# MachinaIO/mxx

Hardware: AMD Instinct MI355X
Metric: dcrt_ring_ops_per_s (higher is better)
Workload: dtype u32

## Files before the change

include/gpupoly.h:

```cpp
#ifndef GPUPOLY_H
#define GPUPOLY_H

#include <stddef.h>
#include <stdint.h>

#ifdef __cplusplus
extern "C" {
#endif

typedef struct GpuContext GpuContext;
typedef struct GpuMatrix GpuMatrix;
typedef struct GpuEventSet GpuEventSet;
typedef struct GpuP1CovarianceCache GpuP1CovarianceCache;
typedef struct GpuComm GpuComm;

typedef struct GpuRngSeed {
    uint64_t words[4];
} GpuRngSeed;

#define GPU_POLY_FORMAT_COEFF 0
#define GPU_POLY_FORMAT_EVAL 1
#define GPU_MATRIX_DIST_UNIFORM 0
#define GPU_MATRIX_DIST_GAUSS 1
#define GPU_MATRIX_DIST_BIT 2
#define GPU_MATRIX_DIST_TERNARY 3
#define GPU_MATRIX_LAYOUT_WORDS 0
#define GPU_MATRIX_LAYOUT_PACKED24 1

int gpu_context_create(uint32_t logN, uint32_t L, uint32_t dnum, const uint64_t *moduli, size_t moduli_len,
                       const int *gpu_ids, size_t gpu_ids_len, GpuContext **out_ctx);
void gpu_context_destroy(GpuContext *ctx);
int gpu_context_get_N(const GpuContext *ctx, int *out_N);

int gpu_event_set_wait(GpuEventSet *events);
void gpu_event_set_destroy(GpuEventSet *events);

int gpu_device_count(int *out_count);
int gpu_device_mem_info(int device, size_t *out_free, size_t *out_total);
int gpu_device_synchronize(void);
int gpu_device_reset(void);

const char *gpu_last_error(void);
int gpu_set_last_error(const char *msg);

void *gpu_pinned_alloc(size_t bytes);
void gpu_pinned_free(void *ptr);

int gpu_matrix_create(GpuContext *ctx, int level, size_t rows, size_t cols, int format, GpuMatrix **out);
void gpu_matrix_destroy(GpuMatrix *mat);
int gpu_matrix_copy(GpuMatrix *dst, const GpuMatrix *src);
int gpu_matrix_copy_block(GpuMatrix *out, const GpuMatrix *src, size_t dst_row, size_t dst_col, size_t src_row,
                          size_t src_col, size_t rows, size_t cols);

int gpu_matrix_add(GpuMatrix *out, const GpuMatrix *lhs, const GpuMatrix *rhs);
int gpu_matrix_sub(GpuMatrix *out, const GpuMatrix *lhs, const GpuMatrix *rhs);
int gpu_matrix_add_block(GpuMatrix *out, const GpuMatrix *src, size_t dst_row, size_t dst_col, size_t src_row,
                         size_t src_col, size_t rows, size_t cols);
int gpu_matrix_mul(GpuMatrix *out, const GpuMatrix *lhs, const GpuMatrix *rhs);
int gpu_matrix_mul_scalar(GpuMatrix *out, const GpuMatrix *lhs, const GpuMatrix *scalar);
int gpu_matrix_equal(const GpuMatrix *lhs, const GpuMatrix *rhs, int *out_equal);

int gpu_matrix_ntt_all(GpuMatrix *mat);
int gpu_matrix_intt_all(GpuMatrix *mat);

int gpu_matrix_fill_gadget(GpuMatrix *out, uint32_t base_bits);
int gpu_matrix_fill_small_gadget(GpuMatrix *out, uint32_t base_bits);
int gpu_matrix_fill_small_decomposed_identity_chunk(GpuMatrix *out, const GpuMatrix *scalar_by_digit,
                                                    size_t chunk_idx);
int gpu_matrix_decompose_base(const GpuMatrix *src, uint32_t base_bits, GpuMatrix *out);
int gpu_matrix_decompose_base_small(const GpuMatrix *src, uint32_t base_bits, GpuMatrix *out);

int gpu_matrix_sample_distribution(GpuMatrix *out, int dist_type, double sigma, GpuRngSeed seed);
int gpu_matrix_sample_distribution_columns(GpuMatrix *out, int dist_type, double sigma, GpuRngSeed seed,
                                           size_t full_ncol, size_t col_offset);
int gpu_matrix_gauss_samp_gq_arb_base(GpuMatrix *src, uint32_t base_bits, double c, double dgg_stddev,
                                      GpuRngSeed seed, GpuMatrix *out);
int gpu_matrix_sample_p1_full(const GpuMatrix *a_mat, const GpuMatrix *b_mat, const GpuMatrix *d_mat,
                              const GpuMatrix *tp2, double sigma, double s, double dgg_stddev, GpuRngSeed seed,
                              GpuMatrix *out);
int gpu_matrix_create_p1_covariance_cache(const GpuMatrix *a_mat, const GpuMatrix *b_mat, const GpuMatrix *d_mat,
                                          double sigma, double s, double dgg_stddev,
                                          GpuP1CovarianceCache **out_cache);
void gpu_matrix_destroy_p1_covariance_cache(GpuP1CovarianceCache *cache);
int gpu_matrix_sample_p1_full_cached(const GpuP1CovarianceCache *cache, const GpuMatrix *tp2, GpuRngSeed seed,
                                     GpuMatrix *out);

int gpu_matrix_load_rns_batch(GpuMatrix *mat, const uint8_t *bytes, size_t bytes_per_poly, int format,
                              GpuEventSet **out_events);
int gpu_matrix_store_rns_batch(const GpuMatrix *mat, uint8_t *bytes_out, size_t bytes_per_poly, int format,
                               GpuEventSet **out_events);
int gpu_matrix_store_const_coeff_batch(const GpuMatrix *mat, uint64_t *words_out, size_t words_per_poly,
                                       GpuEventSet **out_events);
int gpu_matrix_store_compact_bytes(GpuMatrix *mat, uint8_t *payload_out, size_t payload_capacity,
                                   uint16_t *out_max_coeff_bits, uint16_t *out_bytes_per_coeff,
                                   size_t *out_payload_len);
int gpu_matrix_load_compact_bytes(GpuMatrix *mat, const uint8_t *payload, size_t payload_len,
                                  uint16_t max_coeff_bits);
int gpu_poly_store_compact_bytes(GpuMatrix *poly, uint8_t *payload_out, size_t payload_capacity,
                                 uint16_t *out_max_coeff_bits, uint16_t *out_bytes_per_coeff,
                                 size_t *out_payload_len);
int gpu_poly_load_compact_bytes(GpuMatrix *poly, const uint8_t *payload, size_t payload_len,
                                uint16_t max_coeff_bits);

int gpupoly_matrix_mul_decompose(GpuMatrix *out, const GpuMatrix *lhs, const GpuMatrix *rhs, uint32_t base_bits);
int gpupoly_matrix_mul_decompose_many(GpuMatrix *const *outs, const GpuMatrix *const *lhss,
                                      const GpuMatrix *const *addends, const GpuMatrix *const *scalars, size_t n,
                                      const GpuMatrix *rhs, uint32_t base_bits);
int gpupoly_matrix_mul_decompose_pairs(GpuMatrix *const *outs, const GpuMatrix *const *addends,
                                       const GpuMatrix *const *lhss, const GpuMatrix *const *rhss,
                                       const GpuMatrix *const *scalars, size_t n,
                                       size_t col_start, uint32_t base_bits, int negate);
int gpupoly_matrix_mul_batch(GpuMatrix *const *outs, const GpuMatrix *const *lhss, const GpuMatrix *const *rhss, size_t count);
#define GPUPOLY_OP_MUL 0
#define GPUPOLY_OP_ADD 1
#define GPUPOLY_OP_SUB 2
#define GPUPOLY_OP_MUL_SCALAR 3
#define GPUPOLY_OP_NEG 4
#define GPUPOLY_OP_DECOMPOSE 5
#define GPUPOLY_OP_MUL_DECOMPOSE 6
typedef struct GpuBatchOp {
    int kind;
    GpuMatrix *out;
    const GpuMatrix *lhs;
    const GpuMatrix *rhs;
} GpuBatchOp;
int gpupoly_batch(const GpuBatchOp *ops, size_t count, uint32_t base_bits);
int gpupoly_matrix_mul_decompose_small(GpuMatrix *out, const GpuMatrix *lhs, const GpuMatrix *rhs, uint32_t base_bits);
int gpupoly_matrix_mul_tensor_identity(GpuMatrix *out, const GpuMatrix *lhs, const GpuMatrix *rhs, size_t identity_size);
int gpupoly_matrix_mul_tensor_identity_decompose(GpuMatrix *out, const GpuMatrix *lhs, const GpuMatrix *rhs,
                                                 size_t identity_size, uint32_t base_bits);
int gpupoly_matrix_mul_scalar_intt(GpuMatrix *out, const GpuMatrix *lhs, const GpuMatrix *scalar_1x1);
int gpupoly_matrix_transpose(GpuMatrix *out, const GpuMatrix *src);
int gpupoly_matrix_tensor(GpuMatrix *out, const GpuMatrix *lhs, const GpuMatrix *rhs);
int gpupoly_matrix_add_rows(GpuMatrix *out, size_t dst_row, const GpuMatrix *lhs, const GpuMatrix *rhs);
int gpupoly_matrix_ntt_add_rows(GpuMatrix *out, size_t dst_row, GpuMatrix *coeff, const GpuMatrix *addend,
                                int consume_coeff);
int gpupoly_matrix_row_view(GpuMatrix *m, size_t row, size_t rows, GpuMatrix **out_view);
int gpupoly_matrix_reshape_view(GpuMatrix *m, size_t rows, size_t cols, GpuMatrix **out_view);
int gpupoly_matrix_neg(GpuMatrix *out, const GpuMatrix *src);
int gpupoly_matrix_fill_zero(GpuMatrix *out);
int gpupoly_matrix_fill_identity(GpuMatrix *out, const GpuMatrix *scalar_1x1);
int gpupoly_matrix_sample_decomposed(GpuMatrix *out, int dist_type, double sigma, GpuRngSeed seed, uint32_t base_bits,
                                     int small);
int gpupoly_matrix_decompose_rows(const GpuMatrix *src, uint32_t base_bits, int small, size_t row_start, GpuMatrix *out);
int gpupoly_matrix_sample_decomposed_window(GpuMatrix *out, int dist_type, double sigma, GpuRngSeed seed,
                                            uint32_t base_bits, int small, size_t src_rows, size_t full_ncol,
                                            size_t col_offset, size_t row_start);
int gpupoly_timer_start(GpuContext *ctx);
int gpupoly_timer_stop(GpuContext *ctx, float *out_ms);
int gpupoly_timer_mark(GpuContext *ctx, uint32_t slot);
int gpupoly_timer_elapsed(GpuContext *ctx, uint32_t slot_begin, uint32_t slot_end, float *out_ms);
int gpupoly_matrix_device_ptr(const GpuMatrix *mat, void **out_ptr, size_t *out_bytes);
int gpupoly_matrix_layout(const GpuMatrix *mat, int *out);
int gpupoly_matrix_copy_to_context(GpuContext *dst_ctx, const GpuMatrix *src, GpuMatrix **out);
int gpupoly_context_device(const GpuContext *ctx, int *out_device);
int gpupoly_context_word_bytes(const GpuContext *ctx, int *out_bytes);
const char *gpupoly_context_last_kernel(const GpuContext *ctx);
int gpupoly_context_stream(const GpuContext *ctx, void **out_stream);
int gpupoly_comm_create(GpuContext *const *ctxs, size_t n, GpuComm **out_comm);
void gpupoly_comm_destroy(GpuComm *comm);
int gpupoly_comm_size(const GpuComm *comm, int *out_size);
const char *gpupoly_comm_backend(const GpuComm *comm);
int gpupoly_matrix_all_gather_columns(GpuComm *comm, const GpuMatrix *const *local_blocks, GpuMatrix *const *full);
int gpupoly_matrix_sample_distribution_segments(GpuMatrix *out, int dist_type, double sigma, const GpuRngSeed *seeds,
                                                const size_t *seg_cols, size_t nseg);
int gpupoly_matrix_sample_p1_full_cached_segments(const GpuP1CovarianceCache *cache, const GpuMatrix *tp2,
                                                  const GpuRngSeed *seeds, const size_t *seg_cols, size_t nseg,
                                                  GpuMatrix *out);
int gpupoly_matrix_gauss_samp_gq_arb_base_segments(GpuMatrix *src, uint32_t base_bits, double c, double dgg_stddev,
                                                   const GpuRngSeed *seeds, const size_t *seg_cols, size_t nseg,
                                                   GpuMatrix *out);
#define GPUPOLY_BLOCKS_STACKED 0
#define GPUPOLY_BLOCKS_COLUMNS 1
int gpupoly_matrix_sample_distribution_blocks(GpuMatrix *out, int dist_type, const GpuRngSeed *seeds, size_t nblk,
                                              int layout, const size_t *seg_cols);
#define GPUPOLY_HASH_KECCAK256 0
#define GPUPOLY_HASH_SHA3_256 1
#define GPUPOLY_TAGS_TABLE 0
#define GPUPOLY_TAGS_INDEXED_LE64 1
#define GPUPOLY_TAGS_INDEXED_DECIMAL 2
typedef struct GpuHashTags {
    int hash;
    int form;
    uint8_t key[32];
    const uint8_t *tags;
    const size_t *tag_offsets;
    size_t prefix_len;
    uint64_t first_index;
} GpuHashTags;
int gpupoly_hash_seeds(GpuContext *ctx, const GpuHashTags *tags, size_t ntags, GpuRngSeed *seeds_out);
int gpupoly_matrix_sample_hash_blocks(GpuMatrix *out, int dist_type, const GpuHashTags *tags, size_t nblk, int layout,
                                      const size_t *seg_cols);
int gpupoly_matrix_sample_gauss_blocks(GpuMatrix *out, double sigma, const GpuRngSeed *seeds, size_t nblk, int layout,
                                       const size_t *seg_cols);
int gpupoly_matrix_sample_hash_gauss_blocks(GpuMatrix *out, double sigma, const GpuHashTags *tags, size_t nblk, int layout,
                                            const size_t *seg_cols);
int gpupoly_matrix_concat_columns(GpuMatrix *out, const GpuMatrix *const *blocks, size_t n);
int gpupoly_matrix_split_columns(const GpuMatrix *src, GpuMatrix *const *blocks, size_t n);
int gpupoly_trapdoor_preimage_many(const GpuMatrix *re, const GpuP1CovarianceCache *cache, const GpuMatrix *public_matrix,
                                   uint32_t base_bits, const GpuMatrix *const *targets, size_t n, const GpuRngSeed *seeds,
                                   GpuMatrix *const *outs);
int gpupoly_trapdoor_preimage_keyed(const GpuMatrix *const *res, const GpuP1CovarianceCache *const *caches,
                                    const GpuMatrix *const *public_matrices, size_t nkeys, uint32_t base_bits,
                                    const uint32_t *key_of, const GpuMatrix *const *targets, size_t n,
                                    const GpuRngSeed *seeds, GpuMatrix *const *outs);
int gpupoly_matrix_sample_decomposed_blocks(GpuMatrix *out, int dist_type, const GpuRngSeed *seeds, size_t nblk,
                                            uint32_t base_bits, int small, size_t src_rows, size_t full_ncol,
                                            size_t col_offset);
int gpupoly_matrix_sample_hash_decomposed_blocks(GpuMatrix *out, int dist_type, const GpuHashTags *tags, size_t nblk,
                                                 uint32_t base_bits, int small, size_t src_rows, size_t full_ncol,
                                                 size_t col_offset);
int gpupoly_matrix_lut_targets(GpuMatrix *const *outs, size_t nrows_T, const GpuMatrix *w_identity, const GpuMatrix *w_gy,
                               const GpuMatrix *w_v, const GpuMatrix *w_vx, size_t col_start, uint32_t base_bits,
                               const uint64_t *y_words, size_t words_per_y, const uint64_t *idx, const GpuHashTags *tags);
int gpupoly_matrix_lut_targets_combine(GpuMatrix *const *outs, size_t nrows_T, const GpuMatrix *w_identity,
                                       const GpuMatrix *w_gy, const GpuMatrix *product, size_t col_start, uint32_t base_bits,
                                       const uint64_t *y_words, size_t words_per_y, const uint64_t *idx);
int gpupoly_matrix_lwe_targets(GpuMatrix *const *outs, size_t nrows_T, const GpuMatrix *a_z, const GpuMatrix *a_lt,
                               size_t col_start, uint32_t base_bits, const uint64_t *y_words, size_t words_per_y,
                               const uint64_t *x, const GpuHashTags *tags);
int gpupoly_matrix_lwe_targets_combine(GpuMatrix *const *outs, size_t nrows_T, const GpuMatrix *a_lt,
                                       const GpuMatrix *digits, const GpuMatrix *product, size_t col_start,
                                       uint32_t base_bits, const uint64_t *y_words, size_t words_per_y, const uint64_t *x);
int gpupoly_matrix_wee25_targets(GpuMatrix *const *outs, size_t nblocks_T, size_t nparts_P, const GpuMatrix *t_bottom,
                                 size_t part_start, size_t secret_size, uint32_t base_bits, const uint64_t *idx,
                                 const GpuHashTags *tags);
int gpupoly_matrix_wee25_targets_product(GpuMatrix *const *outs, size_t nblocks_T, size_t nparts_P, const GpuMatrix *w_stacked,
                                         const GpuMatrix *t_bottom, size_t part_start, size_t secret_size,
                                         uint32_t base_bits, const uint64_t *idx);
int gpupoly_matrix_ggh15_lookup(GpuMatrix *const *outs, size_t nslots_S, const GpuMatrix *mid_identity,
                                const GpuMatrix *mid_gy, const GpuMatrix *mid_v, const GpuMatrix *mid_vx,
                                const GpuMatrix *mid_rand, const GpuMatrix *mid_gate1,
                                const GpuMatrix *const *lut_preimages, const GpuMatrix *const *xs, size_t col_start,
                                uint32_t base_bits, const uint64_t *y_words, size_t words_per_y, const GpuHashTags *tags);
int gpupoly_matrix_ggh15_lookup_combine(GpuMatrix *const *outs, size_t nslots_S, const GpuMatrix *mid_identity,
                                        const GpuMatrix *mid_gy, const GpuMatrix *mid_v, const GpuMatrix *mid_vx,
                                        const GpuMatrix *mid_rand, const GpuMatrix *mid_gate1,
                                        const GpuMatrix *const *lut_preimages, const GpuMatrix *const *xs, size_t col_start,
                                        uint32_t base_bits, const uint64_t *y_words, size_t words_per_y,
                                        const GpuMatrix *digits);
int gpupoly_matrix_scale_round(GpuMatrix *out, const GpuMatrix *in, uint64_t t, int round_half);
int gpupoly_matrix_crt_recompose_rounded(GpuMatrix *out, const GpuMatrix *const *terms, const int *signs,
                                         size_t terms_per_level, size_t num_slots);
int gpupoly_matrix_store_coeff_words(const GpuMatrix *mat, uint64_t *out, size_t words_per_coeff);
int gpupoly_matrix_load_coeff_words(GpuMatrix *mat, const uint64_t *words, size_t words_per_coeff, size_t coeffs_per_poly,
                                    int out_format);
int gpupoly_matrix_centered_max_abs(const GpuMatrix *mat, uint64_t *out, size_t words_per_value);
int gpupoly_matrix_extract_bits(const GpuMatrix *mat, const uint64_t *lo, const uint64_t *hi, size_t words_per_bound,
                                uint8_t *out, size_t bytes_per_poly);
int gpupoly_matrix_store_coeff_ints(const GpuMatrix *mat, void *out, int elem_bytes, int centred, size_t coeffs_per_poly,
                                    uint64_t *out_misfit_count, uint64_t *out_first_misfit);
int gpupoly_matrix_store_compact_bytes_many(GpuMatrix *const *mats, size_t n, uint8_t *payload_out, size_t payload_capacity,
                                            uint16_t *out_max_coeff_bits, uint16_t *out_bytes_per_coeff,
                                            size_t *out_payload_offsets, size_t *out_payload_lens, size_t *out_total_len);
int gpupoly_matrix_load_compact_bytes_many(GpuMatrix *const *mats, size_t n, const uint8_t *const *payloads,
                                           const size_t *payload_lens, const uint16_t *max_coeff_bits);
int gpupoly_matrix_fill_monomial(GpuMatrix *out, uint64_t shift, int format);
int gpupoly_matrix_mul_monomial(GpuMatrix *out, const GpuMatrix *in, uint64_t shift);
int gpupoly_matrix_monomial_sum(GpuMatrix *out, const GpuMatrix *addend, const GpuMatrix *const *mats,
                                const uint64_t *shifts, size_t n, int negate);
int gpupoly_matrix_mul_sum(GpuMatrix *out, size_t dst_col, size_t cols, const GpuMatrix *addend,
                           const GpuMatrix *const *lhss, const GpuMatrix *const *rhss, size_t n, int negate);
int gpupoly_matrix_mul_acc(GpuMatrix *out, const GpuMatrix *lhs, const GpuMatrix *rhs, int negate);
int gpupoly_matrix_mul_gadget(GpuMatrix *out, size_t dst_col, const GpuMatrix *lhs, const GpuMatrix *scalar_1x1,
                              size_t gadget_col, size_t cols, const GpuMatrix *addend, int negate, uint32_t base_bits,
                              int small);
int gpupoly_matrix_gadget_mul(GpuMatrix *out, const GpuMatrix *rhs, const GpuMatrix *addend, int negate,
                              uint32_t base_bits, int small);
int gpupoly_matrix_mul_decompose_gadget_scalar_many(GpuMatrix *const *outs, const GpuMatrix *const *lhss,
                                                    const GpuMatrix *const *addends, size_t n, const GpuMatrix *scalar_1x1,
                                                    int negate, uint32_t base_bits);
int gpupoly_matrix_mul_decompose_gadget_const_many(GpuMatrix *const *outs, const GpuMatrix *const *lhss,
                                                   const GpuMatrix *const *addends, size_t n, const uint64_t *const_words,
                                                   size_t words_per_const, int negate, uint32_t base_bits);
uint64_t gpupoly_launch_count(void);
int gpupoly_detmath_eval(GpuContext *ctx, int fn, const double *host_in, double *host_out, size_t n);
int gpupoly_device_can_access_peer(int device, int peer, int *out_can);
int gpupoly_marker_launch(GpuContext *ctx, uint32_t id);
int gpupoly_trace_begin(void);
const char *gpupoly_trace_end(void);
const char *gpupoly_version(void);
int gpupoly_reload_env(void);

#ifdef __cplusplus
}
#endif
#endif
```

mxx_amd/__init__.py:

```python
from ._ffi import (
    GPU_MATRIX_DIST_BIT,
    GPU_MATRIX_DIST_GAUSS,
    GPU_MATRIX_DIST_TERNARY,
    GPU_MATRIX_DIST_UNIFORM,
    GPU_POLY_FORMAT_COEFF,
    GPU_POLY_FORMAT_EVAL,
    GpuPolyError,
    GpuRngSeed,
    detected_gpu_device_count,
    detected_gpu_device_ids,
    gpu_device_sync,
)
from .matrix import (
    GpuDCRTMatrixRnsSnapshot,
    GpuDCRTPolyMatrix,
    GpuP1CovarianceCache,
    block_offsets,
    block_size,
    one_rns_bytes,
    rns_bytes_len,
    rns_bytes_len_for_level,
)
from .params import DCRTPolyParams, GpuContext, GpuDCRTPolyParams, gen_crt_basis
from .poly import GpuDCRTPoly
from . import storage
from .sampler import (
    DistType,
    GpuDCRTPolyHashSampler,
    GpuDCRTPolyUniformSampler,
    IndexedTags,
    hash_seed_for_matrix,
    keccak256,
    random_gpu_rng_seed,
    sample_gpu_matrix_native,
    sample_gpu_matrix_with_seed,
    sample_gpu_matrix_with_seed_columns,
)
from .trapdoor import (
    GpuDCRTPolyTrapdoorSampler,
    GpuDCRTTrapdoor,
    GpuPerturbationSamples,
    coeff_cached_matrix,
    compute_preimage_norm,
    p1_covariance_parameters,
    preimage_c,
    preimage_smoothing_parameter,
)
from . import lookup
from . import lwe_lookup
from . import ggh15_eval
from . import slot_transfer
from . import commit
```

mxx_amd/_ffi.py:

```python
from __future__ import annotations

import ctypes as C
import os

_HERE = os.path.dirname(os.path.abspath(__file__))
LIB_PATH = os.environ.get("MXX_GPUPOLY_LIB") or os.path.join(_HERE, "libgpupoly.so")

GPU_POLY_FORMAT_COEFF = 0
GPU_POLY_FORMAT_EVAL = 1
GPU_MATRIX_DIST_UNIFORM = 0
GPU_MATRIX_DIST_GAUSS = 1
GPU_MATRIX_DIST_BIT = 2
GPU_MATRIX_DIST_TERNARY = 3
GPUPOLY_BLOCKS_STACKED = 0
GPUPOLY_BLOCKS_COLUMNS = 1
GPUPOLY_HASH_KECCAK256 = 0
GPUPOLY_HASH_SHA3_256 = 1
GPUPOLY_TAGS_TABLE = 0
GPUPOLY_TAGS_INDEXED_LE64 = 1
GPUPOLY_TAGS_INDEXED_DECIMAL = 2


class GpuPolyError(RuntimeError):
    """Raised where the reference's Rust wrapper panics (`check_status`, gpu.rs:259-263)."""


class GpuRngSeed(C.Structure):

    _fields_ = [("words", C.c_uint64 * 4)]

    @classmethod
    def from_bytes(cls, b: bytes) -> "GpuRngSeed":
        if len(b) != 32:
            raise ValueError("seed must be 32 bytes")
        s = cls()
        for i in range(4):
            s.words[i] = int.from_bytes(b[8 * i : 8 * i + 8], "little")
        return s

    def to_bytes(self) -> bytes:
        return b"".join(int(w).to_bytes(8, "little") for w in self.words)


class GpuHashTags(C.Structure):

    _fields_ = [("hash", C.c_int), ("form", C.c_int), ("key", C.c_uint8 * 32), ("tags", C.c_void_p),
                ("tag_offsets", C.POINTER(C.c_size_t)), ("prefix_len", C.c_size_t), ("first_index", C.c_uint64)]


class GpuBatchOp(C.Structure):

    _fields_ = [("kind", C.c_int), ("out", C.c_void_p), ("lhs", C.c_void_p), ("rhs", C.c_void_p)]


GPUPOLY_OP_MUL, GPUPOLY_OP_ADD, GPUPOLY_OP_SUB, GPUPOLY_OP_MUL_SCALAR, GPUPOLY_OP_NEG, GPUPOLY_OP_DECOMPOSE, GPUPOLY_OP_MUL_DECOMPOSE = range(7)

_vp = C.c_void_p
_sz = C.c_size_t
_u8p = C.POINTER(C.c_uint8)

SIGNATURES = {
    "gpu_context_create": (C.c_int, [C.c_uint32, C.c_uint32, C.c_uint32, C.POINTER(C.c_uint64), _sz, C.POINTER(C.c_int), _sz, C.POINTER(_vp)]),
    "gpu_context_destroy": (None, [_vp]),
    "gpu_context_get_N": (C.c_int, [_vp, C.POINTER(C.c_int)]),
    "gpu_event_set_wait": (C.c_int, [_vp]),
    "gpu_event_set_destroy": (None, [_vp]),
    "gpu_device_count": (C.c_int, [C.POINTER(C.c_int)]),
    "gpu_device_mem_info": (C.c_int, [C.c_int, C.POINTER(_sz), C.POINTER(_sz)]),
    "gpu_device_synchronize": (C.c_int, []),
    "gpu_device_reset": (C.c_int, []),
    "gpu_last_error": (C.c_char_p, []),
    "gpu_set_last_error": (C.c_int, [C.c_char_p]),
    "gpu_pinned_alloc": (_vp, [_sz]),
    "gpu_pinned_free": (None, [_vp]),
    "gpu_matrix_create": (C.c_int, [_vp, C.c_int, _sz, _sz, C.c_int, C.POINTER(_vp)]),
    "gpu_matrix_destroy": (None, [_vp]),
    "gpu_matrix_copy": (C.c_int, [_vp, _vp]),
    "gpu_matrix_copy_block": (C.c_int, [_vp, _vp, _sz, _sz, _sz, _sz, _sz, _sz]),
    "gpu_matrix_add": (C.c_int, [_vp, _vp, _vp]),
    "gpu_matrix_sub": (C.c_int, [_vp, _vp, _vp]),
    "gpu_matrix_add_block": (C.c_int, [_vp, _vp, _sz, _sz, _sz, _sz, _sz, _sz]),
    "gpu_matrix_mul": (C.c_int, [_vp, _vp, _vp]),
    "gpu_matrix_mul_scalar": (C.c_int, [_vp, _vp, _vp]),
    "gpu_matrix_equal": (C.c_int, [_vp, _vp, C.POINTER(C.c_int)]),
    "gpu_matrix_ntt_all": (C.c_int, [_vp]),
    "gpu_matrix_intt_all": (C.c_int, [_vp]),
    "gpu_matrix_fill_gadget": (C.c_int, [_vp, C.c_uint32]),
    "gpu_matrix_fill_small_gadget": (C.c_int, [_vp, C.c_uint32]),
    "gpu_matrix_fill_small_decomposed_identity_chunk": (C.c_int, [_vp, _vp, _sz]),
    "gpu_matrix_decompose_base": (C.c_int, [_vp, C.c_uint32, _vp]),
    "gpu_matrix_decompose_base_small": (C.c_int, [_vp, C.c_uint32, _vp]),
    "gpu_matrix_sample_distribution": (C.c_int, [_vp, C.c_int, C.c_double, GpuRngSeed]),
    "gpu_matrix_sample_distribution_columns": (C.c_int, [_vp, C.c_int, C.c_double, GpuRngSeed, _sz, _sz]),
    "gpu_matrix_gauss_samp_gq_arb_base": (C.c_int, [_vp, C.c_uint32, C.c_double, C.c_double, GpuRngSeed, _vp]),
    "gpu_matrix_sample_p1_full": (C.c_int, [_vp, _vp, _vp, _vp, C.c_double, C.c_double, C.c_double, GpuRngSeed, _vp]),
    "gpu_matrix_create_p1_covariance_cache": (C.c_int, [_vp, _vp, _vp, C.c_double, C.c_double, C.c_double, C.POINTER(_vp)]),
    "gpu_matrix_destroy_p1_covariance_cache": (None, [_vp]),
    "gpu_matrix_sample_p1_full_cached": (C.c_int, [_vp, _vp, GpuRngSeed, _vp]),
    "gpu_matrix_load_rns_batch": (C.c_int, [_vp, _vp, _sz, C.c_int, C.POINTER(_vp)]),
    "gpu_matrix_store_rns_batch": (C.c_int, [_vp, _vp, _sz, C.c_int, C.POINTER(_vp)]),
    "gpu_matrix_store_const_coeff_batch": (C.c_int, [_vp, _vp, _sz, C.POINTER(_vp)]),
    "gpu_matrix_store_compact_bytes": (C.c_int, [_vp, _vp, _sz, C.POINTER(C.c_uint16), C.POINTER(C.c_uint16), C.POINTER(_sz)]),
    "gpu_matrix_load_compact_bytes": (C.c_int, [_vp, _vp, _sz, C.c_uint16]),
    "gpu_poly_store_compact_bytes": (C.c_int, [_vp, _vp, _sz, C.POINTER(C.c_uint16), C.POINTER(C.c_uint16), C.POINTER(_sz)]),
    "gpu_poly_load_compact_bytes": (C.c_int, [_vp, _vp, _sz, C.c_uint16]),
    "gpupoly_matrix_mul_decompose": (C.c_int, [_vp, _vp, _vp, C.c_uint32]),
    "gpupoly_matrix_mul_decompose_many": (C.c_int, [C.POINTER(C.c_void_p), C.POINTER(C.c_void_p), C.POINTER(C.c_void_p), C.POINTER(C.c_void_p), C.c_size_t, _vp, C.c_uint32]),
    "gpupoly_matrix_mul_decompose_pairs": (C.c_int, [C.POINTER(C.c_void_p), C.POINTER(C.c_void_p), C.POINTER(C.c_void_p), C.POINTER(C.c_void_p), C.POINTER(C.c_void_p), _sz, _sz, C.c_uint32, C.c_int]),
    "gpupoly_matrix_mul_batch":(C.c_int, [C.POINTER(C.c_void_p), C.POINTER(C.c_void_p), C.POINTER(C.c_void_p), C.c_size_t]),
    "gpupoly_batch": (C.c_int, [C.POINTER(GpuBatchOp), C.c_size_t, C.c_uint32]),
    "gpupoly_matrix_mul_decompose_small": (C.c_int, [_vp, _vp, _vp, C.c_uint32]),
    "gpupoly_matrix_mul_tensor_identity": (C.c_int, [_vp, _vp, _vp, C.c_size_t]),
    "gpupoly_matrix_mul_tensor_identity_decompose": (C.c_int, [_vp, _vp, _vp, C.c_size_t, C.c_uint32]),
    "gpupoly_matrix_mul_scalar_intt": (C.c_int, [_vp, _vp, _vp]),
    "gpupoly_matrix_transpose": (C.c_int, [_vp, _vp]),
    "gpupoly_matrix_tensor": (C.c_int, [_vp, _vp, _vp]),
    "gpupoly_matrix_add_rows": (C.c_int, [_vp, C.c_size_t, _vp, _vp]),
    "gpupoly_matrix_ntt_add_rows": (C.c_int, [_vp, C.c_size_t, _vp, _vp, C.c_int]),
    "gpupoly_matrix_row_view": (C.c_int, [_vp, C.c_size_t, C.c_size_t, C.POINTER(C.c_void_p)]),
    "gpupoly_matrix_reshape_view": (C.c_int, [_vp, C.c_size_t, C.c_size_t, C.POINTER(C.c_void_p)]),
    "gpupoly_matrix_neg": (C.c_int, [_vp, _vp]),
    "gpupoly_matrix_fill_zero": (C.c_int, [_vp]),
    "gpupoly_matrix_fill_identity": (C.c_int, [_vp, _vp]),
    "gpupoly_matrix_sample_decomposed": (C.c_int, [_vp, C.c_int, C.c_double, GpuRngSeed, C.c_uint32, C.c_int]),
    "gpupoly_matrix_decompose_rows": (C.c_int, [_vp, C.c_uint32, C.c_int, _sz, _vp]),
    "gpupoly_matrix_sample_decomposed_window": (C.c_int, [_vp, C.c_int, C.c_double, GpuRngSeed, C.c_uint32, C.c_int, _sz, _sz, _sz, _sz]),
    "gpupoly_timer_start": (C.c_int, [_vp]),
    "gpupoly_timer_stop": (C.c_int, [_vp, C.POINTER(C.c_float)]),
    "gpupoly_timer_mark": (C.c_int, [_vp, C.c_uint32]),
    "gpupoly_timer_elapsed": (C.c_int, [_vp, C.c_uint32, C.c_uint32, C.POINTER(C.c_float)]),
    "gpupoly_matrix_device_ptr": (C.c_int, [_vp, C.POINTER(_vp), C.POINTER(_sz)]),
    "gpupoly_matrix_layout": (C.c_int, [_vp, C.POINTER(C.c_int)]),
    "gpupoly_matrix_copy_to_context": (C.c_int, [_vp, _vp, C.POINTER(_vp)]),
    "gpupoly_context_device": (C.c_int, [_vp, C.POINTER(C.c_int)]),
    "gpupoly_context_word_bytes": (C.c_int, [_vp, C.POINTER(C.c_int)]),
    "gpupoly_context_last_kernel": (C.c_char_p, [_vp]),
    "gpupoly_context_stream": (C.c_int, [_vp, C.POINTER(C.c_void_p)]),
    "gpupoly_comm_create": (C.c_int, [C.POINTER(C.c_void_p), C.c_size_t, C.POINTER(_vp)]),
    "gpupoly_comm_destroy": (None, [_vp]),
    "gpupoly_comm_size": (C.c_int, [_vp, C.POINTER(C.c_int)]),
    "gpupoly_comm_backend": (C.c_char_p, [_vp]),
    "gpupoly_matrix_all_gather_columns": (C.c_int, [_vp, C.POINTER(C.c_void_p), C.POINTER(C.c_void_p)]),
    "gpupoly_matrix_sample_distribution_segments": (C.c_int, [_vp, C.c_int, C.c_double, C.POINTER(GpuRngSeed), C.POINTER(_sz), _sz]),
    "gpupoly_matrix_sample_distribution_blocks": (C.c_int, [_vp, C.c_int, C.POINTER(GpuRngSeed), _sz, C.c_int, C.POINTER(_sz)]),
    "gpupoly_hash_seeds": (C.c_int, [_vp, C.POINTER(GpuHashTags), _sz, C.POINTER(GpuRngSeed)]),
    "gpupoly_matrix_sample_hash_blocks": (C.c_int, [_vp, C.c_int, C.POINTER(GpuHashTags), _sz, C.c_int, C.POINTER(_sz)]),
    "gpupoly_matrix_sample_gauss_blocks": (C.c_int, [_vp, C.c_double, C.POINTER(GpuRngSeed), _sz, C.c_int, C.POINTER(_sz)]),
    "gpupoly_matrix_sample_hash_gauss_blocks": (C.c_int, [_vp, C.c_double, C.POINTER(GpuHashTags), _sz, C.c_int, C.POINTER(_sz)]),
    "gpupoly_matrix_sample_decomposed_blocks": (C.c_int, [_vp, C.c_int, C.POINTER(GpuRngSeed), _sz, C.c_uint32, C.c_int, _sz, _sz, _sz]),
    "gpupoly_matrix_sample_hash_decomposed_blocks": (C.c_int, [_vp, C.c_int, C.POINTER(GpuHashTags), _sz, C.c_uint32, C.c_int, _sz, _sz, _sz]),
    "gpupoly_matrix_lut_targets": (C.c_int, [C.POINTER(C.c_void_p), _sz, _vp, _vp, _vp, _vp, _sz, C.c_uint32, C.POINTER(C.c_uint64), _sz,
                                   C.POINTER(C.c_uint64), C.POINTER(GpuHashTags)]),
    "gpupoly_matrix_lut_targets_combine": (C.c_int, [C.POINTER(C.c_void_p), _sz, _vp, _vp, _vp, _sz, C.c_uint32, C.POINTER(C.c_uint64), _sz,
                                           C.POINTER(C.c_uint64)]),
    "gpupoly_matrix_lwe_targets": (C.c_int, [C.POINTER(C.c_void_p), _sz, _vp, _vp, _sz, C.c_uint32, C.POINTER(C.c_uint64), _sz,
                                   C.POINTER(C.c_uint64), C.POINTER(GpuHashTags)]),
    "gpupoly_matrix_lwe_targets_combine": (C.c_int, [C.POINTER(C.c_void_p), _sz, _vp, _vp, _vp, _sz, C.c_uint32, C.POINTER(C.c_uint64), _sz,
                                           C.POINTER(C.c_uint64)]),
    "gpupoly_matrix_wee25_targets": (C.c_int, [C.POINTER(C.c_void_p), _sz, _sz, _vp, _sz, _sz, C.c_uint32, C.POINTER(C.c_uint64),
                                     C.POINTER(GpuHashTags)]),
    "gpupoly_matrix_wee25_targets_product": (C.c_int, [C.POINTER(C.c_void_p), _sz, _sz, _vp, _vp, _sz, _sz, C.c_uint32,
                                             C.POINTER(C.c_uint64)]),
    "gpupoly_matrix_ggh15_lookup": (C.c_int, [C.POINTER(C.c_void_p), _sz, _vp, _vp, _vp, _vp, _vp, _vp, C.POINTER(C.c_void_p),
                                    C.POINTER(C.c_void_p), _sz, C.c_uint32, C.POINTER(C.c_uint64), _sz, C.POINTER(GpuHashTags)]),
    "gpupoly_matrix_ggh15_lookup_combine": (C.c_int, [C.POINTER(C.c_void_p), _sz, _vp, _vp, _vp, _vp, _vp, _vp, C.POINTER(C.c_void_p),
                                            C.POINTER(C.c_void_p), _sz, C.c_uint32, C.POINTER(C.c_uint64), _sz, _vp]),
    "gpupoly_matrix_sample_p1_full_cached_segments":(C.c_int, [_vp, _vp, C.POINTER(GpuRngSeed), C.POINTER(_sz), _sz, _vp]),
    "gpupoly_matrix_gauss_samp_gq_arb_base_segments": (C.c_int, [_vp, C.c_uint32, C.c_double, C.c_double, C.POINTER(GpuRngSeed), C.POINTER(_sz), _sz, _vp]),
    "gpupoly_matrix_concat_columns": (C.c_int, [_vp, C.POINTER(C.c_void_p), _sz]),
    "gpupoly_matrix_split_columns": (C.c_int, [_vp, C.POINTER(C.c_void_p), _sz]),
    "gpupoly_trapdoor_preimage_many": (C.c_int, [_vp, _vp, _vp, C.c_uint32, C.POINTER(C.c_void_p), _sz, C.POINTER(GpuRngSeed), C.POINTER(C.c_void_p)]),
    "gpupoly_trapdoor_preimage_keyed": (C.c_int, [C.POINTER(C.c_void_p), C.POINTER(C.c_void_p), C.POINTER(C.c_void_p), _sz, C.c_uint32,
                                        C.POINTER(C.c_uint32), C.POINTER(C.c_void_p), _sz, C.POINTER(GpuRngSeed), C.POINTER(C.c_void_p)]),
    "gpupoly_launch_count": (C.c_uint64, []),
    "gpupoly_matrix_scale_round": (C.c_int, [_vp, _vp, C.c_uint64, C.c_int]),
    "gpupoly_matrix_crt_recompose_rounded": (C.c_int, [_vp, C.POINTER(C.c_void_p), C.POINTER(C.c_int), _sz, _sz]),
    "gpupoly_matrix_store_coeff_words": (C.c_int, [_vp, C.POINTER(C.c_uint64), _sz]),
    "gpupoly_matrix_load_coeff_words": (C.c_int, [_vp, C.POINTER(C.c_uint64), _sz, _sz, C.c_int]),
    "gpupoly_matrix_centered_max_abs": (C.c_int, [_vp, C.POINTER(C.c_uint64), _sz]),
    "gpupoly_matrix_extract_bits": (C.c_int, [_vp, C.POINTER(C.c_uint64), C.POINTER(C.c_uint64), _sz, _u8p, _sz]),
    "gpupoly_matrix_store_coeff_ints": (C.c_int, [_vp, _vp, C.c_int, C.c_int, _sz, C.POINTER(C.c_uint64), C.POINTER(C.c_uint64)]),
    "gpupoly_matrix_fill_monomial": (C.c_int, [_vp, C.c_uint64, C.c_int]),
    "gpupoly_matrix_mul_monomial": (C.c_int, [_vp, _vp, C.c_uint64]),
    "gpupoly_matrix_monomial_sum": (C.c_int, [_vp, _vp, C.POINTER(C.c_void_p), C.POINTER(C.c_uint64), _sz, C.c_int]),
    "gpupoly_matrix_mul_sum": (C.c_int, [_vp, _sz, _sz, _vp, C.POINTER(C.c_void_p), C.POINTER(C.c_void_p), _sz, C.c_int]),
    "gpupoly_matrix_mul_acc": (C.c_int, [_vp, _vp, _vp, C.c_int]),
    "gpupoly_matrix_mul_gadget": (C.c_int, [_vp, _sz, _vp, _vp, _sz, _sz, _vp, C.c_int, C.c_uint32, C.c_int]),
    "gpupoly_matrix_gadget_mul": (C.c_int, [_vp, _vp, _vp, C.c_int, C.c_uint32, C.c_int]),
    "gpupoly_matrix_mul_decompose_gadget_scalar_many": (C.c_int, [C.POINTER(C.c_void_p), C.POINTER(C.c_void_p), C.POINTER(C.c_void_p), _sz, _vp, C.c_int, C.c_uint32]),
    "gpupoly_matrix_mul_decompose_gadget_const_many": (C.c_int, [C.POINTER(C.c_void_p), C.POINTER(C.c_void_p), C.POINTER(C.c_void_p), _sz, C.POINTER(C.c_uint64), _sz, C.c_int, C.c_uint32]),
    "gpupoly_matrix_store_compact_bytes_many": (C.c_int, [C.POINTER(C.c_void_p), _sz, _vp, _sz, C.POINTER(C.c_uint16), C.POINTER(C.c_uint16), C.POINTER(_sz), C.POINTER(_sz), C.POINTER(_sz)]),
    "gpupoly_matrix_load_compact_bytes_many": (C.c_int, [C.POINTER(C.c_void_p), _sz, C.POINTER(C.c_void_p), C.POINTER(_sz), C.POINTER(C.c_uint16)]),
    "gpupoly_detmath_eval": (C.c_int, [_vp, C.c_int, C.POINTER(C.c_double), C.POINTER(C.c_double), _sz]),
    "gpupoly_device_can_access_peer": (C.c_int, [C.c_int, C.c_int, C.POINTER(C.c_int)]),
    "gpupoly_marker_launch": (C.c_int, [_vp, C.c_uint32]),
    "gpupoly_trace_begin": (C.c_int, []),
    "gpupoly_trace_end": (C.c_char_p, []),
    "gpupoly_version": (C.c_char_p, []),
    "gpupoly_reload_env": (C.c_int, []),
}

_lib = None


def lib() -> C.CDLL:
    global _lib
    if _lib is None:
        if not os.path.exists(LIB_PATH):
            raise GpuPolyError(
                f"{LIB_PATH} is missing: build it with `python -c 'import __graft_entry__ as g; g.build()'` "
                "(or `make -C mxx_amd/csrc`). mxx_amd has no CPU fallback."
            )
        handle = C.CDLL(LIB_PATH)
        for name, (res, args) in SIGNATURES.items():
            fn = getattr(handle, name)
            fn.restype = res
            fn.argtypes = args
        _lib = handle
    return _lib


def last_error_string() -> str:
    msg = lib().gpu_last_error()
    return msg.decode("utf-8", "replace") if msg else "unknown GPU error"


def check_status(code: int, context: str) -> None:
    if code != 0:
        raise GpuPolyError(f"{context} failed: {last_error_string()}")


def reload_env() -> None:
    check_status(lib().gpupoly_reload_env(), "gpupoly_reload_env")


def trace_begin() -> None:
    check_status(lib().gpupoly_trace_begin(), "gpupoly_trace_begin")


def trace_end() -> list[dict]:
    text = lib().gpupoly_trace_end()
    if text is None:
        raise GpuPolyError(f"gpupoly_trace_end failed: {last_error_string()}")
    out = []
    for ln in text.decode().splitlines():
        name, blocks, threads, nbytes, ms = ln.split("\t")
        out.append({"kernel": name.strip("()"), "blocks": int(blocks), "threads": int(threads), "bytes": float(nbytes), "ms": float(ms)})
    return out


def gpu_device_sync() -> None:
    check_status(lib().gpu_device_synchronize(), "gpu_device_synchronize")


def detected_gpu_device_ids() -> list[int]:
    n = C.c_int(0)
    if lib().gpu_device_count(C.byref(n)) != 0 or n.value <= 0:
        return []
    return list(range(n.value))


def peer_access_matrix(devices=None) -> list[list[int]]:
    devs = detected_gpu_device_ids() if devices is None else list(devices)
    out = []
    for a in devs:
        row = []
        for b in devs:
            can = C.c_int(0)
            check_status(lib().gpupoly_device_can_access_peer(a, b, C.byref(can)), "gpupoly_device_can_access_peer")
            row.append(int(can.value))
        out.append(row)
    return out


def detected_gpu_device_count() -> int:
    return len(detected_gpu_device_ids())


def wait_and_destroy_events(events: _vp) -> None:
    if events:
        st = lib().gpu_event_set_wait(events)
        lib().gpu_event_set_destroy(events)
        check_status(st, "gpu_event_set_wait")
```

mxx_amd/csrc/common.h:

```cpp
#pragma once

#include <hip/hip_runtime.h>

#include <atomic>
#include <cstddef>
#include <cstdint>
#include <cstdio>
#include <exception>
#include <map>
#include <unordered_map>
#include <mutex>
#include <string>
#include <vector>

#include "../../include/gpupoly.h"

constexpr size_t GPUPOLY_MAX_LIMBS = 64;

struct LimbConst {
    uint64_t q;
    uint64_t mu;
    uint64_t mu64;
    uint64_t n_inv;
    uint64_t n_inv_sh;
    uint64_t mu32;
    uint64_t inv_last_w;
    uint64_t inv_last_w_sh;
    uint32_t kbits;
    uint32_t lazy_terms;
};

struct EnvSwitches {
    int ntt_path = 0;
    int ntt14 = 0;
    bool decompose_fused = true;
    char matmul_path = 0;
    int matmul_tile = 0;
    bool gsamp_simple = false;
    bool gsamp_no_uni = false;
    bool p1_simple = false;
    int sampler_per_lane = 0;
    int sampler_fill_every = 0;
    bool ntt64_int = false;
    int ntt_phase = 0;
    bool serde_general = false;
    bool rng_compat = false;
    bool pack24 = true;
    int skinny24 = 0;
    int skinny24_shape = 0;
    size_t mul_decompose_many_budget = 0;
    size_t mul_decompose_pairs_budget = 0;
    size_t gadget_scalar_budget = 0;
    size_t ggh15_lookup_budget = 0;
    char mul_sum_path = 0;
    size_t crt_recompose_chunk_bytes = size_t(256) << 20;
    void load();
};

struct GpuContext {
    EnvSwitches env;
    int device = 0;
    std::vector<int> gpu_ids;
    uint32_t logN = 0;
    int N = 0;
    int level = 0;
    uint32_t dnum = 0;
    int limb_count = 0;
    bool wide = false;
    int word_bytes = 4;
    uint32_t crt_bits = 0;
    std::vector<uint64_t> moduli;
    hipStream_t stream = nullptr;
    LimbConst *d_limbs = nullptr;
    LimbConst *d_limbs_r = nullptr;
    void *d_tw_fwd = nullptr;
    void *d_tw_fwd_sh = nullptr;
    void *d_tw_inv = nullptr;
    void *d_tw_inv_sh = nullptr;
    void *d_tw2_fwd = nullptr;
    void *d_tw2_inv = nullptr;
    bool lazy_ok = false;
    bool tight_ok = false;
    void *d_tw2s_inv = nullptr;
    bool signed_ok = false;
    void *d_twf_fwd = nullptr, *d_twf_inv = nullptr;
    void *d_flimbs = nullptr;
    bool f64_ok = false;
    uint64_t *d_garner = nullptr;
    std::vector<uint64_t> garner_inv;
    std::vector<LimbConst> limbs;
    hipEvent_t timer_start = nullptr, timer_stop = nullptr;
    std::vector<hipEvent_t> marks;
    std::mutex mutex;
    bool pool_ok = false;
    std::mutex alloc_mutex;
    std::multimap<size_t, void *> free_blocks;
    std::unordered_map<void *, size_t> live_blocks;
    size_t cached_bytes = 0, cache_limit = 0;
    std::atomic<const char *> last_kernel{""};
    bool pack24_ok = false;
    std::mutex layout_mutex;
    std::map<uint32_t, void *> gadget_weights;
    std::map<std::vector<uint64_t>, void *> gadget_const_tables;
};

struct LayoutTag {
    std::atomic<int> v{GPU_MATRIX_LAYOUT_WORDS};
    LayoutTag() = default;
    LayoutTag(const LayoutTag &o) : v(o.v.load(std::memory_order_acquire)) {}
    LayoutTag &operator=(const LayoutTag &o) {
        v.store(o.v.load(std::memory_order_acquire), std::memory_order_release);
        return *this;
    }
};

struct GpuMatrix {
    GpuContext *ctx = nullptr;
    int level = 0;
    size_t rows = 0, cols = 0;
    int format = GPU_POLY_FORMAT_EVAL;
    void *storage = nullptr;
    size_t bytes = 0;
    LayoutTag layout;
    bool borrowed = false;
    GpuMatrix *parent = nullptr;
    int views = 0;
};

struct GpuEventSet {
    std::vector<hipEvent_t> events;
    int device = 0;
    void *staging = nullptr;
    GpuContext *ctx = nullptr;
    void *dev_staging = nullptr;
};

struct GpuP1CovarianceCache {
    GpuContext *ctx = nullptr;
    int level = 0;
    size_t d = 0, m = 0, n = 0;
    double sigma = 0, s = 0, dgg_stddev = 0;
    double *sqrt_var = nullptr;
    double *update_coeff = nullptr;
    void *karney_div = nullptr;
};

struct P1KeyEntry {
    const double *sqrt_var;
    const double *update_coeff;
    const void *karney_div;
};

static inline dim3 item_grid(size_t items, unsigned threads) {
    const size_t blocks = (items + threads - 1) / threads;
    const size_t max_x = (static_cast<size_t>(1) << 31) / threads;
    if (blocks <= max_x) return dim3(static_cast<unsigned>(blocks ? blocks : 1));
    const size_t y = (blocks + max_x - 1) / max_x;
    return dim3(static_cast<unsigned>((blocks + y - 1) / y), static_cast<unsigned>(y));
}
#if defined(__HIPCC__)
__device__ __forceinline__ size_t item_index() {
    return (static_cast<size_t>(blockIdx.y) * gridDim.x + blockIdx.x) * blockDim.x + threadIdx.x;
}
#endif

extern std::atomic<uint64_t> g_kernel_launches;
extern std::atomic<int> g_trace_on;
void trace_launch_begin(const char *name, hipStream_t stream, dim3 grid, dim3 block);
void trace_launch_end(hipStream_t stream);
void trace_set_bytes(double bytes);
#define MXX_TRACE_BYTES(b)                                                                        \
    do {                                                                                          \
        if (g_trace_on.load(std::memory_order_relaxed)) trace_set_bytes(static_cast<double>(b)); \
    } while (0)
#define MXX_LAUNCH(kern, grid, block, lds, strm, ...)                          \
    do {                                                                       \
        g_kernel_launches.fetch_add(1, std::memory_order_relaxed);             \
        const bool mxx_tr_ = g_trace_on.load(std::memory_order_relaxed) != 0;  \
        if (mxx_tr_) trace_launch_begin(#kern, strm, grid, block);             \
        hipLaunchKernelGGL(kern, grid, block, lds, strm, __VA_ARGS__);         \
        if (mxx_tr_) trace_launch_end(strm);                                   \
    } while (0)
#define MXX_TRACED_COPY(name, strm, bytes, stmt)                               \
    do {                                                                       \
        const bool mxx_tr_ = g_trace_on.load(std::memory_order_relaxed) != 0;  \
        if (mxx_tr_) {                                                         \
            trace_set_bytes(static_cast<double>(bytes));                       \
            trace_launch_begin(name, strm, dim3(0), dim3(0));                  \
        }                                                                      \
        stmt;                                                                  \
        if (mxx_tr_) trace_launch_end(strm);                                   \
    } while (0)

int set_error(const char *msg);
int set_error(const std::string &msg);
int set_error(hipError_t err, const char *what);

#define HIP_TRY(expr)                                          \
    do {                                                       \
        hipError_t _e = (expr);                                \
        if (_e != hipSuccess) return set_error(_e, #expr);     \
    } while (0)

template <auto... KERNELS>
static int lds_opt_in(const GpuContext *ctx, size_t lds) {
    static std::atomic<uint64_t> configured{0};
    const uint64_t bit = 1ull << (ctx->device & 63);
    if (lds <= 64 * 1024 || (configured.load() & bit)) return 0;
    for (const void *f : {reinterpret_cast<const void *>(KERNELS)...})
        HIP_TRY(hipFuncSetAttribute(f, hipFuncAttributeMaxDynamicSharedMemorySize, static_cast<int>(lds)));
    configured.fetch_or(bit);
    return 0;
}

extern int (*g_roctx_push)(const char *);
extern int (*g_roctx_pop)();
void roctx_init_once();
struct RoctxScope {
    bool on;
    explicit RoctxScope(const char *name) {
        roctx_init_once();
        on = g_roctx_push != nullptr;
        if (on) g_roctx_push(name);
    }
    ~RoctxScope() {
        if (on) g_roctx_pop();
    }
};

#define ABI_GUARD_BEGIN try { RoctxScope roctx_scope_(__func__);
#define ABI_GUARD_END                                                         \
    }                                                                         \
    catch (const std::exception &e) { return set_error(e.what()); }           \
    catch (...) { return set_error("unknown exception in libgpupoly"); }

inline size_t matrix_polys(const GpuMatrix *m) { return m->rows * m->cols; }
inline size_t matrix_limbs(const GpuMatrix *m) { return static_cast<size_t>(m->level) + 1; }
inline size_t matrix_words(const GpuMatrix *m) { return matrix_polys(m) * matrix_limbs(m) * static_cast<size_t>(m->ctx->N); }

void *words_ptr(const GpuMatrix *m);
const void *packed24_ptr(const GpuMatrix *m, bool *packed);
inline size_t packed24_bytes(const GpuMatrix *m) { return m->bytes / 4 * 3; }
inline bool storage_overlaps(const GpuMatrix *x, const GpuMatrix *y) {
    if (x == y) return true;
    if (!x->storage || !y->storage || x->bytes == 0 || y->bytes == 0) return false;
    const size_t xb = x->layout.v.load(std::memory_order_acquire) == GPU_MATRIX_LAYOUT_PACKED24 ? packed24_bytes(x) : x->bytes;
    const size_t yb = y->layout.v.load(std::memory_order_acquire) == GPU_MATRIX_LAYOUT_PACKED24 ? packed24_bytes(y) : y->bytes;
    const char *xs = static_cast<const char *>(x->storage), *ys = static_cast<const char *>(y->storage);
    return xs < ys + yb && ys < xs + xb;
}
inline bool same_block(const GpuMatrix *x, const GpuMatrix *y) {
    return x == y || (x->storage == y->storage && x->bytes == y->bytes);
}
inline bool partial_overlap(const GpuMatrix *out, const GpuMatrix *operand) {
    return storage_overlaps(out, operand) && !same_block(out, operand);
}
inline bool row_block_overlaps(const GpuMatrix *m, size_t row, size_t rows, const GpuMatrix *y) {
    if (m->layout.v.load(std::memory_order_acquire) == GPU_MATRIX_LAYOUT_PACKED24) return rows && m->cols && storage_overlaps(m, y);
    if (!m->storage) return false;
    const size_t poly_bytes = matrix_limbs(m) * static_cast<size_t>(m->ctx->N) * m->ctx->word_bytes;
    GpuMatrix block;
    block.storage = static_cast<char *>(m->storage) + row * m->cols * poly_bytes;
    block.bytes = rows * m->cols * poly_bytes;
    return storage_overlaps(&block, y);
}
bool pack24_eligible(const GpuMatrix *m);
int pack24_store(GpuMatrix *m, bool ntt);

int sample_impl(GpuMatrix *out, int dist, double sigma, GpuRngSeed seed, size_t full_ncol, size_t col_offset, bool keep_coeff,
                size_t row_offset = 0, uint32_t tower_first = 0, uint32_t tower_count = 0);

struct RngBlockWindow {
    size_t cols, full_ncol, col_offset;
};
int sample_blocks_impl(const char *entry, bool hashed, GpuMatrix *out, int dist_type, const GpuRngSeed *seeds, const GpuHashTags *tags,
                       size_t nblk, int layout, const size_t *seg_cols, const RngBlockWindow *win, const double *sigma = nullptr);
int sample_decomposed_blocks_impl(const char *entry, bool hashed, GpuMatrix *out, int dist_type, const GpuRngSeed *seeds,
                                  const GpuHashTags *tags, size_t nblk, uint32_t base_bits, int small, size_t src_rows, size_t full_ncol,
                                  size_t col_offset);

int hash_tags_check(const char *entry, const GpuHashTags *tags, size_t ntags, size_t *table_bytes);
size_t hash_tags_staged_words(const GpuHashTags *tags, size_t ntags, size_t table_bytes);
void hash_tags_stage(const GpuHashTags *tags, size_t ntags, size_t table_bytes, uint64_t *staging);
int launch_hash_seeds(GpuContext *ctx, GpuRngSeed *d_seeds, const GpuHashTags *tags, size_t ntags, const uint64_t *d_staged);

int ctx_activate(const GpuContext *ctx);
bool ctx_is_registered(const GpuContext *ctx);
int ctx_alloc(GpuContext *ctx, size_t bytes, void **out);
void ctx_free(GpuContext *ctx, void *ptr);
struct CtxBlock {
    GpuContext *ctx;
    void *ptr = nullptr;
    explicit CtxBlock(GpuContext *c) : ctx(c) {}
    CtxBlock(const CtxBlock &) = delete;
    CtxBlock &operator=(const CtxBlock &) = delete;
    ~CtxBlock() {
        if (ptr) ctx_free(ctx, ptr);
    }
    int alloc(size_t bytes) { return ctx_alloc(ctx, bytes, &ptr); }
    void *release() {
        void *p = ptr;
        ptr = nullptr;
        return p;
    }
};
int matrix_check_same_shape(const GpuMatrix *a, const GpuMatrix *b, const char *who);
int coeff_domain_source(const GpuMatrix *mat, CtxBlock &scratch, const void **src);

int launch_ntt(GpuContext *ctx, void *data, size_t vectors, int limbs_per_poly, bool inverse);
int launch_ntt_lds_u32(GpuContext *ctx, uint32_t *data, size_t vectors, uint32_t L, bool inverse);
int launch_ntt_digits_u32(GpuContext *ctx, uint32_t *out, const uint32_t *coeff, size_t out_vectors, uint32_t L,
                          uint32_t src_cols, uint32_t towers, uint32_t dpt, uint32_t base_bits, size_t k, uint32_t td0 = 0);
int launch_ntt_lds_u64(GpuContext *ctx, uint64_t *data, size_t vectors, uint32_t L, bool inverse);
int launch_ntt_digits_u64(GpuContext *ctx, uint64_t *out, const uint64_t *coeff, size_t out_vectors, uint32_t L,
                          uint32_t src_cols, uint32_t towers, uint32_t dpt, uint32_t base_bits, size_t k, uint32_t td0 = 0);
int launch_intt_oop_u32(GpuContext *ctx, uint32_t *out, const uint32_t *in, size_t vectors, uint32_t L);
int launch_ntt_add_u32(GpuContext *ctx, uint32_t *out, const uint32_t *src, const uint32_t *add, size_t vectors, uint32_t L);
int launch_mul_intt_u32(GpuContext *ctx, uint32_t *out, const uint32_t *in, const uint32_t *w, size_t vectors, uint32_t L);
int launch_matmul(GpuMatrix *out, const GpuMatrix *lhs, const GpuMatrix *rhs);
int launch_ntt_fwd_pack24_u32(GpuContext *ctx, uint32_t *out, const uint32_t *in, size_t vectors, uint32_t L);
int launch_matmul_skinny24(GpuMatrix *out, const GpuMatrix *lhs, const GpuMatrix *rhs, bool small_grid);
int skinny24_parse_shape(const char *s);
int launch_matmul_dma_u32(GpuMatrix *out, const GpuMatrix *lhs, const GpuMatrix *rhs);
int launch_matmul_dma32_u32(GpuMatrix *out, const GpuMatrix *lhs, const GpuMatrix *rhs);
int launch_matmul_mfma_u32(GpuMatrix *out, const GpuMatrix *lhs, const GpuMatrix *rhs);
int launch_copy_block(GpuMatrix *out, const GpuMatrix *src, size_t dst_row, size_t dst_col, size_t src_row,
                      size_t src_col, size_t rows, size_t cols, bool add);
int sample_p1_keyed_segments(const GpuP1CovarianceCache *cache, const P1KeyEntry *d_keys, const GpuMatrix *tp2,
                             const GpuRngSeed *seeds, const size_t *seg_cols, size_t nseg, GpuMatrix *out);
int launch_scatter_i64(GpuMatrix *out, const int64_t *vals);
int finish_staged_i64(GpuMatrix *out, CtxBlock &stage, hipError_t launch_err, const char *what, bool transform = true);
```

mxx_amd/csrc/runtime.hip:

```cpp
#include "common.h"

#include <algorithm>
#include <cstdlib>
#include <iterator>
#include <map>
#include <cstring>
#include <dlfcn.h>

typedef unsigned __int128 u128h;

static thread_local std::string g_last_error;

int set_error(const char *msg) {
    g_last_error = msg ? msg : "unknown error";
    return 1;
}
int set_error(const std::string &msg) {
    g_last_error = msg;
    return 1;
}
int set_error(hipError_t err, const char *what) {
    g_last_error = std::string(what ? what : "hip call") + ": " + hipGetErrorString(err);
    (void)hipGetLastError();
    return 1;
// ... 81 lines not shown
    HIP_TRY(hipGetLastError());
    return 0;
    ABI_GUARD_END
}

extern "C" int gpupoly_trace_begin(void) {
    ABI_GUARD_BEGIN
    std::lock_guard<std::mutex> lk(g_trace_mutex);
    for (const TraceEntry &en : g_trace) {
        trace_event_return(en.device, en.e0);
        trace_event_return(en.device, en.e1);
    }
    g_trace.clear();
    g_trace_on.store(1, std::memory_order_relaxed);
    return 0;
    ABI_GUARD_END
}

extern "C" const char *gpupoly_trace_end(void) {
    try {
        g_trace_on.store(0, std::memory_order_relaxed);
        std::lock_guard<std::mutex> lk(g_trace_mutex);
        g_trace_report.clear();
        int prev = 0;
        (void)hipGetDevice(&prev);
        char line[512];
        for (const TraceEntry &en : g_trace) {
            if (!en.closed) continue;
            (void)hipSetDevice(en.device);
            float ms = 0;
            hipError_t e = hipEventSynchronize(en.e1);
            if (e == hipSuccess) e = hipEventElapsedTime(&ms, en.e0, en.e1);
            if (e != hipSuccess) {
                (void)hipSetDevice(prev);
                set_error(e, "gpupoly_trace_end: hipEventElapsedTime");
                return nullptr;
            }
            std::snprintf(line, sizeof line, "%s\t%llu\t%u\t%.0f\t%.6f\n", en.name, en.blocks, en.threads, en.bytes, ms);
            g_trace_report += line;
        }
        for (const TraceEntry &en : g_trace) {
            trace_event_return(en.device, en.e0);
            trace_event_return(en.device, en.e1);
        }
        g_trace.clear();
        (void)hipSetDevice(prev);
        return g_trace_report.c_str();
    } catch (...) {
        set_error("gpupoly_trace_end: exception");
        return nullptr;
    }
}

int (*g_roctx_push)(const char *) = nullptr;
int (*g_roctx_pop)() = nullptr;
void roctx_init_once() {
    static std::once_flag once;
    std::call_once(once, [] {
        const char *sw = std::getenv("MXX_HIP_ROCTX");
        const bool profiled = std::getenv("ROCP_TOOL_LIBRARIES") != nullptr || std::getenv("ROCPROFILER_REGISTER_FORCE_LOAD") != nullptr;
        if (sw ? sw[0] == '0' : !profiled) return;
        for (const char *name : {"librocprofiler-sdk-roctx.so.1", "librocprofiler-sdk-roctx.so", "libroctx64.so.4", "libroctx64.so"}) {
            void *h = dlopen(name, RTLD_NOW | RTLD_GLOBAL);
            if (!h) continue;
            auto push = reinterpret_cast<int (*)(const char *)>(dlsym(h, "roctxRangePushA"));
            auto pop = reinterpret_cast<int (*)()>(dlsym(h, "roctxRangePop"));
            if (push && pop) {
                g_roctx_pop = pop;
                g_roctx_push = push;
                return;
            }
        }
    });
}

static inline uint64_t h_mulmod(uint64_t a, uint64_t b, uint64_t q) { return (uint64_t)(((u128h)a * b) % q); }
static uint64_t h_powmod(uint64_t b, uint64_t e, uint64_t q) {
    uint64_t r = 1 % q;
    b %= q;
    while (e) {
        if (e & 1) r = h_mulmod(r, b, q);
        b = h_mulmod(b, b, q);
        e >>= 1;
    }
    return r;
}
static uint64_t h_invmod_prime(uint64_t a, uint64_t q) { return h_powmod(a % q, q - 2, q); }

static bool h_is_prime(uint64_t n) {
    static const uint64_t bases[] = {2, 3, 5, 7, 11, 13, 17, 19, 23, 29, 31, 37};
    if (n < 2) return false;
    for (uint64_t b : bases)
        if (n % b == 0) return n == b;
    uint64_t d = n - 1;
    int s = 0;
    while (!(d & 1)) { d >>= 1; ++s; }
    for (uint64_t b : bases) {
        uint64_t x = h_powmod(b, d, n);
        if (x == 1 || x == n - 1) continue;
        bool comp = true;
        for (int r = 1; r < s; ++r) {
            x = h_mulmod(x, x, n);
            if (x == n - 1) { comp = false; break; }
        }
        if (comp) return false;
    }
    return true;
}

static uint64_t h_min_primitive_root(uint64_t q, uint64_t order) {
    uint64_t qm1 = q - 1;
    int v = __builtin_ctzll(qm1);
    int want = __builtin_ctzll(order);
    uint64_t odd = qm1 >> v;
    uint64_t maximal = 0;
    for (uint64_t x = 2; x < q; ++x) {
        uint64_t r = h_powmod(x, odd, q);
        if (h_powmod(r, 1ull << (v - 1), q) != 1) { maximal = r; break; }
    }
    uint64_t root = h_powmod(maximal, 1ull << (v - want), q);
    uint64_t sq = h_mulmod(root, root, q);
    uint64_t cur = root, best = root;
    for (uint64_t i = 1; i < order / 2; ++i) {
        cur = h_mulmod(cur, sq, q);
        if (cur < best) best = cur;
    }
    return best;
}

static inline uint32_t h_bitrev(uint32_t x, uint32_t bits) {
    uint32_t r = 0;
    for (uint32_t i = 0; i < bits; ++i) { r = (r << 1) | (x & 1); x >>= 1; }
    return r;
}
static inline uint32_t h_bits(uint64_t v) { return v ? 64 - (uint32_t)__builtin_clzll(v) : 0; }

void EnvSwitches::load() {
    *this = EnvSwitches();
    if (const char *e = std::getenv("MXX_HIP_NTT_PATH")) {
        if (e[0] == 'l') ntt_path = 1;
        else if (e[0] == 'g' && e[1] == 'e') ntt_path = 2;
        else if (e[0] == 'g' && e[1] == 'l') ntt_path = 3;
    }
    if (const char *e = std::getenv("MXX_HIP_NTT14")) ntt14 = e[0] == 'w' ? 1 : (e[0] == 'u' ? 2 : 0);
    if (const char *e = std::getenv("MXX_HIP_DECOMPOSE_FUSED")) decompose_fused = e[0] != '0';
    if (const char *e = std::getenv("MXX_HIP_MATMUL_PATH")) matmul_path = e[0];
    if (const char *e = std::getenv("MXX_HIP_MATMUL_TILE")) {
        if (e[0] && e[1] && e[2]) matmul_tile = ((e[0] - '0') * 100 + (e[1] - '0') * 10 + (e[2] - '0')) * 2 + (e[3] == 'p');
    }
    if (const char *e = std::getenv("MXX_HIP_GSAMP")) {
        gsamp_simple = e[0] == 's';
        gsamp_no_uni = e[0] == 'n';
    }
    if (const char *e = std::getenv("MXX_HIP_P1")) p1_simple = e[0] == 's';
    if (const char *e = std::getenv("MXX_HIP_NTT64")) ntt64_int = e[0] == 'i';
    if (const char *e = std::getenv("MXX_HIP_RNG_COMPAT")) rng_compat = e[0] == 'r';
    if (const char *e = std::getenv("MXX_HIP_SERDE")) serde_general = e[0] == 'g';
    if (const char *e = std::getenv("MXX_HIP_PACK24")) pack24 = !(std::strcmp(e, "0") == 0 || std::strcmp(e, "off") == 0);
    if (const char *e = std::getenv("MXX_HIP_SKINNY24")) {
        if (std::strcmp(e, "0") == 0) skinny24 = 1;
        else if (std::strncmp(e, "force", 5) == 0 && (e[5] == 0 || e[5] == ':')) {
            skinny24 = 2;
            if (e[5] == ':') skinny24_shape = skinny24_parse_shape(e + 6) ? skinny24_parse_shape(e + 6) : -1;
        }
    }
    if (const char *e = std::getenv("MXX_HIP_MUL_DECOMPOSE_MANY_BUDGET")) mul_decompose_many_budget = static_cast<size_t>(std::strtoull(e, nullptr, 10));
    if (const char *e = std::getenv("MXX_HIP_MUL_DECOMPOSE_PAIRS_BUDGET")) mul_decompose_pairs_budget = static_cast<size_t>(std::strtoull(e, nullptr, 10));
    if (const char *e = std::getenv("MXX_HIP_GADGET_SCALAR_BUDGET")) gadget_scalar_budget = static_cast<size_t>(std::strtoull(e, nullptr, 10));
    if (const char *e = std::getenv("MXX_HIP_GGH15_LOOKUP_BUDGET")) ggh15_lookup_budget = static_cast<size_t>(std::strtoull(e, nullptr, 10));
    if (const char *e = std::getenv("MXX_HIP_CRT_RECOMPOSE_CHUNK_BYTES")) {
        const size_t v = static_cast<size_t>(std::strtoull(e, nullptr, 10));
        if (v >= 1) crt_recompose_chunk_bytes = v;
    }
    if (const char *e = std::getenv("MXX_HIP_MUL_SUM_PATH")) mul_sum_path = (e[0] == 't' || e[0] == 's') ? e[0] : 0;
    if (const char *e = std::getenv("MXX_HIP_SAMPLER_PER_LANE")) {
        const int v = std::atoi(e);
        if (v >= 1 && v <= 4096) sampler_per_lane = v;
    }
    if (const char *e = std::getenv("MXX_HIP_NTT_PHASE")) {
        const int v = std::atoi(e);
        if (v >= 0 && v <= 127) ntt_phase = v;
    }
    if (const char *e = std::getenv("MXX_HIP_SAMPLER_FILL_EVERY")) {
        const int v = std::atoi(e);
        if (v >= 1 && v <= 8) sampler_fill_every = v;
    }
}

static std::mutex g_registry_mutex;
static std::vector<GpuContext *> g_contexts;
bool ctx_is_registered(const GpuContext *ctx) {
    std::lock_guard<std::mutex> lk(g_registry_mutex);
    return std::find(g_contexts.begin(), g_contexts.end(), ctx) != g_contexts.end();
}

extern "C" int gpupoly_reload_env(void) {
    std::lock_guard<std::mutex> lk(g_registry_mutex);
    for (GpuContext *c : g_contexts) c->env.load();
    return 0;
}

int ctx_activate(const GpuContext *ctx) {
    HIP_TRY(hipSetDevice(ctx->device));
    return 0;
}

static size_t round_block(size_t bytes) {
    const size_t gran = bytes >= (size_t(1) << 20) ? (size_t(1) << 20) : 4096;
    return (bytes + gran - 1) / gran * gran;
}

static void cache_trim(GpuContext *ctx, size_t limit) {
    while (ctx->cached_bytes > limit && !ctx->free_blocks.empty()) {
        auto it = std::prev(ctx->free_blocks.end());
        (void)hipFree(it->second);
        ctx->cached_bytes -= it->first;
        ctx->free_blocks.erase(it);
    }
}

int ctx_alloc(GpuContext *ctx, size_t bytes, void **out) {
    *out = nullptr;
    if (bytes == 0) return 0;
    const size_t want = round_block(bytes);
    std::lock_guard<std::mutex> lk(ctx->alloc_mutex);
    auto it = ctx->free_blocks.lower_bound(want);
    if (it != ctx->free_blocks.end() && it->first <= want + want / 4) {
        *out = it->second;
        ctx->live_blocks[*out] = it->first;
        ctx->cached_bytes -= it->first;
        ctx->free_blocks.erase(it);
        return 0;
    }
    hipError_t e = hipMalloc(out, want);
    if (e != hipSuccess) {
        (void)hipGetLastError();
        cache_trim(ctx, 0);
        e = hipMalloc(out, want);
    }
    if (e != hipSuccess) {
        (void)hipGetLastError();
        {
            std::lock_guard<std::mutex> reg(g_registry_mutex);
            for (GpuContext *other : g_contexts) {
                if (other == ctx || other->device != ctx->device) continue;
                if (!other->alloc_mutex.try_lock()) continue;
                cache_trim(other, 0);
                other->alloc_mutex.unlock();
            }
        }
        e = hipMalloc(out, want);
        if (e != hipSuccess) {
            *out = nullptr;
            return set_error(e, "hipMalloc");
        }
    }
    ctx->live_blocks[*out] = want;
    return 0;
}

void ctx_free(GpuContext *ctx, void *ptr) {
    if (!ptr) return;
    std::lock_guard<std::mutex> lk(ctx->alloc_mutex);
    auto it = ctx->live_blocks.find(ptr);
    if (it == ctx->live_blocks.end()) {
        (void)hipFree(ptr);
        return;
    }
    const size_t size = it->second;
    ctx->live_blocks.erase(it);
    if (!ctx->pool_ok) {
        (void)hipFree(ptr);
        return;
    }
    ctx->free_blocks.emplace(size, ptr);
    ctx->cached_bytes += size;
    cache_trim(ctx, ctx->cache_limit);
}

template <typename W>
static int upload_tables(GpuContext *ctx, const std::vector<std::vector<uint64_t>> &fwd,
                         const std::vector<std::vector<uint64_t>> &inv) {
    const size_t N = ctx->N, L = ctx->limb_count;
    const unsigned shift = sizeof(W) * 8;
    std::vector<W> h_f(L * N), h_fs(L * N), h_i(L * N), h_is(L * N);
    for (size_t l = 0; l < L; ++l) {
        uint64_t q = ctx->moduli[l];
        for (size_t j = 0; j < N; ++j) {
            h_f[l * N + j] = (W)fwd[l][j];
            h_fs[l * N + j] = (W)(((u128h)fwd[l][j] << shift) / q);
            h_i[l * N + j] = (W)inv[l][j];
            h_is[l * N + j] = (W)(((u128h)inv[l][j] << shift) / q);
        }
    }
    size_t bytes = L * N * sizeof(W);
    HIP_TRY(hipMalloc(&ctx->d_tw_fwd, bytes));
    HIP_TRY(hipMalloc(&ctx->d_tw_fwd_sh, bytes));
    HIP_TRY(hipMalloc(&ctx->d_tw_inv, bytes));
    HIP_TRY(hipMalloc(&ctx->d_tw_inv_sh, bytes));
    HIP_TRY(hipMemcpy(ctx->d_tw_fwd, h_f.data(), bytes, hipMemcpyHostToDevice));
    HIP_TRY(hipMemcpy(ctx->d_tw_fwd_sh, h_fs.data(), bytes, hipMemcpyHostToDevice));
    HIP_TRY(hipMemcpy(ctx->d_tw_inv, h_i.data(), bytes, hipMemcpyHostToDevice));
    HIP_TRY(hipMemcpy(ctx->d_tw_inv_sh, h_is.data(), bytes, hipMemcpyHostToDevice));
    std::vector<W> h_pf(2 * L * N), h_pi(2 * L * N);
    for (size_t i = 0; i < L * N; ++i) {
        h_pf[2 * i] = static_cast<W>(0) - h_f[i];
        h_pf[2 * i + 1] = h_fs[i];
        h_pi[2 * i] = h_i[i];
        h_pi[2 * i + 1] = h_is[i];
    }
    HIP_TRY(hipMalloc(&ctx->d_tw2_fwd, 2 * bytes));
    HIP_TRY(hipMalloc(&ctx->d_tw2_inv, 2 * bytes));
    HIP_TRY(hipMemcpy(ctx->d_tw2_fwd, h_pf.data(), 2 * bytes, hipMemcpyHostToDevice));
    HIP_TRY(hipMemcpy(ctx->d_tw2_inv, h_pi.data(), 2 * bytes, hipMemcpyHostToDevice));
    if (sizeof(W) == 8 && ctx->crt_bits <= 51 && N >= 2) {
        struct HostTwF { double w, wi; };
        struct HostF64Limb { double q, qinv; HostTwF n_inv, last_w; };
        std::vector<HostTwF> tf(L * N), ti(L * N);
        std::vector<HostF64Limb> fl(L);
        for (size_t l = 0; l < L; ++l) {
            const double qd = static_cast<double>(ctx->moduli[l]);
            for (size_t j = 0; j < N; ++j) {
                tf[l * N + j] = {static_cast<double>(fwd[l][j]), static_cast<double>(fwd[l][j]) / qd};
                ti[l * N + j] = {static_cast<double>(inv[l][j]), static_cast<double>(inv[l][j]) / qd};
            }
            const LimbConst &lc = ctx->limbs[l];
            fl[l] = {qd, 1.0 / qd, {static_cast<double>(lc.n_inv), static_cast<double>(lc.n_inv) / qd},
                     {static_cast<double>(lc.inv_last_w), static_cast<double>(lc.inv_last_w) / qd}};
        }
        HIP_TRY(hipMalloc(&ctx->d_twf_fwd, sizeof(HostTwF) * L * N));
        HIP_TRY(hipMalloc(&ctx->d_twf_inv, sizeof(HostTwF) * L * N));
        HIP_TRY(hipMalloc(&ctx->d_flimbs, sizeof(HostF64Limb) * L));
        HIP_TRY(hipMemcpy(ctx->d_twf_fwd, tf.data(), sizeof(HostTwF) * L * N, hipMemcpyHostToDevice));
        HIP_TRY(hipMemcpy(ctx->d_twf_inv, ti.data(), sizeof(HostTwF) * L * N, hipMemcpyHostToDevice));
        HIP_TRY(hipMemcpy(ctx->d_flimbs, fl.data(), sizeof(HostF64Limb) * L, hipMemcpyHostToDevice));
        ctx->f64_ok = true;
    }
    if (ctx->signed_ok && sizeof(W) == 4) {
        auto signed_pair = [](uint64_t w, uint64_t q, W *dst) {
            const int64_t c = w > q / 2 ? static_cast<int64_t>(w) - static_cast<int64_t>(q) : static_cast<int64_t>(w);
            __int128 num = static_cast<__int128>(c) << 32;
            __int128 fl = num / static_cast<__int128>(q);
            if (num % static_cast<__int128>(q) < 0) fl -= 1;
            dst[0] = static_cast<W>(static_cast<uint32_t>(static_cast<int32_t>(c)));
            dst[1] = static_cast<W>(static_cast<uint32_t>(static_cast<int32_t>(fl)));
        };
        for (size_t l = 0; l < L; ++l)
            for (size_t j = 0; j < N; ++j) signed_pair(inv[l][j], ctx->moduli[l], &h_pi[2 * (l * N + j)]);
        HIP_TRY(hipMalloc(&ctx->d_tw2s_inv, 2 * bytes));
        HIP_TRY(hipMemcpy(ctx->d_tw2s_inv, h_pi.data(), 2 * bytes, hipMemcpyHostToDevice));
    }
    return 0;
}

static void context_release(GpuContext *ctx) {
    if (!ctx) return;
    {
        std::lock_guard<std::mutex> reg(g_registry_mutex);
        g_contexts.erase(std::remove(g_contexts.begin(), g_contexts.end(), ctx), g_contexts.end());
    }
    (void)hipSetDevice(ctx->device);
    if (ctx->stream) (void)hipStreamSynchronize(ctx->stream);
    for (auto &kv : ctx->free_blocks) (void)hipFree(kv.second);
    for (auto &kv : ctx->live_blocks) (void)hipFree(kv.first);
    if (ctx->d_limbs) (void)hipFree(ctx->d_limbs);
    if (ctx->d_limbs_r) (void)hipFree(ctx->d_limbs_r);
    if (ctx->d_twf_fwd) (void)hipFree(ctx->d_twf_fwd);
    if (ctx->d_twf_inv) (void)hipFree(ctx->d_twf_inv);
    if (ctx->d_flimbs) (void)hipFree(ctx->d_flimbs);
    if (ctx->d_tw_fwd) (void)hipFree(ctx->d_tw_fwd);
    if (ctx->d_tw_fwd_sh) (void)hipFree(ctx->d_tw_fwd_sh);
    if (ctx->d_tw_inv) (void)hipFree(ctx->d_tw_inv);
    if (ctx->d_tw_inv_sh) (void)hipFree(ctx->d_tw_inv_sh);
    if (ctx->d_garner) (void)hipFree(ctx->d_garner);
    if (ctx->d_tw2_fwd) (void)hipFree(ctx->d_tw2_fwd);
    if (ctx->d_tw2_inv) (void)hipFree(ctx->d_tw2_inv);
    if (ctx->d_tw2s_inv) (void)hipFree(ctx->d_tw2s_inv);
    for (auto &kv : ctx->gadget_weights) (void)hipFree(kv.second);
    for (auto &kv : ctx->gadget_const_tables) (void)hipFree(kv.second);
    if (ctx->timer_start) (void)hipEventDestroy(ctx->timer_start);
    if (ctx->timer_stop) (void)hipEventDestroy(ctx->timer_stop);
    for (hipEvent_t ev : ctx->marks)
        if (ev) (void)hipEventDestroy(ev);
    if (ctx->stream) (void)hipStreamDestroy(ctx->stream);
    delete ctx;
}

extern "C" int gpu_context_create(uint32_t logN, uint32_t L, uint32_t dnum, const uint64_t *moduli,
                                  size_t moduli_len, const int *gpu_ids, size_t gpu_ids_len, GpuContext **out_ctx) {
    ABI_GUARD_BEGIN
    if (!out_ctx) return set_error("gpu_context_create: null out_ctx");
    *out_ctx = nullptr;
    if (!moduli || moduli_len == 0) return set_error("gpu_context_create: empty moduli");
    if (moduli_len != static_cast<size_t>(L) + 1) return set_error("gpu_context_create: moduli_len must equal L+1");
    if (moduli_len > GPUPOLY_MAX_LIMBS) return set_error("gpu_context_create: too many limbs");
    if (!gpu_ids || gpu_ids_len == 0) return set_error("gpu_context_create: empty gpu_ids");
    if (logN < 1 || logN > 17) return set_error("gpu_context_create: logN out of range [1,17]");
    int dev_count = 0;
    HIP_TRY(hipGetDeviceCount(&dev_count));
    for (size_t i = 0; i < gpu_ids_len; ++i) {
        if (gpu_ids[i] < 0 || gpu_ids[i] >= dev_count) return set_error("gpu_context_create: invalid gpu id");
        for (size_t j = 0; j < i; ++j)
            if (gpu_ids[j] == gpu_ids[i]) return set_error("gpu_context_create: duplicate gpu id");
    }
    const uint64_t N = 1ull << logN;
    bool wide = false;
    for (size_t i = 0; i < moduli_len; ++i) {
        uint64_t q = moduli[i];
        if (q < 3 || (q - 1) % (2 * N) != 0) return set_error("gpu_context_create: modulus must be = 1 (mod 2N)");
        if (!h_is_prime(q)) return set_error("gpu_context_create: modulus is not prime");
        if (q >> 62) return set_error("gpu_context_create: modulus must be < 2^62");
        if (q >> 31) wide = true;
        for (size_t j = 0; j < i; ++j)
            if (moduli[j] == q) return set_error("gpu_context_create: duplicate modulus");
    }

    GpuContext *ctx = new GpuContext();
    ctx->device = gpu_ids[0];
    ctx->gpu_ids.assign(gpu_ids, gpu_ids + gpu_ids_len);
    ctx->logN = logN;
    ctx->N = static_cast<int>(N);
    ctx->level = static_cast<int>(L);
    ctx->dnum = dnum;
    ctx->limb_count = static_cast<int>(moduli_len);
    ctx->wide = wide;
    ctx->word_bytes = wide ? 8 : 4;
    ctx->moduli.assign(moduli, moduli + moduli_len);

    hipError_t e = hipSetDevice(ctx->device);
    if (e != hipSuccess) { delete ctx; return set_error(e, "hipSetDevice"); }
    e = hipStreamCreateWithFlags(&ctx->stream, hipStreamNonBlocking);
    if (e != hipSuccess) { delete ctx; return set_error(e, "hipStreamCreate"); }

    ctx->env.load();
    {
        ctx->pool_ok = true;
        size_t free_b = 0, total_b = 0;
        ctx->cache_limit = size_t(64) << 30;
        if (hipMemGetInfo(&free_b, &total_b) == hipSuccess && free_b) ctx->cache_limit = free_b / 2;
        else (void)hipGetLastError();
        const char *env = std::getenv("MXX_HIP_MEMPOOL_RELEASE_THRESHOLD_BYTES");
        if (!env) env = std::getenv("MXX_CUDA_MEMPOOL_RELEASE_THRESHOLD_BYTES");
        if (env && *env) ctx->cache_limit = std::strtoull(env, nullptr, 10);
        const char *nopool = std::getenv("MXX_HIP_DISABLE_MEMPOOL");
        if (nopool && *nopool == '1') ctx->pool_ok = false;
    }

    std::vector<std::vector<uint64_t>> fwd(moduli_len), inv(moduli_len);
    ctx->limbs.resize(moduli_len);
    uint32_t crt_bits = 0;
    for (size_t l = 0; l < moduli_len; ++l) {
        uint64_t q = moduli[l];
        uint64_t psi = h_min_primitive_root(q, 2 * N);
        uint64_t ipsi = h_invmod_prime(psi, q);
        fwd[l].resize(N);
        inv[l].resize(N);
        uint64_t p = 1, ip = 1;
        for (uint64_t i = 0; i < N; ++i) {
            uint32_t r = h_bitrev(static_cast<uint32_t>(i), logN);
            fwd[l][r] = p;
            inv[l][r] = ip;
            p = h_mulmod(p, psi, q);
            ip = h_mulmod(ip, ipsi, q);
        }
        LimbConst &lc = ctx->limbs[l];
        lc.q = q;
        lc.kbits = h_bits(q);
        crt_bits = std::max(crt_bits, lc.kbits);
        lc.mu = static_cast<uint64_t>((((u128h)1) << (2 * lc.kbits)) / q);
        lc.mu64 = static_cast<uint64_t>((((u128h)1) << 64) / q);
        lc.n_inv = h_invmod_prime(N % q, q);
        lc.n_inv_sh = static_cast<uint64_t>(((u128h)lc.n_inv << (wide ? 64 : 32)) / q);
        lc.mu32 = (((uint64_t)1) << 32) / q;
        lc.inv_last_w = h_mulmod(inv[l][1 % N], lc.n_inv, q);
        lc.inv_last_w_sh = static_cast<uint64_t>(((u128h)lc.inv_last_w << (wide ? 64 : 32)) / q);
        if (!wide) {
            u128h q2 = (u128h)(q - 1) * (q - 1);
            u128h terms = ((((u128h)1) << 64) - q) / q2;
            lc.lazy_terms = terms > (1u << 20) ? (1u << 20) : static_cast<uint32_t>(terms);
        } else {
            u128h q2 = (u128h)(q - 1) * (q - 1);
            u128h terms = (~(u128h)0 - q) / q2;
            lc.lazy_terms = terms > (1u << 20) ? (1u << 20) : static_cast<uint32_t>(terms);
        }
    }
    ctx->crt_bits = crt_bits;
    ctx->lazy_ok = crt_bits + 7 <= (wide ? 64u : 32u);
    ctx->tight_ok = !wide && !ctx->lazy_ok && crt_bits + 4 <= 32u;
    ctx->signed_ok = !wide && crt_bits <= 24;
    ctx->pack24_ok = !wide && crt_bits <= 24 && ctx->N % 4 == 0;

    ctx->garner_inv.assign(moduli_len * moduli_len, 0);
    for (size_t i = 0; i < moduli_len; ++i)
        for (size_t j = 0; j < i; ++j)
            ctx->garner_inv[i * moduli_len + j] = h_invmod_prime(moduli[j] % moduli[i], moduli[i]);

    int rc = 0;
    e = hipMalloc(&ctx->d_limbs, sizeof(LimbConst) * moduli_len);
    if (e == hipSuccess)
        e = hipMemcpy(ctx->d_limbs, ctx->limbs.data(), sizeof(LimbConst) * moduli_len, hipMemcpyHostToDevice);
    if (e == hipSuccess) e = hipMalloc(&ctx->d_garner, sizeof(uint64_t) * moduli_len * moduli_len);
    if (e == hipSuccess)
        e = hipMemcpy(ctx->d_garner, ctx->garner_inv.data(), sizeof(uint64_t) * moduli_len * moduli_len,
                      hipMemcpyHostToDevice);
    if (e == hipSuccess && !wide) {
        std::vector<LimbConst> lr = ctx->limbs;
        for (LimbConst &c : lr) {
            const uint64_t r = (1ull << 32) % c.q;
            c.n_inv = h_mulmod(c.n_inv, r, c.q);
            c.n_inv_sh = static_cast<uint64_t>(((u128h)c.n_inv << 32) / c.q);
            c.inv_last_w = h_mulmod(c.inv_last_w, r, c.q);
            c.inv_last_w_sh = static_cast<uint64_t>(((u128h)c.inv_last_w << 32) / c.q);
        }
        e = hipMalloc(&ctx->d_limbs_r, sizeof(LimbConst) * moduli_len);
        if (e == hipSuccess) e = hipMemcpy(ctx->d_limbs_r, lr.data(), sizeof(LimbConst) * moduli_len, hipMemcpyHostToDevice);
// ... 197 lines not shown
```

mxx_amd/csrc/trapdoor.hip:

```cpp
#include "common.h"
#include "modarith.h"
#include "rng.h"

#include <algorithm>
#include <cstdlib>

static constexpr uint64_t kTagGadget = 0x6761646765746731ull;
static constexpr uint64_t kTagP1 = 0x7065727475726231ull;
static constexpr int kGaussMaxDigits = 64;

__host__ __device__ __forceinline__ uint64_t gadget_stream0(uint32_t i, uint32_t t) {
    return ((static_cast<uint64_t>(i) + 1) << 8) | (static_cast<uint64_t>(t) + 1);
}

template <typename W, int MAXD>
__global__ void __launch_bounds__(128) gauss_samp_gq_kernel(W *__restrict__ out, const W *__restrict__ src,
                                     const LimbConst *__restrict__ limbs, size_t src_polys, uint32_t src_cols,
                                     uint32_t L, uint32_t N, uint32_t dpt, uint32_t base_bits, double c, size_t k,
                                     GpuRngSeed seed) {
    __shared__ uint32_t ring[128 * RNG_RING_SLOTS];
    const size_t idx = item_index();
    const size_t total = src_polys * L * N;
    if (idx >= total) return;
    const uint32_t i = static_cast<uint32_t>(idx % N);
    const size_t pt = idx / N;
    const uint32_t t = static_cast<uint32_t>(pt % L);
    const size_t p = pt / L;
    const uint64_t qt = limbs[t].q;
    uint64_t value = static_cast<uint64_t>(src[(p * L + t) * N + i]) % qt;

    const uint64_t base = 1ull << base_bits;
    const double base_f = static_cast<double>(base);
    const double sigma = c / (base_f + 1.0);
    const double kf = static_cast<double>(dpt);

    int64_t m_digits[MAXD], v_digits[MAXD], z[MAXD];
    double a[MAXD], zf[MAXD], cvec[MAXD];
    {
        uint64_t mq = qt, vv = value;
#pragma unroll
        for (int d = 0; d < MAXD; ++d) {
            if (d < (int)dpt) {
                m_digits[d] = static_cast<int64_t>(mq % base);
                mq /= base;
                v_digits[d] = static_cast<int64_t>(vv % base);
                vv /= base;
            } else {
                m_digits[d] = 0;
                v_digits[d] = 0;
            }
        }
    }
    ChaChaRng rng;
    rng_init(rng, ring, seed, gadget_stream0(i, t), static_cast<uint64_t>(p) + 1, 0, kTagGadget);
#pragma unroll
    for (int d = 0; d < MAXD; ++d) {
        if ((d & 3) == 0) rng_fill_lane(rng);
        zf[d] = d < (int)dpt ? sigma * rng_standard_normal(rng) : 0.0;
    }

    {
        double prev_c = 0.0;
#pragma unroll
        for (int d = 0; d < MAXD; ++d) {
            if (d < (int)dpt) {
                cvec[d] = (prev_c + static_cast<double>(m_digits[d])) / base_f;
                prev_c = cvec[d];
            } else {
                cvec[d] = 0.0;
            }
        }
        double prev_a = 0.0;
#pragma unroll
        for (int d = 0; d < MAXD; ++d) {
            if (d < (int)dpt) {
                const double ld = d == 0 ? sqrt(base_f * (1.0 + 1.0 / kf) + 1.0)
                                         : sqrt(base_f * (1.0 + 1.0 / (kf - static_cast<double>(d))));
                double pd;
                if (d + 1 < (int)dpt) {
                    const double hn = sqrt(base_f * (1.0 - 1.0 / (kf - static_cast<double>(d))));
                    pd = ld * zf[d] + hn * zf[d + 1 < MAXD ? d + 1 : d];
                } else {
                    const double hd = d == 0 ? 0.0 : sqrt(base_f * (1.0 - 1.0 / (kf - static_cast<double>(d - 1))));
                    pd = hd * zf[d];
                }
                a[d] = (prev_a + static_cast<double>(v_digits[d]) - pd) / base_f;
                prev_a = a[d];
            } else {
                a[d] = 0.0;
            }
        }
    }
    const int last = static_cast<int>(dpt) - 1;
    double a_last = 0.0, c_last = 1.0;
#pragma unroll
    for (int d = 0; d < MAXD; ++d)
        if (d == last) {
            a_last = a[d];
            c_last = cvec[d];
        }
    const int64_t z_last = sample_integer_karney(rng, -a_last / c_last, sigma / c_last);
#pragma unroll
    for (int d = 0; d < MAXD; ++d) a[d] += static_cast<double>(z_last) * cvec[d];
#pragma unroll
    for (int d = 0; d < MAXD; ++d) {
        if (d < last) z[d] = sample_integer_karney(rng, -a[d], sigma);
        else z[d] = z_last;
    }

    const size_t r = p / src_cols, col = p - r * src_cols;
    int64_t z_prev = 0;
#pragma unroll
    for (int d = 0; d < MAXD; ++d) {
        if (d < (int)dpt) {
            int64_t digit;
            if (dpt == 1) digit = static_cast<int64_t>(base) * z[0] + m_digits[0] * z[0] + v_digits[0];
            else if (d == 0) digit = static_cast<int64_t>(base) * z[0] + m_digits[0] * z_last + v_digits[0];
            else if (d < last) digit = static_cast<int64_t>(base) * z[d] - z_prev + m_digits[d] * z_last + v_digits[d];
            else digit = m_digits[d] * z_last - z_prev + v_digits[d];
            z_prev = z[d];
            const size_t orow = r * k + static_cast<size_t>(t) * dpt + d;
            const size_t opoly = orow * src_cols + col;
            for (uint32_t l = 0; l < L; ++l)
                out[(opoly * L + l) * N + i] = signed_to_residue_mu<W>(digit, limbs[l].q, limbs[l].mu64);
        }
    }
}

struct GqTower {
    double c_last, sd;
    KarneyDivisor div;
    double cvec[4];
};

__global__ void gq_tower_kernel(GqTower *__restrict__ towers, const LimbConst *__restrict__ limbs, uint32_t L,
                                uint32_t dpt, uint32_t base_bits, double c) {
    const uint32_t t = blockIdx.x * blockDim.x + threadIdx.x;
    if (t >= L) return;
    const uint64_t base = 1ull << base_bits;
    const double base_f = static_cast<double>(base);
    const double sigma = c / (base_f + 1.0);
    const uint64_t qt = limbs[t].q;
    double c_last = 0.0;
    GqTower g;
    for (uint32_t d = 0; d < 4; ++d) g.cvec[d] = 0.0;
    for (uint32_t d = 0; d < dpt; ++d) {
        c_last = (c_last + static_cast<double>(static_cast<int64_t>((qt >> (base_bits * d)) & (base - 1)))) / base_f;
        if (d < 4) g.cvec[d] = c_last;
    }
    g.c_last = c_last;
    g.sd = sigma / c_last;
    g.div = karney_divisor(g.sd);
    towers[t] = g;
}

struct GqPertConsts {
    double ld[4], hn[4];
};

static inline GqPertConsts gq_pert_consts(uint32_t dpt, uint32_t base_bits) {
    GqPertConsts k{};
    const double base_f = static_cast<double>(1ull << base_bits), kf = static_cast<double>(dpt);
    for (uint32_t d = 0; d < 4 && d < dpt; ++d) {
        k.ld[d] = d == 0 ? sqrt(base_f * (1.0 + 1.0 / kf) + 1.0) : sqrt(base_f * (1.0 + 1.0 / (kf - static_cast<double>(d))));
        k.hn[d] = sqrt(base_f * (1.0 - 1.0 / (kf - static_cast<double>(d))));
    }
    return k;
}

template <typename W, int MAXD, bool SEG = false>
__global__ void __launch_bounds__(256) gauss_samp_prep_kernel(double *__restrict__ a_out, uint64_t *__restrict__ left_out,
                                       const W *__restrict__ src, const LimbConst *__restrict__ limbs,
                                       ChaChaKey key, size_t total, uint32_t L, uint32_t logN,
                                       uint32_t dpt, uint32_t base_bits, double c, GqPertConsts pc,
                                       uint32_t src_cols, SegArg<SEG> segs) {
    static_assert(MAXD <= 4, "GqPertConsts holds four digits");
    const size_t idx = item_index();
    if (idx >= total) return;
    const uint32_t i = static_cast<uint32_t>(idx & ((1u << logN) - 1));
    const uint32_t pt = static_cast<uint32_t>(idx >> logN);
    uint32_t p = pt / L;
    const uint32_t t = pt - p * L;
    if constexpr (SEG) {
        const uint32_t p_u = static_cast<uint32_t>(__builtin_amdgcn_readfirstlane(p));
        const uint32_t row = p_u / src_cols, col = p_u - row * src_cols;
        const uint32_t j = rng_segment_of(segs, col);
        key = segs.key[j];
        p = row * (segs.start[j + 1] - segs.start[j]) + (col - segs.start[j]);
    }
    const uint64_t qt = limbs[t].q;
    uint64_t value = static_cast<uint64_t>(src[idx]);
    if (value >= qt) value %= qt;
    const uint64_t base = 1ull << base_bits;
    const double base_f = static_cast<double>(base);
    const double sigma = c / (base_f + 1.0);

    uint64_t w[8];
    chacha_block_words(key, gadget_stream0(i, t), static_cast<uint64_t>(p) + 1, 0, w);
    double zf[MAXD];
#pragma unroll
    for (int d = 0; d < MAXD; ++d)
        zf[d] = d < (int)dpt ? sigma * (sqrt(-2.0 * det_log(u64_to_open01(w[2 * d]))) * det_cos2pi(u64_to_open01(w[2 * d + 1]))) : 0.0;
#pragma unroll
    for (int j = 0; j < 8; ++j)
        if (j >= 2 * (int)dpt) left_out[static_cast<size_t>(j - 2 * (int)dpt) * total + idx] = w[j];
    double prev_a = 0.0;
#pragma unroll
    for (int d = 0; d < MAXD; ++d) {
        if (d < (int)dpt) {
            double pd;
            if (d + 1 < (int)dpt) pd = pc.ld[d] * zf[d] + pc.hn[d] * zf[d + 1 < MAXD ? d + 1 : d];
            else pd = (d == 0 ? 0.0 : pc.hn[d - 1 < 0 ? 0 : d - 1]) * zf[d];
            const double vd = static_cast<double>(static_cast<int64_t>((value >> (base_bits * d)) & (base - 1)));
            const double ad = (prev_a + vd - pd) / base_f;
            prev_a = ad;
            a_out[static_cast<size_t>(d) * total + idx] = ad;
        }
    }
}

template <typename W, int MAXD, int SV, bool UNI = false, bool SEG = false>
__global__ void __launch_bounds__(SAMPLER_THREADS, 4) gauss_samp_lanes_kernel(int64_t *__restrict__ stage,
                                        const LimbConst *__restrict__ limbs, ChaChaKey key,
                                        const GqTower *__restrict__ towers, const double *__restrict__ a_in,
                                        const uint64_t *__restrict__ left_in, size_t total, uint32_t src_cols,
                                        uint32_t L, uint32_t logN, uint32_t dpt, uint32_t base_bits, double c,
                                        KarneyDivisor div_sigma, uint32_t per_lane, uint32_t fill_every,
                                        SegArg<SEG> segs) {
    static_assert(!SEG || UNI, "segments need a wave's chunk inside one polynomial");
    __shared__ uint32_t ring[SAMPLER_THREADS * RNG_RING_SLOTS];
    const uint64_t base = 1ull << base_bits;
    const double base_f = static_cast<double>(base);
    const double sigma = c / (base_f + 1.0);
    const int last = static_cast<int>(dpt) - 1;
    const uint32_t nleft = 8 - 2 * dpt;
    WaveChunk chunk = wave_chunk(total, per_lane);
    const uint32_t pt_u = static_cast<uint32_t>(__builtin_amdgcn_readfirstlane(static_cast<uint32_t>(chunk.base >> logN)));
    uint32_t p_u = pt_u / L;
    const uint32_t t_u = pt_u - p_u * L;
    const GqTower tw_u = towers[UNI ? t_u : 0];
    if constexpr (SEG) {
        const uint32_t row = p_u / src_cols, col = p_u - row * src_cols;
        const uint32_t j = rng_segment_of(segs, col);
        key = segs.key[j];
        p_u = row * (segs.start[j + 1] - segs.start[j]) + (col - segs.start[j]);
    }

    ChaChaRng rng;
    rng_init_keyed(rng, ring, key, 0, 0, SAMPLER_THREADS);
    KarneyFsm f;
    karney_reset(f);
    bool fin = true, have = false;
    uint32_t ph = 0;
    size_t idx = 0;
    uint32_t tower = 0;
    double a[MAXD];
    int64_t z[MAXD];
    int64_t z_last = 0;
#pragma unroll
    for (int d = 0; d < MAXD; ++d) { a[d] = 0.0; z[d] = 0; }

    auto integer_ready = [&]() {
        if (f.st == KS_DONE && !fin) {
            if (ph == 0) {
                z_last = f.result;
                const double zl = static_cast<double>(z_last);
#pragma unroll
                for (int d = 0; d < MAXD; ++d)
                    if (d < (int)dpt) a[d] += zl * (UNI ? tw_u.cvec[d] : towers[tower].cvec[d]);
            } else {
#pragma unroll
                for (int d = 0; d < MAXD; ++d)
                    if (d == (int)ph - 1) z[d] = f.result;
            }
            ++ph;
            if (ph == dpt) {
                fin = true;
            } else {
                double an = 0.0;
#pragma unroll
                for (int d = 0; d < MAXD; ++d)
                    if (d == (int)ph - 1) an = a[d];
                karney_begin(f, -an, sigma, div_sigma);
            }
        }
    };
    auto element_done = [&]() {
        const bool take = f.st == KS_DONE && fin;
        if (take && have) {
#pragma unroll
            for (int d = 0; d < MAXD; ++d) {
                if (d < (int)dpt) {
                    stage[idx * dpt + d] = d < last ? z[d] : z_last;
                }
            }
        }
        const uint32_t e = wave_take(chunk, take);
        if (take) {
            have = e < chunk.len;
            if (have) {
                idx = chunk.base + e;
                const uint32_t i = static_cast<uint32_t>(idx & ((1u << logN) - 1));
                uint32_t p, t;
                if constexpr (UNI) {
                    p = p_u;
                    t = t_u;
                } else {
                    const uint32_t pt = static_cast<uint32_t>(idx >> logN);
                    p = pt / L;
                    t = pt - p * L;
                }
                tower = t;
                rng_reopen(rng, gadget_stream0(i, t), static_cast<uint64_t>(p) + 1, 1);
                const uint32_t slot0 = (rng.tail >> RNG_DRAW_LOG) & (RNG_RING_SLOTS - 1);
                for (uint32_t w = 0; w < nleft; ++w) {
                    const uint64_t lw = left_in[static_cast<size_t>(w) * total + idx];
                    rng.ring[(slot0 + 4 * dpt + 2 * w) * rng.ring_stride] = static_cast<uint32_t>(lw);
                    rng.ring[(slot0 + 4 * dpt + 2 * w + 1) * rng.ring_stride] = static_cast<uint32_t>(lw >> 32);
                }
                rng.head = rng.tail + 2 * RNG_U64_DRAWS * dpt;
                rng.tail += RNG_BLOCK_DRAWS;
                double a_last = 0.0;
#pragma unroll
                for (int d = 0; d < MAXD; ++d) {
                    if (d < (int)dpt) {
                        a[d] = a_in[static_cast<size_t>(d) * total + idx];
                        a_last = a[d];
                    }
                }
                ph = 0;
                fin = false;
                if constexpr (UNI) {
                    karney_begin(f, -a_last / tw_u.c_last, tw_u.sd, tw_u.div);
                } else {
                    const GqTower tw = towers[t];
                    karney_begin(f, -a_last / tw.c_last, tw.sd, tw.div);
                }
            } else {
                f.st = KS_IDLE;
            }
        }
    };
    for (uint32_t step = 0;; ++step) {
        integer_ready();
        element_done();
        if (__all(f.st == KS_IDLE)) break;
        rng_fill_wave(rng, f.st != KS_IDLE, step % fill_every == 0, 16, karney_urgent(SV));
        karney_heavy(f, rng);
#pragma unroll
        for (int s4 = 0; s4 < KARNEY_SUPERSTEP / SV; ++s4) karney_light(f, rng);
#pragma unroll
        for (int sv = 1; sv < SV; ++sv) {
            integer_ready();
            karney_heavy(f, rng);
#pragma unroll
            for (int s4 = 0; s4 < KARNEY_SUPERSTEP / SV; ++s4) karney_light(f, rng);
        }
    }
}

template <typename W>
__global__ void __launch_bounds__(256) gauss_samp_expand_kernel(W *__restrict__ out, const int64_t *__restrict__ stage,
                                         const W *__restrict__ src, const LimbConst *__restrict__ limbs, size_t total,
                                         uint32_t src_cols, uint32_t L, uint32_t logN, uint32_t dpt, uint32_t k,
                                         uint32_t base_bits) {
    const size_t idx = item_index();
    if (idx >= total) return;
    const uint32_t i = static_cast<uint32_t>(idx & ((1u << logN) - 1));
    const uint32_t pt = static_cast<uint32_t>(idx >> logN);
    const uint32_t p = pt / L, t = pt - p * L;
    const uint32_t r = p / src_cols, col = p - r * src_cols;
    const uint64_t qt = limbs[t].q, base = 1ull << base_bits;
    uint64_t value = static_cast<uint64_t>(src[idx]);
    if (value >= qt) value %= qt;
    const int last = static_cast<int>(dpt) - 1;
    const int64_t z_last = stage[idx * dpt + last];
    int64_t z_prev = 0;
    for (uint32_t d = 0; d < dpt; ++d) {
        const int64_t md = static_cast<int64_t>((qt >> (base_bits * d)) & (base - 1));
        const int64_t vd = static_cast<int64_t>((value >> (base_bits * d)) & (base - 1));
        const int64_t zd = stage[idx * dpt + d];
        int64_t digit;
        if (dpt == 1) digit = static_cast<int64_t>(base) * zd + md * zd + vd;
        else if (d == 0) digit = static_cast<int64_t>(base) * zd + md * z_last + vd;
        else if (static_cast<int>(d) < last) digit = static_cast<int64_t>(base) * zd - z_prev + md * z_last + vd;
        else digit = md * z_last - z_prev + vd;
        z_prev = zd;
        const size_t orow = static_cast<size_t>(r) * k + t * dpt + d;
        W *dst = out + (((orow * src_cols + col) * L) << logN) + i;
        for (uint32_t l = 0; l < L; ++l)
            dst[static_cast<size_t>(l) << logN] = signed_to_residue_mu<W>(digit, limbs[l].q, limbs[l].mu64);
    }
}

template <typename W, int MAXD>
static int launch_gauss_samp_lanes(GpuContext *ctx, W *out, const W *src, size_t total, uint32_t src_cols, uint32_t L,
                                   uint32_t dpt, uint32_t base_bits, double c, size_t k, GpuRngSeed seed,
                                   const RngSegments *segs = nullptr) {
    if ((total >> ctx->logN) >> 32 || k >> 32) return set_error("gpu_matrix_gauss_samp_gq_arb_base: matrix too large");
    CtxBlock stage(ctx), a_buf(ctx), towers(ctx);
    if (towers.alloc(static_cast<size_t>(L) * sizeof(GqTower)) || a_buf.alloc(total * 8 * sizeof(uint64_t)) ||
        stage.alloc(total * dpt * sizeof(int64_t)))
        return 1;
    double *a_words = static_cast<double *>(a_buf.ptr);
    uint64_t *left_words = static_cast<uint64_t *>(a_buf.ptr) + total * dpt;
    const ChaChaKey key = chacha_subkey(seed, 0, kTagGadget);
    MXX_LAUNCH(gq_tower_kernel, dim3(1), dim3(64), 0, ctx->stream, static_cast<GqTower *>(towers.ptr), ctx->d_limbs,
                       L, dpt, base_bits, c);
    MXX_TRACE_BYTES(static_cast<double>(total) * (sizeof(W) + 8.0 * (8 - dpt)));
    if (segs)
        MXX_LAUNCH((gauss_samp_prep_kernel<W, MAXD, true>), item_grid(total, 256), dim3(256), 0,
                           ctx->stream, a_words, left_words, src, ctx->d_limbs, key, total, L,
                           ctx->logN, dpt, base_bits, c, gq_pert_consts(dpt, base_bits), src_cols, *segs);
    else
        MXX_LAUNCH((gauss_samp_prep_kernel<W, MAXD>), item_grid(total, 256), dim3(256), 0,
                           ctx->stream, a_words, left_words, src, ctx->d_limbs, key, total, L,
                           ctx->logN, dpt, base_bits, c, gq_pert_consts(dpt, base_bits), src_cols, NoSegments{});
    const LanePlan plan = lane_plan(total, static_cast<size_t>(ctx->N),
                                    sampler_per_lane(total, reinterpret_cast<const void *>(gauss_samp_lanes_kernel<W, MAXD, KARNEY_SERVICES>), ctx->device, ctx->env.sampler_per_lane),
                                    segs != nullptr, ctx->env.sampler_fill_every, kCadenceGadget, !ctx->env.gsamp_no_uni);
    const double sigma = c / (static_cast<double>(1ull << base_bits) + 1.0);
    MXX_TRACE_BYTES(static_cast<double>(total) * (8.0 * (8 - dpt) + 8.0 * dpt));
    int64_t *digits = static_cast<int64_t *>(stage.ptr);
    const GqTower *d_towers = static_cast<const GqTower *>(towers.ptr);
    const KarneyDivisor div = karney_divisor(sigma);
    if (segs)
        MXX_LAUNCH_LANES(plan, ctx->stream, (gauss_samp_lanes_kernel<W, MAXD, 1, true, true>),
                         (gauss_samp_lanes_kernel<W, MAXD, KARNEY_SERVICES, true, true>), digits, ctx->d_limbs, key, d_towers, a_words,
                         left_words, total, src_cols, L, ctx->logN, dpt, base_bits, c, div, plan.per_lane, plan.fill_every, *segs);
    else
        MXX_LAUNCH_LANES_UNI(plan, ctx->stream, (gauss_samp_lanes_kernel<W, MAXD, 1, true>), (gauss_samp_lanes_kernel<W, MAXD, 1, false>),
                             (gauss_samp_lanes_kernel<W, MAXD, KARNEY_SERVICES, true>), (gauss_samp_lanes_kernel<W, MAXD, KARNEY_SERVICES, false>),
                             digits, ctx->d_limbs, key, d_towers, a_words, left_words, total, src_cols, L, ctx->logN, dpt, base_bits, c, div,
                             plan.per_lane, plan.fill_every, NoSegments{});
    MXX_TRACE_BYTES(static_cast<double>(total) * (8.0 * dpt + sizeof(W) + static_cast<double>(dpt) * L * sizeof(W)));
    MXX_LAUNCH(gauss_samp_expand_kernel<W>, item_grid(total, 256), dim3(256), 0,
                       ctx->stream, out, digits, src, ctx->d_limbs, total, src_cols, L, ctx->logN,
                       dpt, static_cast<uint32_t>(k), base_bits);
    const hipError_t err = hipGetLastError();
    HIP_TRY(err);
    return 0;
}

template <typename W>
static int launch_gauss_samp(GpuContext *ctx, W *out, const W *src, size_t polys, uint32_t src_cols, uint32_t L,
                             uint32_t dpt, uint32_t base_bits, double c, size_t k, GpuRngSeed seed,
                             const RngSegments *segs = nullptr) {
    const size_t total = polys * L * static_cast<size_t>(ctx->N);
    const bool simple = ctx->env.gsamp_simple && !segs;
    if (!simple && dpt <= 2) return launch_gauss_samp_lanes<W, 2>(ctx, out, src, total, src_cols, L, dpt, base_bits, c, k, seed, segs);
    if (!simple && dpt <= 4) return launch_gauss_samp_lanes<W, 4>(ctx, out, src, total, src_cols, L, dpt, base_bits, c, k, seed, segs);
    if (segs) return set_error("gpupoly_matrix_gauss_samp_gq_arb_base_segments: unsupported: more than four digits per tower");
    const dim3 blocks = item_grid(total, 128);
    const uint32_t N = static_cast<uint32_t>(ctx->N);
    MXX_TRACE_BYTES(static_cast<double>(total) * (sizeof(W) + static_cast<double>(dpt) * L * sizeof(W)));
#define LAUNCH_GS(MAXD)                                                                                        \
    MXX_LAUNCH((gauss_samp_gq_kernel<W, MAXD>), dim3(blocks), dim3(128), 0, ctx->stream, out, src,      \
                       ctx->d_limbs, polys, src_cols, L, N, dpt, base_bits, c, k, seed)
    if (dpt <= 2) LAUNCH_GS(2);
    else if (dpt <= 4) LAUNCH_GS(4);
    else if (dpt <= 8) LAUNCH_GS(8);
    else if (dpt <= 20) LAUNCH_GS(20);
    else LAUNCH_GS(64);
#undef LAUNCH_GS
    HIP_TRY(hipGetLastError());
    return 0;
}

static int gauss_samp_impl(GpuMatrix *src, uint32_t base_bits, double c, GpuRngSeed seed, GpuMatrix *out, const RngSegments *segs);

extern "C" int gpu_matrix_gauss_samp_gq_arb_base(GpuMatrix *src, uint32_t base_bits, double c, double dgg_stddev,
                                                 GpuRngSeed seed, GpuMatrix *out) {
    ABI_GUARD_BEGIN
    (void)dgg_stddev;
    return gauss_samp_impl(src, base_bits, c, seed, out, nullptr);
    ABI_GUARD_END
}

extern "C" int gpupoly_matrix_gauss_samp_gq_arb_base_segments(GpuMatrix *src, uint32_t base_bits, double c, double dgg_stddev,
                                                              const GpuRngSeed *seeds, const size_t *seg_cols, size_t nseg,
                                                              GpuMatrix *out) {
    ABI_GUARD_BEGIN
    (void)dgg_stddev;
    if (!src || !out) return set_error("invalid gpupoly_matrix_gauss_samp_gq_arb_base_segments arguments");
    if (static_cast<size_t>(src->ctx->N) % SAMPLER_THREADS)
        return set_error("gpupoly_matrix_gauss_samp_gq_arb_base_segments: unsupported: ring too small for a wave per polynomial chunk");
    RngSegments segs;
    if (!rng_segments_build(segs, seeds, seg_cols, nseg, kTagGadget, src->cols))
        return set_error("gpupoly_matrix_gauss_samp_gq_arb_base_segments: segments must be 1..64, non-empty and cover the source's columns");
    return gauss_samp_impl(src, base_bits, c, GpuRngSeed{}, out, &segs);
    ABI_GUARD_END
}

static int gauss_samp_impl(GpuMatrix *src, uint32_t base_bits, double c, GpuRngSeed seed, GpuMatrix *out, const RngSegments *segs) {
    {
    if (!src || !out) return set_error("invalid gpu_matrix_gauss_samp_gq_arb_base arguments");
    if (base_bits == 0 || base_bits >= 63) return set_error("invalid base_bits in gpu_matrix_gauss_samp_gq_arb_base");
    if (!(c > 0.0)) return set_error("c must be positive in gpu_matrix_gauss_samp_gq_arb_base");
    if (src->ctx != out->ctx || src->level != out->level)
        return set_error("context mismatch in gpu_matrix_gauss_samp_gq_arb_base");
    GpuContext *ctx = src->ctx;
    const int requested = out->format;
    const size_t L = matrix_limbs(src);
    const uint32_t dpt = (ctx->crt_bits + base_bits - 1) / base_bits;
    if (dpt == 0 || dpt > kGaussMaxDigits)
        return set_error("invalid digits_per_tower in gpu_matrix_gauss_samp_gq_arb_base");
    const size_t k = static_cast<size_t>(dpt) * L;
    if (out->rows != src->rows * k || out->cols != src->cols)
        return set_error("output size mismatch in gpu_matrix_gauss_samp_gq_arb_base");
    if (storage_overlaps(src, out)) return set_error("gpu_matrix_gauss_samp_gq_arb_base: output must not alias the source");
    const size_t polys = matrix_polys(src);
    if (polys == 0) {
        out->format = GPU_POLY_FORMAT_EVAL;
        return 0;
    }
    if (ctx_activate(ctx)) return 1;
    if (src->format == GPU_POLY_FORMAT_EVAL) {
        int rc = gpu_matrix_intt_all(src);
        if (rc) return rc;
    }
    int rc = ctx->wide ? launch_gauss_samp<uint64_t>(ctx, static_cast<uint64_t *>(words_ptr(out)),
                                                     static_cast<const uint64_t *>(words_ptr(src)), polys,
                                                     (uint32_t)src->cols, (uint32_t)L, dpt, base_bits, c, k, seed, segs)
                       : launch_gauss_samp<uint32_t>(ctx, static_cast<uint32_t *>(words_ptr(out)),
                                                     static_cast<const uint32_t *>(words_ptr(src)), polys,
                                                     (uint32_t)src->cols, (uint32_t)L, dpt, base_bits, c, k, seed, segs);
    if (rc) return rc;
    out->format = GPU_POLY_FORMAT_COEFF;
    if (requested == GPU_POLY_FORMAT_EVAL) {
        rc = launch_ntt(ctx, words_ptr(out), matrix_polys(out) * L, static_cast<int>(L), false);
        if (rc) return rc;
        out->format = GPU_POLY_FORMAT_EVAL;
    }
    return 0;
    }
}

struct P1KeyedSegments {
    RngSegments segs;
    const P1KeyEntry *keys;
};
template <typename W>
__global__ void p1_covariance_kernel(const W *__restrict__ a_mat, const W *__restrict__ b_mat,
                                     const W *__restrict__ d_mat, uint32_t d, uint32_t L, uint32_t N, uint64_t q0,
                                     double sigma, double s, double dgg_stddev, double *__restrict__ cov_ws,
                                     double *__restrict__ sqrt_var_out, double *__restrict__ update_out) {
    const uint32_t i = blockIdx.x * blockDim.x + threadIdx.x;
    if (i >= N) return;
    const uint32_t m = 2 * d;
    double *cov = cov_ws + static_cast<size_t>(i) * m * m;
    double *sqrt_var = sqrt_var_out + static_cast<size_t>(i) * m;
    double *upd = update_out + static_cast<size_t>(i) * m * m;
    const double sigma2 = sigma * sigma, s2 = s * s, fallback = dgg_stddev * dgg_stddev, eps = 1e-9;
    for (uint32_t r = 0; r < d; ++r)
        for (uint32_t c = 0; c < d; ++c) {
            const size_t rc = (static_cast<size_t>(r) * d + c) * L * N + i;
            const size_t cr = (static_cast<size_t>(c) * d + r) * L * N + i;
            const double a_rc = static_cast<double>(centered_residue(a_mat[rc], q0));
            const double d_rc = static_cast<double>(centered_residue(d_mat[rc], q0));
            const double b_rc = static_cast<double>(centered_residue(b_mat[rc], q0));
            const double b_cr = static_cast<double>(centered_residue(b_mat[cr], q0));
            cov[r * m + c] = -sigma2 * a_rc + (r == c ? s2 : 0.0);
            cov[(r + d) * m + (c + d)] = -sigma2 * d_rc + (r == c ? s2 : 0.0);
            cov[r * m + (c + d)] = -sigma2 * b_rc;
            cov[(r + d) * m + c] = -sigma2 * b_cr;
        }
    for (int t = static_cast<int>(m) - 1; t >= 0; --t) {
        double var = cov[t * m + t];
        if (!(var > eps)) var = fallback;
        sqrt_var[t] = sqrt(var);
        for (int r = 0; r < t; ++r) upd[t * m + r] = cov[r * m + t] / var;
        if (t == 0) break;
        for (int r = 0; r < t; ++r) {
            const double cr = upd[t * m + r];
            for (int c = 0; c <= r; ++c) {
                const double colc = upd[t * m + c] * var;
                const double v = cov[r * m + c] - cr * colc;
                cov[r * m + c] = v;
                cov[c * m + r] = v;
            }
        }
    }
}

template <typename W, int MAXM>
__global__ void __launch_bounds__(128) p1_sample_kernel(W *__restrict__ out, const W *__restrict__ tp2,
                                 const LimbConst *__restrict__ limbs, const double *__restrict__ sqrt_var_base,
                                 const double *__restrict__ update_base, uint32_t m, uint32_t cols, uint32_t L,
                                 uint32_t N, uint64_t q0, double c_scale, GpuRngSeed seed,
                                 double *__restrict__ mean_ws) {
    __shared__ uint32_t ring[128 * RNG_RING_SLOTS];
    const size_t idx = item_index();
    if (idx >= static_cast<size_t>(cols) * N) return;
    const uint32_t col = static_cast<uint32_t>(idx / N);
    const uint32_t i = static_cast<uint32_t>(idx - static_cast<size_t>(col) * N);
    const double *sqrt_var = sqrt_var_base + static_cast<size_t>(i) * m;
    const double *upd = update_base + static_cast<size_t>(i) * m * m;
    ChaChaRng rng;
    rng_init(rng, ring, seed, static_cast<uint64_t>(col) + 1, static_cast<uint64_t>(i) + 1, 0, kTagP1);

    if constexpr (MAXM > 0) {
        double mean[MAXM];
#pragma unroll
        for (int r = 0; r < MAXM; ++r)
            mean[r] = r < (int)m ? c_scale * static_cast<double>(centered_residue(
                                                 tp2[((static_cast<size_t>(r) * cols + col) * L) * N + i], q0))
                                 : 0.0;
#pragma unroll
        for (int t = MAXM - 1; t >= 0; --t) {
            if (t >= (int)m) continue;
            const double mu = mean[t];
            const int64_t z = sample_integer_karney(rng, mu, sqrt_var[t]);
            for (uint32_t l = 0; l < L; ++l)
                out[((static_cast<size_t>(t) * cols + col) * L + l) * N + i] =
                    signed_to_residue_mu<W>(z, limbs[l].q, limbs[l].mu64);
            const double delta = static_cast<double>(z) - mu;
#pragma unroll
            for (int r = 0; r < MAXM; ++r)
                if (r < t) mean[r] += upd[t * m + r] * delta;
        }
    } else {
        double *mean = mean_ws + idx * m;
        for (uint32_t r = 0; r < m; ++r)
            mean[r] = c_scale * static_cast<double>(centered_residue(
                                    tp2[((static_cast<size_t>(r) * cols + col) * L) * N + i], q0));
        for (int t = static_cast<int>(m) - 1; t >= 0; --t) {
            const double mu = mean[t];
            const int64_t z = sample_integer_karney(rng, mu, sqrt_var[t]);
            for (uint32_t l = 0; l < L; ++l)
                out[((static_cast<size_t>(t) * cols + col) * L + l) * N + i] =
                    signed_to_residue_mu<W>(z, limbs[l].q, limbs[l].mu64);
            const double delta = static_cast<double>(z) - mu;
            for (int r = 0; r < t; ++r) mean[r] += upd[t * m + r] * delta;
        }
    }
}

__global__ void p1_divisor_kernel(KarneyDivisor *__restrict__ div, const double *__restrict__ sqrt_var, size_t count) {
    const size_t idx = item_index();
    if (idx < count) div[idx] = karney_divisor(sqrt_var[idx]);
}

template <bool SEG, bool KEYED>
using P1SegArg = typename std::conditional<KEYED, P1KeyedSegments, SegArg<SEG>>::type;
template <typename T>
__device__ __forceinline__ const T *wave_uniform_ptr(const void *p) {
    const uint64_t v = reinterpret_cast<uint64_t>(p);
    const uint32_t lo = __builtin_amdgcn_readfirstlane(static_cast<uint32_t>(v));
    const uint32_t hi = __builtin_amdgcn_readfirstlane(static_cast<uint32_t>(v >> 32));
    return reinterpret_cast<const T *>((static_cast<uint64_t>(hi) << 32) | lo);
}
template <typename W, int MAXM, int SV, bool SEG = false, bool KEYED = false>
__global__ void __launch_bounds__(SAMPLER_THREADS) p1_sample_lanes_kernel(int64_t *__restrict__ stage, const W *__restrict__ tp2,
                                       const double *__restrict__ sqrt_var_base, const double *__restrict__ update_base,
                                       const KarneyDivisor *__restrict__ div_base, uint32_t m, uint32_t cols, uint32_t L,
                                       uint32_t logN, uint64_t q0, double c_scale, ChaChaKey key, size_t total,
                                       uint32_t per_lane, uint32_t fill_every, P1SegArg<SEG, KEYED> segs) {
    static_assert(SEG || !KEYED, "the keyed form is a form of the segment path");
    __shared__ uint32_t ring[SAMPLER_THREADS * RNG_RING_SLOTS];
    WaveChunk chunk = wave_chunk(total, per_lane);
    uint32_t seg_col0 = 0;
    if constexpr (KEYED) {
        const uint32_t col_u = static_cast<uint32_t>(__builtin_amdgcn_readfirstlane(static_cast<uint32_t>(chunk.base >> logN)));
        const uint32_t j = rng_segment_of(segs.segs, col_u < cols ? col_u : cols - 1);
        key = segs.segs.key[j];
        seg_col0 = segs.segs.start[j];
        const P1KeyEntry e = segs.keys[j];
        sqrt_var_base = wave_uniform_ptr<double>(e.sqrt_var);
        update_base = wave_uniform_ptr<double>(e.update_coeff);
        div_base = wave_uniform_ptr<KarneyDivisor>(e.karney_div);
    } else if constexpr (SEG) {
        const uint32_t col_u = static_cast<uint32_t>(__builtin_amdgcn_readfirstlane(static_cast<uint32_t>(chunk.base >> logN)));
        const uint32_t j = rng_segment_of(segs, col_u < cols ? col_u : cols - 1);
        key = segs.key[j];
        seg_col0 = segs.start[j];
    }
    ChaChaRng rng;
    rng_init_keyed(rng, ring, key, 0, 0, SAMPLER_THREADS);
    KarneyFsm f;
    karney_reset(f);
    bool fin = true, have = false;
    uint32_t t = 0, col = 0, i = 0;
    double mean[MAXM], mu = 0.0;
#pragma unroll
    for (int r = 0; r < MAXM; ++r) mean[r] = 0.0;

    auto integer_ready = [&]() {
        if (f.st == KS_DONE && !fin) {
// ... 312 lines not shown
```

mxx_amd/matrix.py:

```python
from __future__ import annotations

import ctypes as C
import os
import threading
import weakref

import numpy as np

from . import _ffi
from ._ffi import GPU_POLY_FORMAT_COEFF, GPU_POLY_FORMAT_EVAL, GpuRngSeed, check_status
from .params import GpuDCRTPolyParams


def mul_decompose_column_chunk_width_is_set() -> bool:
    return bool(os.environ.get("MXX_MUL_DECOMPOSE_COLUMN_CHUNK_WIDTH"))


def mul_decompose_column_chunk_width() -> int:
    try:
        return max(1, int(os.environ.get("MXX_MUL_DECOMPOSE_COLUMN_CHUNK_WIDTH", "1")))
    except ValueError:
        return 1


# ... 1 lines not shown
    if v < 251:
        return bytes([v])
    if v < 1 << 16:
        return bytes([251]) + v.to_bytes(2, "little")
    if v < 1 << 32:
        return bytes([252]) + v.to_bytes(4, "little")
    return bytes([253]) + v.to_bytes(8, "little")


def _bincode_read_varint(data: bytes, pos: int):
    tag = data[pos]
    if tag < 251:
        return tag, pos + 1
    width = {251: 2, 252: 4, 253: 8}[tag]
    return int.from_bytes(data[pos + 1 : pos + 1 + width], "little"), pos + 1 + width


def block_size() -> int:
    try:
        value = int(os.environ.get("BLOCK_SIZE", "100"))
    except ValueError:
        return 100
    return value if value >= 1 else 100


def block_offsets(rng: range, block: int) -> list:
    assert block > 0, "block_offsets: block must be positive"
    offsets, cur = [rng.start], rng.start
    while cur < rng.stop:
        cur = min(cur + block, rng.stop)
        offsets.append(cur)
    return offsets


def rns_bytes_len_for_level(params, level: int) -> int:
    assert level < params.crt_depth(), "invalid RNS byte length level"
    return (level + 1) * params.ring_dimension() * 8


def rns_bytes_len(params) -> int:
    return rns_bytes_len_for_level(params, max(params.crt_depth() - 1, 0))


def one_rns_bytes(params) -> bytes:
    if rns_bytes_len(params) == 0:
        return b""
    one = GpuDCRTPolyMatrix.identity(params, 1)
    return one.to_rns().tobytes()


class GpuDCRTMatrixRnsSnapshot:

    __slots__ = ("_nrow", "_ncol", "_level", "_is_ntt", "_bytes_per_poly", "_bytes")

    def __init__(self, nrow, ncol, level, is_ntt, bytes_per_poly, data):
        self._nrow, self._ncol, self._level, self._is_ntt = int(nrow), int(ncol), int(level), bool(is_ntt)
        self._bytes_per_poly = int(bytes_per_poly)
        self._bytes = bytes(data)

    def nrow(self) -> int:
        return self._nrow

    def ncol(self) -> int:
        return self._ncol

    def level(self) -> int:
        return self._level

    def is_ntt(self) -> bool:
        return self._is_ntt

    def bytes_per_poly(self) -> int:
        return self._bytes_per_poly

    def bytes(self) -> bytes:
        return self._bytes

    def validate_for_params(self, params) -> None:
        assert self._level < params.crt_depth(), "invalid RNS snapshot level"
        assert self._bytes_per_poly == rns_bytes_len_for_level(params, self._level), "RNS snapshot bytes_per_poly mismatch"
        assert len(self._bytes) == self._nrow * self._ncol * self._bytes_per_poly, "RNS snapshot byte length mismatch"

    def __eq__(self, other) -> bool:
        if not isinstance(other, GpuDCRTMatrixRnsSnapshot):
            return NotImplemented
        return all(getattr(self, f) == getattr(other, f) for f in self.__slots__)

    def __repr__(self) -> str:
        return (f"GpuDCRTMatrixRnsSnapshot(nrow={self._nrow}, ncol={self._ncol}, level={self._level}, "
                f"is_ntt={self._is_ntt}, bytes_per_poly={self._bytes_per_poly}, bytes={len(self._bytes)})")


def _bincode_read_nested_bytes(data: bytes) -> list:
    pos = 0
    nrows, pos = _bincode_read_varint(data, pos)
    out = []
    for _ in range(nrows):
        ncols, pos = _bincode_read_varint(data, pos)
        row = []
        for _ in range(ncols):
            blen, pos = _bincode_read_varint(data, pos)
            assert pos + blen <= len(data), "truncated matrix block file"
            row.append(data[pos : pos + blen])
            pos += blen
        out.append(row)
    return out


def _bincode_nested_bytes(entries) -> bytes:
    parts = [_bincode_varint(len(entries))]
    for row in entries:
        parts.append(_bincode_varint(len(row)))
        for e in row:
            parts.append(_bincode_varint(len(e)))
            parts.append(bytes(e))
    return b"".join(parts)


_pinned_tls = threading.local()


def _pinned_capacity() -> int:
    return getattr(_pinned_tls, "size", 0)


def _pinned_buffer(nbytes: int) -> int:
    if _pinned_capacity() < nbytes:
        old = getattr(_pinned_tls, "holder", None)
        if old is not None:
            old.release()
        size = max(nbytes, 1 << 20)
        ptr = _ffi.lib().gpu_pinned_alloc(size)
        if not ptr:
            _pinned_tls.holder, _pinned_tls.size = None, 0
            raise _ffi.GpuPolyError(f"gpu_pinned_alloc({size}) failed: {_ffi.last_error_string()}")
        _pinned_tls.holder, _pinned_tls.size = _PinnedBlock(ptr), size
    return _pinned_tls.holder.ptr


class _PinnedBlock:
    def __init__(self, ptr):
        self.ptr = ptr
        self._fin = weakref.finalize(self, _ffi.lib().gpu_pinned_free, C.c_void_p(ptr))

    def release(self):
        self._fin()


class GpuP1CovarianceCache:
    def __init__(self, raw, params=None):
        self.raw = raw
        self.params = params
        self._finalizer = weakref.finalize(self, _ffi.lib().gpu_matrix_destroy_p1_covariance_cache, raw)


def _max_along(entries, axis, nrow, ncol):
    if isinstance(axis, str):
        if axis != "entries":
            raise ValueError(f"axis must be None, 0, 1 or 'entries' (got {axis!r})")
        return entries
    if axis is None:
        return max((v for row in entries for v in row), default=0)
    if axis == 1:
        return [max(row, default=0) for row in entries]
    if axis == 0:
        return [max((entries[r][c] for r in range(nrow)), default=0) for c in range(ncol)]
    raise ValueError(f"axis must be None, 0, 1 or 'entries' (got {axis!r})")


DEVICE_HASHES = {"keccak256": _ffi.GPUPOLY_HASH_KECCAK256, "keccak_256": _ffi.GPUPOLY_HASH_KECCAK256, "sha3_256": _ffi.GPUPOLY_HASH_SHA3_256}


class IndexedTags:

    __slots__ = ("prefix", "first", "count", "decimal")

    def __init__(self, prefix: bytes, first: int, count: int, decimal: bool = False):
        prefix, first, count = bytes(prefix), int(first), int(count)
        if first < 0 or count < 0 or (count and first + count - 1 >= 1 << 64):
            raise ValueError("IndexedTags: the indices must stay within 64 bits")
        self.prefix, self.first, self.count, self.decimal = prefix, first, count, bool(decimal)

    def __len__(self) -> int:
        return self.count

    def tag(self, t: int) -> bytes:
        idx = self.first + t
        return self.prefix + (str(idx).encode("ascii") if self.decimal else idx.to_bytes(8, "little"))

    def __iter__(self):
        return (self.tag(t) for t in range(self.count))

    def __getitem__(self, item):
        if isinstance(item, slice):
            lo, hi, step = item.indices(self.count)
            if step == 1:
                return IndexedTags(self.prefix, self.first + lo, max(hi - lo, 0), self.decimal)
            return [self.tag(t) for t in range(lo, hi, step)]
        t = item + self.count if item < 0 else item
        if not 0 <= t < self.count:
            raise IndexError("IndexedTags index out of range")
        return self.tag(t)

    def __repr__(self):
        return f"IndexedTags({self.prefix!r}, {self.first}, {self.count}, decimal={self.decimal})"


def hash_tags_arg(key: bytes, tags, hash_name: str = "keccak256"):
    if hash_name not in DEVICE_HASHES:
        raise ValueError(f"no device-side hash {hash_name!r}")
    key = bytes(key)
    assert len(key) == 32
    arg = _ffi.GpuHashTags()
    arg.hash = DEVICE_HASHES[hash_name]
    arg.key[:] = key
    if isinstance(tags, IndexedTags) and len(tags.prefix) <= 64:
        buf = C.create_string_buffer(tags.prefix, max(len(tags.prefix), 1))
        arg.form = _ffi.GPUPOLY_TAGS_INDEXED_DECIMAL if tags.decimal else _ffi.GPUPOLY_TAGS_INDEXED_LE64
        arg.tags = C.cast(buf, C.c_void_p)
        arg.tag_offsets = None
        arg.prefix_len, arg.first_index = len(tags.prefix), tags.first
        return arg, (buf,), len(tags)
    literal = [bytes(t) for t in tags]
    offsets = (C.c_size_t * (len(literal) + 1))()
    at = 0
    for t, tag in enumerate(literal):
        at += len(tag)
        offsets[t + 1] = at
    packed = b"".join(literal)
    buf = C.create_string_buffer(packed, max(len(packed), 1))
    arg.form = _ffi.GPUPOLY_TAGS_TABLE
    arg.tags = C.cast(buf, C.c_void_p)
    arg.tag_offsets = offsets
    return arg, (buf, offsets), len(literal)


def device_hash_seeds(params, key: bytes, tags, hash_name: str = "keccak256") -> list:
    arg, keep, count = hash_tags_arg(key, tags, hash_name)
    if count == 0:
        return []
    seeds = (GpuRngSeed * count)()
    check_status(_ffi.lib().gpupoly_hash_seeds(params.ctx().raw, C.byref(arg), count, seeds), "gpupoly_hash_seeds")
    del keep
    out = []
    for s in seeds:
        c = GpuRngSeed()
        c.words[:] = s.words[:]
        out.append(c)
    return out


class GpuDCRTPolyMatrix:
    __slots__ = ("params", "nrow", "ncol", "level", "is_ntt", "raw", "_finalizer", "_parent", "_version", "__weakref__")

    def __init__(self, params: GpuDCRTPolyParams, nrow: int, ncol: int, level: int, is_ntt: bool):
        if not (0 <= level < params.crt_depth()):
            raise AssertionError("invalid level for matrix create")
        raw = C.c_void_p()
        fmt = GPU_POLY_FORMAT_EVAL if is_ntt else GPU_POLY_FORMAT_COEFF
        st = _ffi.lib().gpu_matrix_create(params.ctx_raw(), level, nrow, ncol, fmt, C.byref(raw))
        check_status(st, f"gpu_matrix_create(nrow={nrow}, ncol={ncol}, level={level}, format={fmt})")
        self.params = params
        self.nrow = nrow
        self.ncol = ncol
        self.level = level
        self.is_ntt = is_ntt
        self.raw = raw
        self._parent = None
        self._version = 0
        self._finalizer = weakref.finalize(self, _ffi.lib().gpu_matrix_destroy, raw)

    @property
    def layout(self) -> str:
        out = C.c_int(-1)
        check_status(_ffi.lib().gpupoly_matrix_layout(self.raw, C.byref(out)), "gpupoly_matrix_layout")
        return "packed24" if out.value == 1 else "words"

    @classmethod
    def new_empty(cls, params, nrow, ncol) -> "GpuDCRTPolyMatrix":
        return cls(params, nrow, ncol, params.crt_depth() - 1, True)

    @classmethod
    def zero(cls, params, nrow, ncol) -> "GpuDCRTPolyMatrix":
        return cls._new_zero_with_state(params, nrow, ncol, params.crt_depth() - 1, True)

    new_zero = zero

    @classmethod
    def _new_zero_with_state(cls, params, nrow, ncol, level, is_ntt) -> "GpuDCRTPolyMatrix":
        out = cls(params, nrow, ncol, level, is_ntt)
        if nrow == 0 or ncol == 0:
            return out
        check_status(_ffi.lib().gpupoly_matrix_fill_zero(out.raw), "gpupoly_matrix_fill_zero")
        return out

    @classmethod
    def from_rns(cls, params, data: np.ndarray, eval_format: bool) -> "GpuDCRTPolyMatrix":
        data = np.ascontiguousarray(data, dtype=np.uint64)
        rows, cols, L, n = data.shape
        if n != params.ring_dimension():
            raise ValueError("ring dimension mismatch")
        out = cls(params, rows, cols, L - 1, eval_format)
        out.load_rns(data, eval_format)
        return out

    @classmethod
# ... 1395 lines not shown
        if isinstance(scalar, (list, tuple)):
            if len(scalar) == 1:
                return int(scalar[0]), None
            assert len(scalar) <= first.params.ring_dimension(), "more coefficients than the ring dimension"
            words = [GpuDCRTPolyMatrix._int_words(c) for c in scalar]
            wpc = max((len(w) for w in words), default=1)
            arr = np.zeros((1, 1, max(len(words), 1), wpc), dtype=np.uint64)
            for i, w in enumerate(words):
                arr[0, 0, i, : len(w)] = w
            return None, GpuDCRTPolyMatrix.from_coeff_words(first.params, arr, True, level=first.level)
        s = scalar.inner if hasattr(scalar, "inner") else scalar
        assert s.size() == (1, 1), "large_scalar_mul: the scalar is a polynomial or a 1 x 1 matrix"
        return None, s

    def large_scalar_mul(self, scalar) -> "GpuDCRTPolyMatrix":
        return GpuDCRTPolyMatrix.large_scalar_mul_many([self], scalar)[0]

    @staticmethod
    def large_scalar_mul_many(lhss, scalar, addends=None, negate: bool = False) -> list:
        lhss = list(lhss)
        n = len(lhss)
        addends = [None] * n if addends is None else list(addends)
        assert len(addends) == n, "large_scalar_mul_many: one addend slot per operand"
        if n == 0:
            return []
        first = lhss[0]
        k = GpuDCRTPolyMatrix._gadget_digits(first.params, first.level, False)
        for l_, a_ in zip(lhss, addends):
            assert l_.params == first.params and l_.level == first.level, "large_scalar_mul_many: one context and level per call"
            assert l_.ncol % k == 0, "large_scalar_mul_many: lhs columns must be a multiple of the digit count"
            assert a_ is None or (a_.nrow, a_.ncol) == (l_.nrow, l_.ncol), "large_scalar_mul_many: addend shape"
        const, sc = GpuDCRTPolyMatrix._large_scalar(first, scalar)
        if mul_decompose_column_chunk_width_is_set():
            outs = []
            for l_, a_ in zip(lhss, addends):
                prod = l_._large_scalar_mul_host(const if sc is None else sc)
                if a_ is None:
                    outs.append(-prod if negate else prod)
                else:
                    outs.append(a_.ensure_eval() - prod if negate else a_.ensure_eval() + prod)
            return outs
        ls = [m.ensure_eval() for m in lhss]
        ads = [None if m is None else m.ensure_eval() for m in addends]
        outs = [GpuDCRTPolyMatrix(first.params, l_.nrow, l_.ncol, l_.level, True) for l_ in ls]
        raw = lambda m: None if m is None else (m.raw.value if hasattr(m.raw, "value") else m.raw)
        arr = lambda ms: (C.c_void_p * n)(*[raw(m) for m in ms])
        base = first.params.base_bits()
        if sc is None:
            words = GpuDCRTPolyMatrix._int_words(const)
            st = _ffi.lib().gpupoly_matrix_mul_decompose_gadget_const_many(
                arr(outs), arr(ls), arr(ads), n, words.ctypes.data_as(C.POINTER(C.c_uint64)), len(words), 1 if negate else 0, base)
            check_status(st, "gpupoly_matrix_mul_decompose_gadget_const_many")
        else:
            st = _ffi.lib().gpupoly_matrix_mul_decompose_gadget_scalar_many(arr(outs), arr(ls), arr(ads), n, sc.raw, 1 if negate else 0, base)
            check_status(st, "gpupoly_matrix_mul_decompose_gadget_scalar_many")
        return outs

    def _large_scalar_mul_host(self, scalar) -> "GpuDCRTPolyMatrix":
        k = self._gadget_digits(self.params, self.level, False)
        assert self.ncol % k == 0
        d = self.ncol // k
        out = GpuDCRTPolyMatrix(self.params, self.nrow, self.ncol, self.level, True)
        if self.nrow == 0 or d == 0:
            return out
        if isinstance(scalar, (int, np.integer)):
            words = self._int_words(scalar).reshape(1, 1, 1, -1)
            scalar = GpuDCRTPolyMatrix.from_coeff_words(self.params, words, True, level=self.level)
        s = (scalar.inner if hasattr(scalar, "inner") else scalar).ensure_eval()
        g = GpuDCRTPolyMatrix(self.params, d, d * k, self.level, True)
        check_status(_ffi.lib().gpu_matrix_fill_gadget(g.raw, self.params.base_bits()), "gpu_matrix_fill_gadget")
        gs = GpuDCRTPolyMatrix(self.params, d, d * k, self.level, True)
        check_status(_ffi.lib().gpu_matrix_mul_scalar(gs.raw, g.raw, s.raw), "gpu_matrix_mul_scalar")
        lhs = self.ensure_eval()
        st = _ffi.lib().gpupoly_matrix_mul_decompose(out.raw, lhs.raw, gs.raw, self.params.base_bits())
        check_status(st, "gpupoly_matrix_mul_decompose")
        return out

    def mul_decompose_small(self, other) -> "GpuDCRTPolyMatrix":
        k = -(-self.params.crt_bits() // self.params.base_bits())
        assert self.ncol == other.nrow * k
        ncol = other.ncol
        out = GpuDCRTPolyMatrix.new_empty(self.params, self.nrow, ncol)
        if self.nrow == 0 or ncol == 0:
            return out
        if not mul_decompose_column_chunk_width_is_set():
            lhs = self.ensure_eval()
            st = _ffi.lib().gpupoly_matrix_mul_decompose_small(out.raw, lhs.raw, other.raw, self.params.base_bits())
            check_status(st, "gpupoly_matrix_mul_decompose_small")
            return out
        width = min(mul_decompose_column_chunk_width(), ncol)
        for c0 in range(0, ncol, width):
            c1 = min(c0 + width, ncol)
            dec = other.slice(0, other.nrow, c0, c1).small_decompose_owned()
            prod = self._mul_internal(dec)
            out.copy_block_from(prod, 0, c0, 0, 0, self.nrow, c1 - c0)
        return out

    @classmethod
    def sample_distribution(cls, params, nrow, ncol, dist: int, sigma: float, seed: GpuRngSeed):
        out = cls.new_empty(params, nrow, ncol)
        if nrow == 0 or ncol == 0:
            return out
        check_status(_ffi.lib().gpu_matrix_sample_distribution(out.raw, dist, sigma, seed), "gpu_matrix_sample_distribution")
        return out

    @classmethod
    def sample_distribution_columns(cls, params, nrow, total_ncol, col_start, col_len, dist, sigma, seed):
        assert col_start + col_len <= total_ncol, "sample_distribution_columns range out of bounds"
        out = cls.new_empty(params, nrow, col_len)
        if nrow == 0 or col_len == 0:
            return out
        st = _ffi.lib().gpu_matrix_sample_distribution_columns(out.raw, dist, sigma, seed, total_ncol, col_start)
        check_status(st, "gpu_matrix_sample_distribution_columns")
        return out

    @classmethod
    def sample_distribution_decomposed(cls, params, nrow, ncol, dist: int, sigma: float, seed: GpuRngSeed, small=False):
        k = -(-params.crt_bits() // params.base_bits()) if small else params.modulus_digits()
        out = cls.new_empty(params, nrow * k, ncol)
        if nrow == 0 or ncol == 0:
            return out
        st = _ffi.lib().gpupoly_matrix_sample_decomposed(out.raw, dist, sigma, seed, params.base_bits(), 1 if small else 0)
        check_status(st, "gpupoly_matrix_sample_decomposed")
        return out

    @classmethod
    def sample_distribution_decomposed_window(cls, params, nrow, total_ncol, col_start, col_len, dist: int, sigma: float,
                                              seed: GpuRngSeed, small=False, row_start=0, row_end=None, is_ntt=True,
                                              level=None):
        assert col_start + col_len <= total_ncol, "sample_distribution_decomposed_window column range out of bounds"
        level = params.crt_depth() - 1 if level is None else level
        dpt = -(-params.crt_bits() // params.base_bits())
        k = dpt if small else dpt * (level + 1)
        if row_end is None:
            row_end = nrow * k
        assert 0 <= row_start <= row_end <= nrow * k, f"sample_distribution_decomposed_window rows [{row_start}, {row_end}) out of range: {nrow * k} digit rows"
        out = cls(params, row_end - row_start, col_len, level, is_ntt)
        st = _ffi.lib().gpupoly_matrix_sample_decomposed_window(out.raw, dist, sigma, seed, params.base_bits(), 1 if small else 0,
                                                                nrow, total_ncol, col_start, row_start)
        check_status(st, "gpupoly_matrix_sample_decomposed_window")
        if row_end == row_start or col_len == 0:
            out.is_ntt = True
        return out

    def gauss_samp_gq_arb_base(self, c: float, dgg_stddev: float, seed: GpuRngSeed, coeff_out: bool = False) -> "GpuDCRTPolyMatrix":
        out = GpuDCRTPolyMatrix(self.params, self.nrow * self.params.modulus_digits(), self.ncol, self.params.crt_depth() - 1,
                                not coeff_out)
        self.intt_all_in_place()
        self._touch()
        st = _ffi.lib().gpu_matrix_gauss_samp_gq_arb_base(self.raw, self.params.base_bits(), c, dgg_stddev, seed, out.raw)
        check_status(st, "gpu_matrix_gauss_samp_gq_arb_base")
        return out

    @staticmethod
    def create_p1_covariance_cache(a_mat, b_mat, d_mat, sigma, s, dgg_stddev) -> GpuP1CovarianceCache:
        raw = C.c_void_p()
        st = _ffi.lib().gpu_matrix_create_p1_covariance_cache(a_mat.raw, b_mat.raw, d_mat.raw, sigma, s, dgg_stddev, C.byref(raw))
        check_status(st, "gpu_matrix_create_p1_covariance_cache")
        return GpuP1CovarianceCache(raw, a_mat.params)

    @staticmethod
    def sample_p1_full_cached(cache: GpuP1CovarianceCache, tp2, seed: GpuRngSeed) -> "GpuDCRTPolyMatrix":
        out = GpuDCRTPolyMatrix.new_empty(tp2.params, tp2.nrow, tp2.ncol)
        if tp2.nrow == 0 or tp2.ncol == 0:
            return out
        tp2.intt_all_in_place()
        check_status(_ffi.lib().gpu_matrix_sample_p1_full_cached(cache.raw, tp2.raw, seed, out.raw), "gpu_matrix_sample_p1_full_cached")
        return out

    @staticmethod
    def _segment_args(seeds, seg_cols):
        assert len(seeds) == len(seg_cols) and seeds, "one seed per segment"
        return (GpuRngSeed * len(seeds))(*seeds), (C.c_size_t * len(seg_cols))(*seg_cols), len(seeds)

    @classmethod
    def sample_distribution_segments(cls, params, nrow, seg_cols, dist: int, sigma: float, seeds) -> "GpuDCRTPolyMatrix":
        out = cls.new_empty(params, nrow, sum(seg_cols))
        arr, cols, n = cls._segment_args(seeds, seg_cols)
        check_status(_ffi.lib().gpupoly_matrix_sample_distribution_segments(out.raw, dist, sigma, arr, cols, n),
                     "gpupoly_matrix_sample_distribution_segments")
        return out

    @classmethod
    def sample_distribution_blocks(cls, params, seeds, dist: int, *, block_polys=None, nrow=None, seg_cols=None) -> "GpuDCRTPolyMatrix":
        seeds = list(seeds)
        level = params.crt_depth() - 1
        arr = (GpuRngSeed * max(len(seeds), 1))(*seeds)
        if seg_cols is None:
            assert block_polys is not None and nrow is None, "sample_distribution_blocks: block_polys (stacked) or nrow and seg_cols (columns)"
            out = cls(params, len(seeds), block_polys, level, True)
            layout, cols = _ffi.GPUPOLY_BLOCKS_STACKED, None
        else:
            assert block_polys is None and nrow is not None, "sample_distribution_blocks: block_polys (stacked) or nrow and seg_cols (columns)"
            seg_cols = list(seg_cols)
            assert len(seg_cols) == len(seeds), "sample_distribution_blocks: one seed per block"
            out = cls(params, nrow, sum(seg_cols), level, True)
            layout, cols = _ffi.GPUPOLY_BLOCKS_COLUMNS, (C.c_size_t * max(len(seg_cols), 1))(*seg_cols)
        check_status(_ffi.lib().gpupoly_matrix_sample_distribution_blocks(out.raw, dist, arr, len(seeds), layout, cols),
                     "gpupoly_matrix_sample_distribution_blocks")
        return out

    @classmethod
    def sample_hash_blocks(cls, params, key: bytes, tags, dist: int, *, hash_name: str = "keccak256", block_polys=None, nrow=None,
                           seg_cols=None) -> "GpuDCRTPolyMatrix":
        arg, keep, count = hash_tags_arg(key, tags, hash_name)
        level = params.crt_depth() - 1
        if seg_cols is None:
            assert block_polys is not None and nrow is None, "sample_hash_blocks: block_polys (stacked) or nrow and seg_cols (columns)"
            out = cls(params, count, block_polys, level, True)
            layout, cols = _ffi.GPUPOLY_BLOCKS_STACKED, None
        else:
            assert block_polys is None and nrow is not None, "sample_hash_blocks: block_polys (stacked) or nrow and seg_cols (columns)"
            seg_cols = list(seg_cols)
            assert len(seg_cols) == count, "sample_hash_blocks: one tag per block"
            out = cls(params, nrow, sum(seg_cols), level, True)
            layout, cols = _ffi.GPUPOLY_BLOCKS_COLUMNS, (C.c_size_t * max(len(seg_cols), 1))(*seg_cols)
        check_status(_ffi.lib().gpupoly_matrix_sample_hash_blocks(out.raw, dist, C.byref(arg), count, layout, cols),
                     "gpupoly_matrix_sample_hash_blocks")
        del keep
        return out

    @classmethod
    def _blocks_out(cls, who, params, count, block_polys, nrow, seg_cols):
        level = params.crt_depth() - 1
        if seg_cols is None:
            assert block_polys is not None and nrow is None, f"{who}: block_polys (stacked) or nrow and seg_cols (columns)"
            return cls(params, count, block_polys, level, True), _ffi.GPUPOLY_BLOCKS_STACKED, None
        assert block_polys is None and nrow is not None, f"{who}: block_polys (stacked) or nrow and seg_cols (columns)"
        seg_cols = list(seg_cols)
        assert len(seg_cols) == count, f"{who}: one seed or tag per block"
        return cls(params, nrow, sum(seg_cols), level, True), _ffi.GPUPOLY_BLOCKS_COLUMNS, (C.c_size_t * max(len(seg_cols), 1))(*seg_cols)

    @classmethod
    def sample_gauss_blocks(cls, params, seeds, sigma: float, *, block_polys=None, nrow=None, seg_cols=None) -> "GpuDCRTPolyMatrix":
        seeds = list(seeds)
        arr = (GpuRngSeed * max(len(seeds), 1))(*seeds)
        out, layout, cols = cls._blocks_out("sample_gauss_blocks", params, len(seeds), block_polys, nrow, seg_cols)
        check_status(_ffi.lib().gpupoly_matrix_sample_gauss_blocks(out.raw, float(sigma), arr, len(seeds), layout, cols),
                     "gpupoly_matrix_sample_gauss_blocks")
        return out

    @classmethod
    def sample_hash_gauss_blocks(cls, params, key: bytes, tags, sigma: float, *, hash_name: str = "keccak256", block_polys=None,
                                 nrow=None, seg_cols=None) -> "GpuDCRTPolyMatrix":
        arg, keep, count = hash_tags_arg(key, tags, hash_name)
        out, layout, cols = cls._blocks_out("sample_hash_gauss_blocks", params, count, block_polys, nrow, seg_cols)
        check_status(_ffi.lib().gpupoly_matrix_sample_hash_gauss_blocks(out.raw, float(sigma), C.byref(arg), count, layout, cols),
                     "gpupoly_matrix_sample_hash_gauss_blocks")
        del keep
        return out

    @classmethod
    def _decomposed_blocks_out(cls, params, nblk, nrow, col_len, small, is_ntt, level):
        level = params.crt_depth() - 1 if level is None else level
        dpt = -(-params.crt_bits() // params.base_bits())
        k = dpt if small else dpt * (level + 1)
        return cls(params, nrow * k, nblk * col_len, level, is_ntt)

    @classmethod
    def sample_decomposed_blocks(cls, params, seeds, nrow, total_ncol, col_start, col_len, dist: int, small=False, is_ntt=True,
                                 level=None) -> "GpuDCRTPolyMatrix":
        seeds = list(seeds)
        out = cls._decomposed_blocks_out(params, len(seeds), nrow, col_len, small, is_ntt, level)
        arr = (GpuRngSeed * max(len(seeds), 1))(*seeds)
        st = _ffi.lib().gpupoly_matrix_sample_decomposed_blocks(out.raw, dist, arr, len(seeds), params.base_bits(), 1 if small else 0, nrow,
                                                                total_ncol, col_start)
        check_status(st, "gpupoly_matrix_sample_decomposed_blocks")
        if out.nrow == 0 or out.ncol == 0:
            out.is_ntt = True
        return out

    @classmethod
    def sample_hash_decomposed_blocks(cls, params, key: bytes, tags, nrow, total_ncol, col_start, col_len, dist: int, small=False,
                                      is_ntt=True, level=None, hash_name: str = "keccak256") -> "GpuDCRTPolyMatrix":
        arg, keep, count = hash_tags_arg(key, tags, hash_name)
        out = cls._decomposed_blocks_out(params, count, nrow, col_len, small, is_ntt, level)
        st = _ffi.lib().gpupoly_matrix_sample_hash_decomposed_blocks(out.raw, dist, C.byref(arg), count, params.base_bits(), 1 if small else 0,
                                                                     nrow, total_ncol, col_start)
        check_status(st, "gpupoly_matrix_sample_hash_decomposed_blocks")
        del keep
        if out.nrow == 0 or out.ncol == 0:
            out.is_ntt = True
        return out

    @staticmethod
    def _int_rows(values):
        words = [GpuDCRTPolyMatrix._int_words(v) for v in values]
        arr = np.zeros((len(words), max(len(w) for w in words)), dtype=np.uint64)
        for t, w in enumerate(words):
            arr[t, : len(w)] = w
        return arr, arr.shape[1]

    @staticmethod
    def _wee25_call(entry: str, t_bottom, nparts, secret_size, idxs, args) -> list:
        p = t_bottom.params
        outs = [GpuDCRTPolyMatrix(p, secret_size, t_bottom.nrow, t_bottom.level, True) for _ in range(len(idxs) * nparts)]
        if outs:
            i_arr = np.array(idxs, dtype=np.uint64)
            st = getattr(_ffi.lib(), entry)(GpuDCRTPolyMatrix._raw_array(outs), len(idxs), nparts, *args(i_arr.ctypes.data_as(C.POINTER(C.c_uint64))))
            check_status(st, entry)
        return [outs[t * nparts:(t + 1) * nparts] for t in range(len(idxs))]

    @staticmethod
    def lut_targets(w_identity, w_gy, w_v, w_vx, col_start, col_len, ys, idxs, key: bytes, tags, hash_name: str = "keccak256") -> list:
        ys, idxs = [int(y) for y in ys], [int(i) for i in idxs]
        arg, keep, count = hash_tags_arg(key, tags, hash_name)
# ... 121 lines not shown
```

mxx_amd/trapdoor.py:

```python
from __future__ import annotations

import math
import threading
import weakref

from .matrix import GpuDCRTPolyMatrix
from .sampler import DistType, GpuDCRTPolyUniformSampler, random_gpu_rng_seed, sample_gpu_matrix_with_seed

SPECTRAL_CONSTANT = 1.8


def preimage_c(base: int, sigma: float) -> float:
    return (base + 1.0) * sigma


def preimage_smoothing_parameter(base: int, sigma: float, d: int, n: int, k: int) -> float:
    return SPECTRAL_CONSTANT * (base + 1.0) * sigma * sigma * (math.sqrt(d * n * k) + math.sqrt(2 * n) + 4.7)


def p1_covariance_parameters(params, d: int, dgg_stddev: float):
    base = 1 << params.base_bits()
    n, k = params.ring_dimension(), params.modulus_digits()
    return preimage_c(base, dgg_stddev), preimage_smoothing_parameter(base, dgg_stddev, d, n, k), dgg_stddev


def compute_preimage_norm(ring_dim_sqrt: float, m_g: int, base: float, b_nrow=None, sigma=None) -> float:
    sigma = 4.578 if sigma is None else sigma
    b_nrow = 1 if b_nrow is None else b_nrow
    term = math.sqrt(b_nrow) * ring_dim_sqrt * math.sqrt(m_g) + math.sqrt(2.0) * ring_dim_sqrt + 4.7
    return 1.8 * 6.5 * sigma * ((base + 1.0) * sigma) * term


def _coeff_cached(m: GpuDCRTPolyMatrix) -> GpuDCRTPolyMatrix:
    return m.clone().into_coeff_domain()


coeff_cached_matrix = _coeff_cached


class GpuPerturbationSamples:

    __slots__ = ("p1", "p2")

    def __init__(self, p1, p2):
        self.p1, self.p2 = p1, p2

    def __iter__(self):
        return iter((self.p1, self.p2))


class GpuDCRTTrapdoor:

    def __init__(self, r: GpuDCRTPolyMatrix, e: GpuDCRTPolyMatrix):
        self.r = r
        self.e = e
        self.re = r.concat_rows([e])
        rt, et = r.transpose(), e.transpose()
        self.a_mat_coeff = _coeff_cached(r * rt)
        self.b_mat_coeff = _coeff_cached(r * et)
        self.d_mat_coeff = _coeff_cached(e * et)
        self._p1_cache = None
        self._p1_lock = threading.Lock()
        self._stacked = None
        self._replicas = {}

    @classmethod
    def new(cls, params, size: int, sigma: float) -> "GpuDCRTTrapdoor":
        u = GpuDCRTPolyUniformSampler()
        k = params.modulus_digits()
        dist = DistType.GaussDist(sigma)
        return cls(u.sample_uniform(params, size, size * k, dist), u.sample_uniform(params, size, size * k, dist))

    def p1_covariance_cache(self, c: float, s: float, dgg_stddev: float):
        with self._p1_lock:
            if self._p1_cache is not None and self._p1_cache[0] == (c, s, dgg_stddev):
                return self._p1_cache[1]
            cache = GpuDCRTPolyMatrix.create_p1_covariance_cache(
                self.a_mat_coeff, self.b_mat_coeff, self.d_mat_coeff, c, s, dgg_stddev
            )
            self._p1_cache = ((c, s, dgg_stddev), cache)
            return cache

    get_or_create_p1_covariance_cache = p1_covariance_cache

    def public_matrix_parts(self, public_matrix: GpuDCRTPolyMatrix):
        with self._p1_lock:
            if self._stacked is not None and self._stacked[0]() is public_matrix and self._stacked[2] == public_matrix.content_version():
                return self._stacked[1]
            d, p1_rows, p2_rows = public_matrix.row_size(), self.re.row_size(), self.re.col_size()
            left = public_matrix.slice(0, d, 0, p1_rows)
            right = public_matrix.slice(0, d, p1_rows, p1_rows + p2_rows)
            parts = (left, right, self.re.concat_rows([right]))
            self._stacked = (weakref.ref(public_matrix), parts, public_matrix.content_version())
            return parts

    def clear_public_matrix_cache(self) -> None:
        with self._p1_lock:
            self._stacked = None
            self._replicas = {}

    def replica_for(self, params, public_matrix: GpuDCRTPolyMatrix):
        key = params.ctx_raw().value
        with self._p1_lock:
            hit = self._replicas.get(key)
            if hit is not None and hit[2]() is public_matrix and hit[3] == public_matrix.content_version():
                return hit[0], hit[1]
        td, a = self.to_params(params), public_matrix.to_params(params)
        with self._p1_lock:
            self._replicas[key] = (td, a, weakref.ref(public_matrix), public_matrix.content_version())
        return td, a

    def to_params(self, params) -> "GpuDCRTTrapdoor":
        return GpuDCRTTrapdoor(self.r.to_params(params), self.e.to_params(params))

    def to_compact_bytes(self) -> bytes:
        out = b""
        for m in (self.r, self.e):
            b = m.to_compact_bytes()
            out += len(b).to_bytes(8, "little") + b
        return out

    @classmethod
    def from_compact_bytes(cls, params, data: bytes):
        mats, off = [], 0
        for _ in range(2):
            if off + 8 > len(data):
                return None
            ln = int.from_bytes(data[off : off + 8], "little")
            off += 8
            if off + ln > len(data):
                return None
            mats.append(GpuDCRTPolyMatrix.from_compact_bytes(params, data[off : off + ln]))
            off += ln
        if off != len(data):
            return None
        return cls(mats[0], mats[1])

    def __eq__(self, other):
        return isinstance(other, GpuDCRTTrapdoor) and self.r == other.r and self.e == other.e

    __hash__ = None


WORKER_DNUM = 0x5700
_worker_params_cache: dict = {}
_worker_params_lock = threading.Lock()


def preimage_workers() -> int:
    import os

    try:
        return max(1, min(8, int(os.environ.get("MXX_PREIMAGE_WORKERS", "4"))))
    except ValueError:
        return 4


def worker_params(params, k: int):
    from .params import GpuDCRTPolyParams

    key = (params.ctx_raw().value, k)
    with _worker_params_lock:
        for dead in [kk for kk, (owner, _) in _worker_params_cache.items() if owner() is None]:
            del _worker_params_cache[dead]
        hit = _worker_params_cache.get(key)
        if hit is not None and hit[0]() is params.ctx():
            return hit[1]
        pw = GpuDCRTPolyParams(params.ring_dimension(), params.moduli(), params.base_bits(), gpu_ids=params.gpu_ids(), dnum=WORKER_DNUM + k)
        _worker_params_cache[key] = (weakref.ref(params.ctx()), pw)
        return pw


TRAFFIC_BOUND_BYTES = 32 << 20


def _traffic_bound(params, polys: int) -> bool:
    word = 4 if max(params.moduli()) < (1 << 31) else 8
    return polys * params.crt_depth() * params.ring_dimension() * word >= TRAFFIC_BOUND_BYTES


class GpuDCRTPolyTrapdoorSampler:
    def __init__(self, params, sigma: float):
        self.sigma = float(sigma)
        self.base = 1 << params.base_bits()
        self.c = preimage_c(self.base, self.sigma)

    @staticmethod
    def trapdoor_to_bytes(trapdoor: "GpuDCRTTrapdoor") -> bytes:
        return trapdoor.to_compact_bytes()

    @staticmethod
    def trapdoor_from_bytes(params, data: bytes):
        return GpuDCRTTrapdoor.from_compact_bytes(params, data)

    def trapdoor(self, params, size: int):
        u = GpuDCRTPolyUniformSampler()
        td = GpuDCRTTrapdoor.new(params, size, self.sigma)
        a_bar = u.sample_uniform(params, size, size, DistType.FinRingDist())
        g = GpuDCRTPolyMatrix.gadget_matrix(params, size)
        a0 = a_bar.concat_columns([GpuDCRTPolyMatrix.identity(params, size)])
        a1 = g - (a_bar * td.r + td.e)
        return td, a0.concat_columns([a1])

    def _sample_pert(self, params, td: GpuDCRTTrapdoor, s, c, dgg_stddev, sigma_large, total_ncol):
        return self._sample_pert_parts(params, td, s, c, dgg_stddev, sigma_large, total_ncol)[:2]

    def sample_pert_square_mat_gpu_native_parts(self, params, td, s, c, dgg_stddev, sigma_large, total_ncol):
        return GpuPerturbationSamples(*self._sample_pert(params, td, s, c, dgg_stddev, sigma_large, total_ncol))

    def sample_pert_square_mat_gpu_native(self, params, td, s, c, dgg_stddev, sigma_large, total_ncol):
        p1, p2 = self._sample_pert(params, td, s, c, dgg_stddev, sigma_large, total_ncol)
        assert p1.col_size() >= total_ncol and p2.col_size() >= total_ncol, "p1 / p2 must include the target columns"
        p_hat = GpuDCRTPolyMatrix(params, p1.row_size() + p2.row_size(), total_ncol, p1.level, p1.is_ntt)
        p_hat.copy_block_from(p1, 0, 0, 0, 0, p1.row_size(), total_ncol)
        p_hat.copy_block_from(p2, p1.row_size(), 0, 0, 0, p2.row_size(), total_ncol)
        return p_hat

    @staticmethod
    def _draw_seeds():
        return random_gpu_rng_seed(), random_gpu_rng_seed(), random_gpu_rng_seed()

    def _sample_pert_parts(self, params, td: GpuDCRTTrapdoor, s, c, dgg_stddev, sigma_large, total_ncol, stacked=None, seeds=None):
        d, dk = td.r.row_size(), td.r.col_size()
        padded = -(-total_ncol // d) * d
        seed_p2 = seeds[0] if seeds is not None else random_gpu_rng_seed()
        p2 = sample_gpu_matrix_with_seed(params, dk, padded, DistType.GaussDist(sigma_large), seed_p2)
        rp2 = tp2_eval = None
        if stacked is not None and _traffic_bound(params, dk * padded):
            t = stacked * p2
            re_rows = td.re.row_size()
            tp2 = t.slice(0, re_rows, 0, padded)
            tp2_eval = t.row_view(0, re_rows)
            rp2 = t.row_view(re_rows, t.row_size())
        else:
            tp2 = td.re * p2
            if _traffic_bound(params, dk * padded):
                tp2_eval = tp2.clone()
        cache = td.p1_covariance_cache(c, s, dgg_stddev)
        p1 = GpuDCRTPolyMatrix.sample_p1_full_cached(cache, tp2, seeds[1] if seeds is not None else random_gpu_rng_seed())
        return p1, p2, tp2_eval, rp2

    def preimage(self, params, td: GpuDCRTTrapdoor, public_matrix, target, _seeds=None) -> GpuDCRTPolyMatrix:
        d = public_matrix.row_size()
        target_cols = target.col_size()
        assert target.row_size() == d, "Target matrix should have the same number of rows as the public matrix"
        n, k = params.ring_dimension(), params.modulus_digits()
        s = preimage_smoothing_parameter(self.base, self.sigma, d, n, k)
        dgg_large_std = math.sqrt(s * s - self.c * self.c)
        p1_rows, p2_rows = td.re.row_size(), td.re.col_size()
        assert public_matrix.col_size() == p1_rows + p2_rows, "public matrix columns must match perturbation rows"
        left, right, stacked = td.public_matrix_parts(public_matrix)
        p1, p2, tp2, rp2 = self._sample_pert_parts(params, td, s, self.c, self.sigma, dgg_large_std, target_cols, stacked, _seeds)
        seed_z = _seeds[2] if _seeds is not None else None
        assert (p1.row_size(), p2.row_size()) == (p1_rows, p2_rows)
        p_hat_image = (left * p1) + (rp2 if rp2 is not None else right * p2)
        if p_hat_image.col_size() != target_cols:
            p_hat_image = p_hat_image.slice_columns(0, target_cols)
        perturbed = target - p_hat_image
        out = GpuDCRTPolyMatrix(params, p1_rows + p2_rows, target_cols, p1.level, p1.is_ntt)
        if p1.col_size() == target_cols and tp2 is not None:
            z = perturbed.gauss_samp_gq_arb_base(self.c, self.sigma, seed_z if seed_z is not None else random_gpu_rng_seed(), coeff_out=True)
            out.ntt_add_rows_from(p1_rows, z, p2, consume=True)
            re_x = td.re * out.row_view(p1_rows, p1_rows + p2_rows)
            out.add_rows_from(0, p1 - tp2, re_x)
            return out
        z_hat = perturbed.gauss_samp_gq_arb_base(self.c, self.sigma, seed_z if seed_z is not None else random_gpu_rng_seed())
        re_z = td.re * z_hat
        if p1.col_size() == target_cols:
            out.add_rows_from(0, p1, re_z)
            out.add_rows_from(p1_rows, p2, z_hat)
            return out
        out.copy_block_from(p1, 0, 0, 0, 0, p1_rows, target_cols)
        out.copy_block_from(p2, p1_rows, 0, 0, 0, p2_rows, target_cols)
        out.add_block_from(re_z, 0, 0, 0, 0, re_z.row_size(), target_cols)
        out.add_block_from(z_hat, 2 * d, 0, 0, 0, z_hat.row_size(), target_cols)
        return out

    def preimage_reference_sequence(self, params, td: GpuDCRTTrapdoor, public_matrix, target) -> GpuDCRTPolyMatrix:
        d = public_matrix.row_size()
        target_cols = target.col_size()
        assert target.row_size() == d, "Target matrix should have the same number of rows as the public matrix"
        n, k = params.ring_dimension(), params.modulus_digits()
        s = preimage_smoothing_parameter(self.base, self.sigma, d, n, k)
        dgg_large_std = math.sqrt(s * s - self.c * self.c)
        u = GpuDCRTPolyUniformSampler()
        dd, dk = td.r.row_size(), td.r.col_size()
        padded = -(-target_cols // dd) * dd
        p2 = u.sample_uniform(params, dk, padded, DistType.GaussDist(dgg_large_std))
        tp2 = td.r.concat_rows([td.e]) * p2
        cache = td.p1_covariance_cache(self.c, s, self.sigma)
        p1 = GpuDCRTPolyMatrix.sample_p1_full_cached(cache, tp2, random_gpu_rng_seed())
        p1_rows, p2_rows = p1.row_size(), p2.row_size()
        assert public_matrix.col_size() == p1_rows + p2_rows, "public matrix columns must match perturbation rows"
        public_left = public_matrix.slice(0, d, 0, p1_rows)
        public_right = public_matrix.slice(0, d, p1_rows, p1_rows + p2_rows)
        p_hat_image = (public_left * p1) + (public_right * p2)
        if p_hat_image.col_size() != target_cols:
            p_hat_image = p_hat_image.slice_columns(0, target_cols)
        perturbed = target - p_hat_image
        z_hat = perturbed.gauss_samp_gq_arb_base(self.c, self.sigma, random_gpu_rng_seed())
        r_z = td.r * z_hat
        out = GpuDCRTPolyMatrix(params, p1_rows + p2_rows, target_cols, p1.level, p1.is_ntt)
        out.copy_block_from(p1, 0, 0, 0, 0, p1_rows, target_cols)
        out.copy_block_from(p2, p1_rows, 0, 0, 0, p2_rows, target_cols)
        del p1, p2
        out.add_block_from(r_z, 0, 0, 0, 0, r_z.row_size(), target_cols)
        del r_z
        e_z = td.e * z_hat
        out.add_block_from(e_z, d, 0, 0, 0, e_z.row_size(), target_cols)
        del e_z
        out.add_block_from(z_hat, 2 * d, 0, 0, 0, z_hat.row_size(), target_cols)
        return out

    def preimage_extend(self, params, td, public_matrix, ext_matrix, target) -> GpuDCRTPolyMatrix:
        d = public_matrix.row_size()
        n, k = params.ring_dimension(), params.modulus_digits()
        s = preimage_smoothing_parameter(self.base, self.sigma, d, n, k)
        u = GpuDCRTPolyUniformSampler()
        right = u.sample_uniform(params, ext_matrix.col_size(), target.col_size(), DistType.GaussDist(s))
        t = target - (ext_matrix * right)
        left = self.preimage(params, td, public_matrix, t)
        return left.concat_rows([right])

    BATCH_BYTES = 1 << 30

    @staticmethod
    def _segments_supported(params, td: GpuDCRTTrapdoor) -> bool:
        import os

        dpt = -(-params.crt_bits() // params.base_bits())
        return (params.ring_dimension() % 128 == 0 and td.r.row_size() <= 4 and dpt <= 4
                and not os.environ.get("MXX_HIP_RNG_COMPAT", "").startswith("r")
                and not os.environ.get("MXX_HIP_P1", "").startswith("s")
                and os.environ.get("MXX_PREIMAGE_BATCH", "1") != "0")

    def preimage_many(self, params, td: GpuDCRTTrapdoor, public_matrix, targets, _seeds=None) -> list:
        targets = list(targets)
        seeds = list(_seeds) if _seeds is not None else [self._draw_seeds() for _ in targets]
        results = [None] * len(targets)
        dd, dk = td.r.row_size(), td.r.col_size()
        word = 4 if max(params.moduli()) < (1 << 31) else 8
        poly_bytes = params.crt_depth() * params.ring_dimension() * word
        batchable = []
        for j, t in enumerate(targets):
            pad = -(-t.col_size() // dd) * dd
            if t.col_size() == 0 or _traffic_bound(params, dk * pad) or not self._segments_supported(params, td):
                results[j] = self.preimage(params, td, public_matrix, t, _seeds=seeds[j])
            else:
                batchable.append(j)
        while batchable:
            group, size = [], 0
            while batchable and len(group) < 64:
                j = batchable[0]
                pad = -(-targets[j].col_size() // dd) * dd
                if group and size + dk * pad * poly_bytes > self.BATCH_BYTES:
                    break
                group.append(batchable.pop(0))
                size += dk * pad * poly_bytes
            if len(group) == 1:
                results[group[0]] = self.preimage(params, td, public_matrix, targets[group[0]], _seeds=seeds[group[0]])
                continue
            for j, x in zip(group, self._preimage_segments(params, td, public_matrix, [targets[j] for j in group], [seeds[j] for j in group])):
                results[j] = x
        return results

    @staticmethod
    def _drop_padding(m, cols, pads):
        if cols == pads:
            return m
        widths = []
        for c, p_ in zip(cols, pads):
            widths += [c, p_ - c]
        parts = m.split_columns(widths)
        return GpuDCRTPolyMatrix.concat_columns_of(parts[0::2])

    def _preimage_segments(self, params, td: GpuDCRTTrapdoor, public_matrix, targets, seeds) -> list:
        M = GpuDCRTPolyMatrix
        d = public_matrix.row_size()
        dd, dk = td.r.row_size(), td.r.col_size()
        cols = [t.col_size() for t in targets]
        pads = [-(-c // dd) * dd for c in cols]
        for t in targets:
            assert t.row_size() == d, "Target matrix should have the same number of rows as the public matrix"
        n, k = params.ring_dimension(), params.modulus_digits()
        s = preimage_smoothing_parameter(self.base, self.sigma, d, n, k)
        dgg_large_std = math.sqrt(s * s - self.c * self.c)
        p1_rows, p2_rows = td.re.row_size(), td.re.col_size()
        assert public_matrix.col_size() == p1_rows + p2_rows, "public matrix columns must match perturbation rows"
        left, right, _ = td.public_matrix_parts(public_matrix)
        gauss = DistType.GaussDist(dgg_large_std)
        p2_pad = M.sample_distribution_segments(params, dk, pads, gauss.as_ffi(), gauss.sigma, [sd[0] for sd in seeds])
        tp2 = td.re * p2_pad
        cache = td.p1_covariance_cache(self.c, s, self.sigma)
        p1_pad = M.sample_p1_full_cached_segments(cache, tp2, [sd[1] for sd in seeds], pads)
        p1, p2 = self._drop_padding(p1_pad, cols, pads), self._drop_padding(p2_pad, cols, pads)
        perturbed = M.concat_columns_of(targets) - ((left * p1) + (right * p2))
        z_hat = perturbed.gauss_samp_gq_arb_base_segments(self.c, self.sigma, [sd[2] for sd in seeds], cols)
        re_z = td.re * z_hat
        out = M(params, p1_rows + p2_rows, sum(cols), p1.level, True)
        out.add_rows_from(0, p1, re_z)
        out.add_rows_from(p1_rows, p2, z_hat)
        return out.split_columns(cols)

    def preimage_many_abi(self, params, td: GpuDCRTTrapdoor, public_matrix, targets, _seeds=None) -> list:
        from . import _ffi

        targets = list(targets)
        seeds = list(_seeds) if _seeds is not None else [self._draw_seeds() for _ in targets]
        if not targets:
            return []
        d = public_matrix.row_size()
        n, k = params.ring_dimension(), params.modulus_digits()
        s = preimage_smoothing_parameter(self.base, self.sigma, d, n, k)
        cache = td.p1_covariance_cache(self.c, s, self.sigma)
        rows = td.re.row_size() + td.re.col_size()
        outs = [GpuDCRTPolyMatrix(params, rows, t.col_size(), public_matrix.level, True) for t in targets]
        flat = (_ffi.GpuRngSeed * (3 * len(seeds)))(*[x for triple in seeds for x in triple])
        raw = GpuDCRTPolyMatrix._raw_array
        st = _ffi.lib().gpupoly_trapdoor_preimage_many(td.re.raw, cache.raw, public_matrix.raw, params.base_bits(),
                                                       raw(targets), len(targets), flat, raw(outs))
        if st != 0:
            msg = _ffi.last_error_string()
            if "unsupported" in msg:
                return [self.preimage(params, td, public_matrix, t, _seeds=sd) for t, sd in zip(targets, seeds)]
            raise _ffi.GpuPolyError(f"gpupoly_trapdoor_preimage_many failed: {msg}")
        return outs

    keyed_calls = 0
# ... 111 lines not shown
```

Measured before the change: 8.269 million.

## Hoist gadget-sampler normal generation onto a low-priority side stream overlapping p1 sampling

Splits the gauss_samp prep kernel into a target-independent normals kernel (ChaCha plus Box-Muller perturbation draws) and a centres kernel that needs the perturbed target. The normals kernel is launched on a new low-priority side stream before p1 sampling, so it can overlap with the perturbation sampling and matrix products, and the main stream joins on an event before the final lane sampling. This adds a side stream, an event pool, a prepared-handle API and an extra pass over the a-buffer, and it changes memory lifetime because the buffer is held across the p1 stage.

```diff
diff --git a/include/gpupoly.h b/include/gpupoly.h
--- a/include/gpupoly.h
+++ b/include/gpupoly.h
@@ -13,6 +13,7 @@
 typedef struct GpuEventSet GpuEventSet;
 typedef struct GpuP1CovarianceCache GpuP1CovarianceCache;
 typedef struct GpuComm GpuComm;
+typedef struct GpuGaussSampPrepared GpuGaussSampPrepared;
 
 typedef struct GpuRngSeed {
     uint64_t words[4];
@@ -170,6 +171,10 @@
 int gpupoly_matrix_gauss_samp_gq_arb_base_segments(GpuMatrix *src, uint32_t base_bits, double c, double dgg_stddev,
                                                    const GpuRngSeed *seeds, const size_t *seg_cols, size_t nseg,
                                                    GpuMatrix *out);
+int gpupoly_gauss_samp_prepare(const GpuMatrix *shape_of, uint32_t base_bits, double c, GpuRngSeed seed,
+                               GpuGaussSampPrepared **out);
+int gpupoly_matrix_gauss_samp_gq_arb_base_prepared(GpuMatrix *src, GpuGaussSampPrepared *prep, GpuMatrix *out);
+void gpupoly_gauss_samp_prepared_destroy(GpuGaussSampPrepared *prep);
 #define GPUPOLY_BLOCKS_STACKED 0
 #define GPUPOLY_BLOCKS_COLUMNS 1
 int gpupoly_matrix_sample_distribution_blocks(GpuMatrix *out, int dist_type, const GpuRngSeed *seeds, size_t nblk,
diff --git a/mxx_amd/__init__.py b/mxx_amd/__init__.py
--- a/mxx_amd/__init__.py
+++ b/mxx_amd/__init__.py
@@ -14,6 +14,7 @@
 from .matrix import (
     GpuDCRTMatrixRnsSnapshot,
     GpuDCRTPolyMatrix,
+    GpuGaussSampPrepared,
     GpuP1CovarianceCache,
     block_offsets,
     block_size,
diff --git a/mxx_amd/_ffi.py b/mxx_amd/_ffi.py
--- a/mxx_amd/_ffi.py
+++ b/mxx_amd/_ffi.py
@@ -167,7 +167,10 @@
                                             C.POINTER(C.c_void_p), _sz, C.c_uint32, C.POINTER(C.c_uint64), _sz, _vp]),
     "gpupoly_matrix_sample_p1_full_cached_segments":(C.c_int, [_vp, _vp, C.POINTER(GpuRngSeed), C.POINTER(_sz), _sz, _vp]),
     "gpupoly_matrix_gauss_samp_gq_arb_base_segments": (C.c_int, [_vp, C.c_uint32, C.c_double, C.c_double, C.POINTER(GpuRngSeed), C.POINTER(_sz), _sz, _vp]),
-    "gpupoly_matrix_concat_columns": (C.c_int, [_vp, C.POINTER(C.c_void_p), _sz]),
+    "gpupoly_gauss_samp_prepare": (C.c_int, [_vp, C.c_uint32, C.c_double, GpuRngSeed, C.POINTER(_vp)]),
+    "gpupoly_matrix_gauss_samp_gq_arb_base_prepared": (C.c_int, [_vp, _vp, _vp]),
+    "gpupoly_gauss_samp_prepared_destroy": (None, [_vp]),
+    "gpupoly_matrix_concat_columns":(C.c_int, [_vp, C.POINTER(C.c_void_p), _sz]),
     "gpupoly_matrix_split_columns": (C.c_int, [_vp, C.POINTER(C.c_void_p), _sz]),
     "gpupoly_trapdoor_preimage_many": (C.c_int, [_vp, _vp, _vp, C.c_uint32, C.POINTER(C.c_void_p), _sz, C.POINTER(GpuRngSeed), C.POINTER(C.c_void_p)]),
     "gpupoly_trapdoor_preimage_keyed": (C.c_int, [C.POINTER(C.c_void_p), C.POINTER(C.c_void_p), C.POINTER(C.c_void_p), _sz, C.c_uint32,
diff --git a/mxx_amd/csrc/common.h b/mxx_amd/csrc/common.h
--- a/mxx_amd/csrc/common.h
+++ b/mxx_amd/csrc/common.h
@@ -38,6 +38,7 @@
     int matmul_tile = 0;
     bool gsamp_simple = false;
     bool gsamp_no_uni = false;
+    bool gsamp_hoist = true;
     bool p1_simple = false;
     int sampler_per_lane = 0;
     int sampler_fill_every = 0;
@@ -71,6 +72,9 @@
     uint32_t crt_bits = 0;
     std::vector<uint64_t> moduli;
     hipStream_t stream = nullptr;
+    hipStream_t side_stream = nullptr;
+    std::vector<hipEvent_t> side_events;
+    std::mutex side_mutex;
     LimbConst *d_limbs = nullptr;
     LimbConst *d_limbs_r = nullptr;
     void *d_tw_fwd = nullptr;
@@ -288,6 +292,11 @@
 bool ctx_is_registered(const GpuContext *ctx);
 int ctx_alloc(GpuContext *ctx, size_t bytes, void **out);
 void ctx_free(GpuContext *ctx, void *ptr);
+int ctx_side_stream(GpuContext *ctx, hipStream_t *out);
+hipEvent_t ctx_event_take(GpuContext *ctx);
+void ctx_event_return(GpuContext *ctx, hipEvent_t ev);
+int ctx_side_fork(GpuContext *ctx, hipStream_t *side);
+int ctx_side_join(GpuContext *ctx, hipEvent_t done);
 struct CtxBlock {
     GpuContext *ctx;
     void *ptr = nullptr;
diff --git a/mxx_amd/csrc/runtime.hip b/mxx_amd/csrc/runtime.hip
--- a/mxx_amd/csrc/runtime.hip
+++ b/mxx_amd/csrc/runtime.hip
@@ -257,6 +257,7 @@
         gsamp_simple = e[0] == 's';
         gsamp_no_uni = e[0] == 'n';
     }
+    if (const char *e = std::getenv("MXX_HIP_GSAMP_HOIST")) gsamp_hoist = e[0] != '0';
     if (const char *e = std::getenv("MXX_HIP_P1")) p1_simple = e[0] == 's';
     if (const char *e = std::getenv("MXX_HIP_NTT64")) ntt64_int = e[0] == 'i';
     if (const char *e = std::getenv("MXX_HIP_RNG_COMPAT")) rng_compat = e[0] == 'r';
@@ -381,6 +382,57 @@
     ctx->free_blocks.emplace(size, ptr);
     ctx->cached_bytes += size;
     cache_trim(ctx, ctx->cache_limit);
+}
+
+int ctx_side_stream(GpuContext *ctx, hipStream_t *out) {
+    std::lock_guard<std::mutex> lk(ctx->side_mutex);
+    if (!ctx->side_stream) {
+        int least = 0, greatest = 0;
+        HIP_TRY(hipDeviceGetStreamPriorityRange(&least, &greatest));
+        HIP_TRY(hipStreamCreateWithPriority(&ctx->side_stream, hipStreamNonBlocking, least));
+    }
+    *out = ctx->side_stream;
+    return 0;
+}
+
+hipEvent_t ctx_event_take(GpuContext *ctx) {
+    {
+        std::lock_guard<std::mutex> lk(ctx->side_mutex);
+        if (!ctx->side_events.empty()) {
+            hipEvent_t ev = ctx->side_events.back();
+            ctx->side_events.pop_back();
+            return ev;
+        }
+    }
+    hipEvent_t ev = nullptr;
+    const hipError_t e = hipEventCreateWithFlags(&ev, hipEventDisableTiming);
+    if (e != hipSuccess) {
+        set_error(e, "hipEventCreateWithFlags");
+        return nullptr;
+    }
+    return ev;
+}
+
+void ctx_event_return(GpuContext *ctx, hipEvent_t ev) {
+    if (!ev) return;
+    std::lock_guard<std::mutex> lk(ctx->side_mutex);
+    ctx->side_events.push_back(ev);
+}
+
+int ctx_side_fork(GpuContext *ctx, hipStream_t *side) {
+    if (ctx_side_stream(ctx, side)) return 1;
+    hipEvent_t ev = ctx_event_take(ctx);
+    if (!ev) return 1;
+    hipError_t e = hipEventRecord(ev, ctx->stream);
+    if (e == hipSuccess) e = hipStreamWaitEvent(*side, ev, 0);
+    ctx_event_return(ctx, ev);
+    if (e != hipSuccess) return set_error(e, "side stream fork");
+    return 0;
+}
+
+int ctx_side_join(GpuContext *ctx, hipEvent_t done) {
+    HIP_TRY(hipStreamWaitEvent(ctx->stream, done, 0));
+    return 0;
 }
 
 template <typename W>
@@ -466,6 +518,11 @@
     }
     (void)hipSetDevice(ctx->device);
     if (ctx->stream) (void)hipStreamSynchronize(ctx->stream);
+    if (ctx->side_stream) {
+        (void)hipStreamSynchronize(ctx->side_stream);
+        (void)hipStreamDestroy(ctx->side_stream);
+    }
+    for (hipEvent_t ev : ctx->side_events) (void)hipEventDestroy(ev);
     for (auto &kv : ctx->free_blocks) (void)hipFree(kv.second);
     for (auto &kv : ctx->live_blocks) (void)hipFree(kv.first);
     if (ctx->d_limbs) (void)hipFree(ctx->d_limbs);
diff --git a/mxx_amd/csrc/trapdoor.hip b/mxx_amd/csrc/trapdoor.hip
--- a/mxx_amd/csrc/trapdoor.hip
+++ b/mxx_amd/csrc/trapdoor.hip
@@ -168,13 +168,50 @@
     return k;
 }
 
+template <int MAXD>
+__device__ __forceinline__ void gq_normals(const ChaChaKey &key, uint32_t i, uint32_t t, uint32_t p, uint32_t dpt,
+                                           uint32_t base_bits, double c, const GqPertConsts &pc, uint64_t (&w)[8],
+                                           double (&pd)[MAXD]) {
+    static_assert(MAXD <= 4, "GqPertConsts holds four digits");
+    const double base_f = static_cast<double>(1ull << base_bits);
+    const double sigma = c / (base_f + 1.0);
+    chacha_block_words(key, gadget_stream0(i, t), static_cast<uint64_t>(p) + 1, 0, w);
+    double zf[MAXD];
+#pragma unroll
+    for (int d = 0; d < MAXD; ++d)
+        zf[d] = d < (int)dpt ? sigma * (sqrt(-2.0 * det_log(u64_to_open01(w[2 * d]))) * det_cos2pi(u64_to_open01(w[2 * d + 1]))) : 0.0;
+#pragma unroll
+    for (int d = 0; d < MAXD; ++d) {
+        if (d + 1 < (int)dpt) pd[d] = pc.ld[d] * zf[d] + pc.hn[d] * zf[d + 1 < MAXD ? d + 1 : d];
+        else pd[d] = (d == 0 ? 0.0 : pc.hn[d - 1 < 0 ? 0 : d - 1]) * zf[d];
+    }
+}
+
+template <typename W, int MAXD, typename Store>
+__device__ __forceinline__ void gq_centres(W word, uint64_t qt, uint32_t dpt, uint32_t base_bits, const double (&pd)[MAXD],
+                                           Store store) {
+    uint64_t value = static_cast<uint64_t>(word);
+    if (value >= qt) value %= qt;
+    const uint64_t base = 1ull << base_bits;
+    const double base_f = static_cast<double>(base);
+    double prev_a = 0.0;
+#pragma unroll
+    for (int d = 0; d < MAXD; ++d) {
+        if (d < (int)dpt) {
+            const double vd = static_cast<double>(static_cast<int64_t>((value >> (base_bits * d)) & (base - 1)));
+            const double ad = (prev_a + vd - pd[d]) / base_f;
+            prev_a = ad;
+            store(d, ad);
+        }
+    }
+}
+
 template <typename W, int MAXD, bool SEG = false>
 __global__ void __launch_bounds__(256) gauss_samp_prep_kernel(double *__restrict__ a_out, uint64_t *__restrict__ left_out,
                                        const W *__restrict__ src, const LimbConst *__restrict__ limbs,
                                        ChaChaKey key, size_t total, uint32_t L, uint32_t logN,
                                        uint32_t dpt, uint32_t base_bits, double c, GqPertConsts pc,
                                        uint32_t src_cols, SegArg<SEG> segs) {
-    static_assert(MAXD <= 4, "GqPertConsts holds four digits");
     const size_t idx = item_index();
     if (idx >= total) return;
     const uint32_t i = static_cast<uint32_t>(idx & ((1u << logN) - 1));
@@ -189,34 +226,50 @@
         p = row * (segs.start[j + 1] - segs.start[j]) + (col - segs.start[j]);
     }
     const uint64_t qt = limbs[t].q;
-    uint64_t value = static_cast<uint64_t>(src[idx]);
-    if (value >= qt) value %= qt;
-    const uint64_t base = 1ull << base_bits;
-    const double base_f = static_cast<double>(base);
-    const double sigma = c / (base_f + 1.0);
-
+    const W word = src[idx];
     uint64_t w[8];
-    chacha_block_words(key, gadget_stream0(i, t), static_cast<uint64_t>(p) + 1, 0, w);
-    double zf[MAXD];
-#pragma unroll
-    for (int d = 0; d < MAXD; ++d)
-        zf[d] = d < (int)dpt ? sigma * (sqrt(-2.0 * det_log(u64_to_open01(w[2 * d]))) * det_cos2pi(u64_to_open01(w[2 * d + 1]))) : 0.0;
+    double pd[MAXD];
+    gq_normals<MAXD>(key, i, t, p, dpt, base_bits, c, pc, w, pd);
 #pragma unroll
     for (int j = 0; j < 8; ++j)
         if (j >= 2 * (int)dpt) left_out[static_cast<size_t>(j - 2 * (int)dpt) * total + idx] = w[j];
-    double prev_a = 0.0;
-#pragma unroll
-    for (int d = 0; d < MAXD; ++d) {
-        if (d < (int)dpt) {
-            double pd;
-            if (d + 1 < (int)dpt) pd = pc.ld[d] * zf[d] + pc.hn[d] * zf[d + 1 < MAXD ? d + 1 : d];
-            else pd = (d == 0 ? 0.0 : pc.hn[d - 1 < 0 ? 0 : d - 1]) * zf[d];
-            const double vd = static_cast<double>(static_cast<int64_t>((value >> (base_bits * d)) & (base - 1)));
-            const double ad = (prev_a + vd - pd) / base_f;
-            prev_a = ad;
-            a_out[static_cast<size_t>(d) * total + idx] = ad;
-        }
-    }
+    gq_centres<W, MAXD>(word, qt, dpt, base_bits, pd, [&](int d, double ad) { a_out[static_cast<size_t>(d) * total + idx] = ad; });
+}
+
+template <int MAXD>
+__global__ void __launch_bounds__(256) gauss_samp_normals_kernel(double *__restrict__ pd_out, uint64_t *__restrict__ left_out,
+                                          ChaChaKey key, size_t total, uint32_t L, uint32_t logN, uint32_t dpt,
+                                          uint32_t base_bits, double c, GqPertConsts pc) {
+    const size_t idx = item_index();
+    if (idx >= total) return;
+    const uint32_t i = static_cast<uint32_t>(idx & ((1u << logN) - 1));
+    const uint32_t pt = static_cast<uint32_t>(idx >> logN);
+    const uint32_t p = pt / L;
+    const uint32_t t = pt - p * L;
+    uint64_t w[8];
+    double pd[MAXD];
+    gq_normals<MAXD>(key, i, t, p, dpt, base_bits, c, pc, w, pd);
+#pragma unroll
+    for (int j = 0; j < 8; ++j)
+        if (j >= 2 * (int)dpt) left_out[static_cast<size_t>(j - 2 * (int)dpt) * total + idx] = w[j];
+#pragma unroll
+    for (int d = 0; d < MAXD; ++d)
+        if (d < (int)dpt) pd_out[static_cast<size_t>(d) * total + idx] = pd[d];
+}
+
+template <typename W, int MAXD>
+__global__ void __launch_bounds__(256) gauss_samp_centres_kernel(double *__restrict__ a_io, const W *__restrict__ src,
+                                          const LimbConst *__restrict__ limbs, size_t total, uint32_t L, uint32_t logN,
+                                          uint32_t dpt, uint32_t base_bits) {
+    const size_t idx = item_index();
+    if (idx >= total) return;
+    const uint32_t pt = static_cast<uint32_t>(idx >> logN);
+    const uint32_t t = pt - (pt / L) * L;
+    double pd[MAXD];
+#pragma unroll
+    for (int d = 0; d < MAXD; ++d) pd[d] = d < (int)dpt ? a_io[static_cast<size_t>(d) * total + idx] : 0.0;
+    gq_centres<W, MAXD>(src[idx], limbs[t].q, dpt, base_bits, pd,
+                        [&](int d, double ad) { a_io[static_cast<size_t>(d) * total + idx] = ad; });
 }
 
 template <typename W, int MAXD, int SV, bool UNI = false, bool SEG = false>
@@ -394,35 +447,18 @@
 }
 
 template <typename W, int MAXD>
-static int launch_gauss_samp_lanes(GpuContext *ctx, W *out, const W *src, size_t total, uint32_t src_cols, uint32_t L,
-                                   uint32_t dpt, uint32_t base_bits, double c, size_t k, GpuRngSeed seed,
-                                   const RngSegments *segs = nullptr) {
-    if ((total >> ctx->logN) >> 32 || k >> 32) return set_error("gpu_matrix_gauss_samp_gq_arb_base: matrix too large");
-    CtxBlock stage(ctx), a_buf(ctx), towers(ctx);
-    if (towers.alloc(static_cast<size_t>(L) * sizeof(GqTower)) || a_buf.alloc(total * 8 * sizeof(uint64_t)) ||
-        stage.alloc(total * dpt * sizeof(int64_t)))
-        return 1;
-    double *a_words = static_cast<double *>(a_buf.ptr);
-    uint64_t *left_words = static_cast<uint64_t *>(a_buf.ptr) + total * dpt;
-    const ChaChaKey key = chacha_subkey(seed, 0, kTagGadget);
-    MXX_LAUNCH(gq_tower_kernel, dim3(1), dim3(64), 0, ctx->stream, static_cast<GqTower *>(towers.ptr), ctx->d_limbs,
-                       L, dpt, base_bits, c);
-    MXX_TRACE_BYTES(static_cast<double>(total) * (sizeof(W) + 8.0 * (8 - dpt)));
-    if (segs)
-        MXX_LAUNCH((gauss_samp_prep_kernel<W, MAXD, true>), item_grid(total, 256), dim3(256), 0,
-                           ctx->stream, a_words, left_words, src, ctx->d_limbs, key, total, L,
-                           ctx->logN, dpt, base_bits, c, gq_pert_consts(dpt, base_bits), src_cols, *segs);
-    else
-        MXX_LAUNCH((gauss_samp_prep_kernel<W, MAXD>), item_grid(total, 256), dim3(256), 0,
-                           ctx->stream, a_words, left_words, src, ctx->d_limbs, key, total, L,
-                           ctx->logN, dpt, base_bits, c, gq_pert_consts(dpt, base_bits), src_cols, NoSegments{});
+static int launch_gauss_samp_lanes_finish(GpuContext *ctx, W *out, const W *src, size_t total, uint32_t src_cols, uint32_t L,
+                                          uint32_t dpt, uint32_t base_bits, double c, size_t k, const ChaChaKey &key,
+                                          const GqTower *d_towers, const double *a_words, const RngSegments *segs) {
+    CtxBlock stage(ctx);
+    if (stage.alloc(total * dpt * sizeof(int64_t))) return 1;
+    const uint64_t *left_words = reinterpret_cast<const uint64_t *>(a_words) + total * dpt;
     const LanePlan plan = lane_plan(total, static_cast<size_t>(ctx->N),
                                     sampler_per_lane(total, reinterpret_cast<const void *>(gauss_samp_lanes_kernel<W, MAXD, KARNEY_SERVICES>), ctx->device, ctx->env.sampler_per_lane),
                                     segs != nullptr, ctx->env.sampler_fill_every, kCadenceGadget, !ctx->env.gsamp_no_uni);
     const double sigma = c / (static_cast<double>(1ull << base_bits) + 1.0);
     MXX_TRACE_BYTES(static_cast<double>(total) * (8.0 * (8 - dpt) + 8.0 * dpt));
     int64_t *digits = static_cast<int64_t *>(stage.ptr);
-    const GqTower *d_towers = static_cast<const GqTower *>(towers.ptr);
     const KarneyDivisor div = karney_divisor(sigma);
     if (segs)
         MXX_LAUNCH_LANES(plan, ctx->stream, (gauss_samp_lanes_kernel<W, MAXD, 1, true, true>),
@@ -440,6 +476,31 @@
     const hipError_t err = hipGetLastError();
     HIP_TRY(err);
     return 0;
+}
+
+template <typename W, int MAXD>
+static int launch_gauss_samp_lanes(GpuContext *ctx, W *out, const W *src, size_t total, uint32_t src_cols, uint32_t L,
+                                   uint32_t dpt, uint32_t base_bits, double c, size_t k, GpuRngSeed seed,
+                                   const RngSegments *segs = nullptr) {
+    if ((total >> ctx->logN) >> 32 || k >> 32) return set_error("gpu_matrix_gauss_samp_gq_arb_base: matrix too large");
+    CtxBlock a_buf(ctx), towers(ctx);
+    if (towers.alloc(static_cast<size_t>(L) * sizeof(GqTower)) || a_buf.alloc(total * 8 * sizeof(uint64_t))) return 1;
+    double *a_words = static_cast<double *>(a_buf.ptr);
+    uint64_t *left_words = static_cast<uint64_t *>(a_buf.ptr) + total * dpt;
+    const ChaChaKey key = chacha_subkey(seed, 0, kTagGadget);
+    MXX_LAUNCH(gq_tower_kernel, dim3(1), dim3(64), 0, ctx->stream, static_cast<GqTower *>(towers.ptr), ctx->d_limbs,
+                       L, dpt, base_bits, c);
+    MXX_TRACE_BYTES(static_cast<double>(total) * (sizeof(W) + 8.0 * (8 - dpt)));
+    if (segs)
+        MXX_LAUNCH((gauss_samp_prep_kernel<W, MAXD, true>), item_grid(total, 256), dim3(256), 0,
+                           ctx->stream, a_words, left_words, src, ctx->d_limbs, key, total, L,
+                           ctx->logN, dpt, base_bits, c, gq_pert_consts(dpt, base_bits), src_cols, *segs);
+    else
+        MXX_LAUNCH((gauss_samp_prep_kernel<W, MAXD>), item_grid(total, 256), dim3(256), 0,
+                           ctx->stream, a_words, left_words, src, ctx->d_limbs, key, total, L,
+                           ctx->logN, dpt, base_bits, c, gq_pert_consts(dpt, base_bits), src_cols, NoSegments{});
+    return launch_gauss_samp_lanes_finish<W, MAXD>(ctx, out, src, total, src_cols, L, dpt, base_bits, c, k, key,
+                                                   static_cast<const GqTower *>(towers.ptr), a_words, segs);
 }
 
 template <typename W>
@@ -534,6 +595,155 @@
     }
     return 0;
     }
+}
+
+struct GpuGaussSampPrepared {
+    GpuContext *ctx = nullptr;
+    int level = 0;
+    size_t rows = 0, cols = 0;
+    uint32_t base_bits = 0, dpt = 0;
+    double c = 0;
+    ChaChaKey key;
+    void *towers = nullptr;
+    void *a_buf = nullptr;
+    hipEvent_t done = nullptr;
+};
+
+static void gauss_samp_prepared_release(GpuGaussSampPrepared *prep) {
+    GpuContext *ctx = prep->ctx;
+    (void)hipSetDevice(ctx->device);
+    if (hipStreamWaitEvent(ctx->stream, prep->done, 0) != hipSuccess) {
+        (void)hipGetLastError();
+        (void)hipEventSynchronize(prep->done);
+    }
+    ctx_free(ctx, prep->a_buf);
+    ctx_free(ctx, prep->towers);
+    ctx_event_return(ctx, prep->done);
+    delete prep;
+}
+
+extern "C" int gpupoly_gauss_samp_prepare(const GpuMatrix *shape_of, uint32_t base_bits, double c, GpuRngSeed seed,
+                                          GpuGaussSampPrepared **out) {
+    ABI_GUARD_BEGIN
+    if (!out) return set_error("invalid gpupoly_gauss_samp_prepare arguments");
+    *out = nullptr;
+    if (!shape_of) return set_error("invalid gpupoly_gauss_samp_prepare arguments");
+    if (base_bits == 0 || base_bits >= 63) return set_error("invalid base_bits in gpupoly_gauss_samp_prepare");
+    if (!(c > 0.0)) return set_error("c must be positive in gpupoly_gauss_samp_prepare");
+    GpuContext *ctx = shape_of->ctx;
+    const uint32_t L = static_cast<uint32_t>(matrix_limbs(shape_of));
+    const uint32_t dpt = (ctx->crt_bits + base_bits - 1) / base_bits;
+    if (dpt == 0 || dpt > kGaussMaxDigits) return set_error("invalid digits_per_tower in gpupoly_gauss_samp_prepare");
+    if (!ctx->env.gsamp_hoist) return set_error("gpupoly_gauss_samp_prepare: unsupported: switched off (MXX_HIP_GSAMP_HOIST=0)");
+    if (ctx->env.gsamp_simple) return set_error("gpupoly_gauss_samp_prepare: unsupported: the one-kernel sampler has no first pass (MXX_HIP_GSAMP=simple)");
+    if (dpt > 4) return set_error("gpupoly_gauss_samp_prepare: unsupported: more than four digits per tower");
+    const size_t polys = matrix_polys(shape_of);
+    if (polys == 0) return set_error("gpupoly_gauss_samp_prepare: unsupported: a source without polynomials");
+    const size_t total = polys * L * static_cast<size_t>(ctx->N);
+    if ((total >> ctx->logN) >> 32 || (static_cast<size_t>(dpt) * L) >> 32)
+        return set_error("gpupoly_gauss_samp_prepare: matrix too large");
+    if (ctx_activate(ctx)) return 1;
+    CtxBlock a_buf(ctx), towers(ctx);
+    if (towers.alloc(static_cast<size_t>(L) * sizeof(GqTower)) || a_buf.alloc(total * 8 * sizeof(uint64_t))) return 1;
+    hipStream_t side = nullptr;
+    if (ctx_side_fork(ctx, &side)) return 1;
+    hipEvent_t done = ctx_event_take(ctx);
+    if (!done) return 1;
+    double *pd_words = static_cast<double *>(a_buf.ptr);
+    uint64_t *left_words = static_cast<uint64_t *>(a_buf.ptr) + total * dpt;
+    const ChaChaKey key = chacha_subkey(seed, 0, kTagGadget);
+    MXX_LAUNCH(gq_tower_kernel, dim3(1), dim3(64), 0, side, static_cast<GqTower *>(towers.ptr), ctx->d_limbs, L, dpt,
+                       base_bits, c);
+    MXX_TRACE_BYTES(static_cast<double>(total) * 8.0 * (8 - dpt));
+    const dim3 grid = item_grid(total, 256);
+    if (dpt <= 2)
+        MXX_LAUNCH(gauss_samp_normals_kernel<2>, grid, dim3(256), 0, side, pd_words, left_words, key, total,
+                           L, ctx->logN, dpt, base_bits, c, gq_pert_consts(dpt, base_bits));
+    else
+        MXX_LAUNCH(gauss_samp_normals_kernel<4>, grid, dim3(256), 0, side, pd_words, left_words, key, total,
+                           L, ctx->logN, dpt, base_bits, c, gq_pert_consts(dpt, base_bits));
+    hipError_t err = hipGetLastError();
+    if (err == hipSuccess) err = hipEventRecord(done, side);
+    if (err != hipSuccess) {
+        (void)hipStreamSynchronize(side);
+        ctx_event_return(ctx, done);
+        return set_error(err, "gpupoly_gauss_samp_prepare");
+    }
+    GpuGaussSampPrepared *prep = new GpuGaussSampPrepared();
+    prep->ctx = ctx;
+    prep->level = shape_of->level;
+    prep->rows = shape_of->rows;
+    prep->cols = shape_of->cols;
+    prep->base_bits = base_bits;
+    prep->dpt = dpt;
+    prep->c = c;
+    prep->key = key;
+    prep->towers = towers.release();
+    prep->a_buf = a_buf.release();
+    prep->done = done;
+    *out = prep;
+    return 0;
+    ABI_GUARD_END
+}
+
+extern "C" void gpupoly_gauss_samp_prepared_destroy(GpuGaussSampPrepared *prep) {
+    if (prep) gauss_samp_prepared_release(prep);
+}
+
+template <typename W, int MAXD>
+static int launch_gauss_samp_prepared(GpuContext *ctx, W *out, const W *src, size_t total, uint32_t src_cols, uint32_t L,
+                                      size_t k, const GpuGaussSampPrepared *prep) {
+    double *a_words = static_cast<double *>(prep->a_buf);
+    MXX_TRACE_BYTES(static_cast<double>(total) * (sizeof(W) + 16.0 * prep->dpt));
+    MXX_LAUNCH((gauss_samp_centres_kernel<W, MAXD>), item_grid(total, 256), dim3(256), 0, ctx->stream, a_words, src,
+                       ctx->d_limbs, total, L, ctx->logN, prep->dpt, prep->base_bits);
+    return launch_gauss_samp_lanes_finish<W, MAXD>(ctx, out, src, total, src_cols, L, prep->dpt, prep->base_bits, prep->c, k,
+                                                   prep->key, static_cast<const GqTower *>(prep->towers), a_words, nullptr);
+}
+
+extern "C" int gpupoly_matrix_gauss_samp_gq_arb_base_prepared(GpuMatrix *src, GpuGaussSampPrepared *prep, GpuMatrix *out) {
+    ABI_GUARD_BEGIN
+    if (!src || !prep || !out) return set_error("invalid gpupoly_matrix_gauss_samp_gq_arb_base_prepared arguments");
+    GpuContext *ctx = prep->ctx;
+    if (src->ctx != ctx || out->ctx != ctx)
+        return set_error("context mismatch in gpupoly_matrix_gauss_samp_gq_arb_base_prepared");
+    if (src->level != prep->level || out->level != prep->level)
+        return set_error("level mismatch in gpupoly_matrix_gauss_samp_gq_arb_base_prepared: not the level that was prepared");
+    if (src->rows != prep->rows || src->cols != prep->cols)
+        return set_error("shape mismatch in gpupoly_matrix_gauss_samp_gq_arb_base_prepared: not the shape that was prepared");
+    const size_t L = matrix_limbs(src);
+    const size_t k = static_cast<size_t>(prep->dpt) * L;
+    if (out->rows != src->rows * k || out->cols != src->cols)
+        return set_error("output size mismatch in gpupoly_matrix_gauss_samp_gq_arb_base_prepared");
+    if (storage_overlaps(src, out))
+        return set_error("gpupoly_matrix_gauss_samp_gq_arb_base_prepared: output must not alias the source");
+    const int requested = out->format;
+    const size_t total = matrix_words(src);
+    if (ctx_activate(ctx)) return 1;
+    if (src->format == GPU_POLY_FORMAT_EVAL) {
+        int rc = gpu_matrix_intt_all(src);
+        if (rc) return rc;
+    }
+    void *out_words = words_ptr(out);
+    const void *src_words = words_ptr(src);
+    if (ctx_side_join(ctx, prep->done)) return 1;
+    int rc;
+    if (ctx->wide)
+        rc = prep->dpt <= 2 ? launch_gauss_samp_prepared<uint64_t, 2>(ctx, static_cast<uint64_t *>(out_words), static_cast<const uint64_t *>(src_words), total, (uint32_t)src->cols, (uint32_t)L, k, prep)
+                            : launch_gauss_samp_prepared<uint64_t, 4>(ctx, static_cast<uint64_t *>(out_words), static_cast<const uint64_t *>(src_words), total, (uint32_t)src->cols, (uint32_t)L, k, prep);
+    else
+        rc = prep->dpt <= 2 ? launch_gauss_samp_prepared<uint32_t, 2>(ctx, static_cast<uint32_t *>(out_words), static_cast<const uint32_t *>(src_words), total, (uint32_t)src->cols, (uint32_t)L, k, prep)
+                            : launch_gauss_samp_prepared<uint32_t, 4>(ctx, static_cast<uint32_t *>(out_words), static_cast<const uint32_t *>(src_words), total, (uint32_t)src->cols, (uint32_t)L, k, prep);
+    if (rc) return rc;
+    gauss_samp_prepared_release(prep);
+    out->format = GPU_POLY_FORMAT_COEFF;
+    if (requested == GPU_POLY_FORMAT_EVAL) {
+        rc = launch_ntt(ctx, words_ptr(out), matrix_polys(out) * L, static_cast<int>(L), false);
+        if (rc) return rc;
+        out->format = GPU_POLY_FORMAT_EVAL;
+    }
+    return 0;
+    ABI_GUARD_END
 }
 
 struct P1KeyedSegments {
diff --git a/mxx_amd/matrix.py b/mxx_amd/matrix.py
--- a/mxx_amd/matrix.py
+++ b/mxx_amd/matrix.py
@@ -177,6 +177,34 @@
         self.raw = raw
         self.params = params
         self._finalizer = weakref.finalize(self, _ffi.lib().gpu_matrix_destroy_p1_covariance_cache, raw)
+
+
+class GpuGaussSampPrepared:
+
+    def __init__(self, raw, params):
+        self.raw = raw
+        self.params = params
+        self._finalizer = weakref.finalize(self, _ffi.lib().gpupoly_gauss_samp_prepared_destroy, raw)
+
+    @classmethod
+    def prepare(cls, shape_of: "GpuDCRTPolyMatrix", c: float, seed: GpuRngSeed):
+        raw = C.c_void_p()
+        st = _ffi.lib().gpupoly_gauss_samp_prepare(shape_of.raw, shape_of.params.base_bits(), c, seed, C.byref(raw))
+        if st != 0:
+            msg = _ffi.last_error_string()
+            if "unsupported" in msg:
+                return None
+            raise _ffi.GpuPolyError(f"gpupoly_gauss_samp_prepare failed: {msg}")
+        return cls(raw, shape_of.params)
+
+    def _consumed(self) -> None:
+        self._finalizer.detach()
+        self.raw = None
+
+    def destroy(self) -> None:
+        if self.raw is not None:
+            self.raw = None
+            self._finalizer()
 
 
 def _max_along(entries, axis, nrow, ncol):
@@ -1878,6 +1906,17 @@
         check_status(st, "gpu_matrix_gauss_samp_gq_arb_base")
         return out
 
+    def gauss_samp_gq_arb_base_prepared(self, prep: GpuGaussSampPrepared, coeff_out: bool = False) -> "GpuDCRTPolyMatrix":
+        assert prep.raw is not None, "the prepared handle was consumed or destroyed"
+        out = GpuDCRTPolyMatrix(self.params, self.nrow * self.params.modulus_digits(), self.ncol, self.params.crt_depth() - 1,
+                                not coeff_out)
+        st = _ffi.lib().gpupoly_matrix_gauss_samp_gq_arb_base_prepared(self.raw, prep.raw, out.raw)
+        check_status(st, "gpupoly_matrix_gauss_samp_gq_arb_base_prepared")
+        prep._consumed()
+        self._touch()
+        self.is_ntt = False
+        return out
+
     @staticmethod
     def create_p1_covariance_cache(a_mat, b_mat, d_mat, sigma, s, dgg_stddev) -> GpuP1CovarianceCache:
         raw = C.c_void_p()
diff --git a/mxx_amd/trapdoor.py b/mxx_amd/trapdoor.py
--- a/mxx_amd/trapdoor.py
+++ b/mxx_amd/trapdoor.py
@@ -4,7 +4,7 @@
 import threading
 import weakref
 
-from .matrix import GpuDCRTPolyMatrix
+from .matrix import GpuDCRTPolyMatrix, GpuGaussSampPrepared
 from .sampler import DistType, GpuDCRTPolyUniformSampler, random_gpu_rng_seed, sample_gpu_matrix_with_seed
 
 SPECTRAL_CONSTANT = 1.8
@@ -220,7 +220,8 @@
     def _draw_seeds():
         return random_gpu_rng_seed(), random_gpu_rng_seed(), random_gpu_rng_seed()
 
-    def _sample_pert_parts(self, params, td: GpuDCRTTrapdoor, s, c, dgg_stddev, sigma_large, total_ncol, stacked=None, seeds=None):
+    def _sample_pert_parts(self, params, td: GpuDCRTTrapdoor, s, c, dgg_stddev, sigma_large, total_ncol, stacked=None, seeds=None,
+                           before_p1=None):
         d, dk = td.r.row_size(), td.r.col_size()
         padded = -(-total_ncol // d) * d
         seed_p2 = seeds[0] if seeds is not None else random_gpu_rng_seed()
@@ -237,6 +238,8 @@
             if _traffic_bound(params, dk * padded):
                 tp2_eval = tp2.clone()
         cache = td.p1_covariance_cache(c, s, dgg_stddev)
+        if before_p1 is not None:
+            before_p1()
         p1 = GpuDCRTPolyMatrix.sample_p1_full_cached(cache, tp2, seeds[1] if seeds is not None else random_gpu_rng_seed())
         return p1, p2, tp2_eval, rp2
 
@@ -250,6 +253,10 @@
         p1_rows, p2_rows = td.re.row_size(), td.re.col_size()
         assert public_matrix.col_size() == p1_rows + p2_rows, "public matrix columns must match perturbation rows"
         left, right, stacked = td.public_matrix_parts(public_matrix)
+        dd, dk = td.r.row_size(), td.r.col_size()
+        if target_cols % dd == 0 and _traffic_bound(params, dk * target_cols):
+            return self._preimage_traffic_bound(params, td, s, dgg_large_std, left, right, stacked, target,
+                                                _seeds if _seeds is not None else self._draw_seeds())
         p1, p2, tp2, rp2 = self._sample_pert_parts(params, td, s, self.c, self.sigma, dgg_large_std, target_cols, stacked, _seeds)
         seed_z = _seeds[2] if _seeds is not None else None
         assert (p1.row_size(), p2.row_size()) == (p1_rows, p2_rows)
@@ -258,12 +265,6 @@
             p_hat_image = p_hat_image.slice_columns(0, target_cols)
         perturbed = target - p_hat_image
         out = GpuDCRTPolyMatrix(params, p1_rows + p2_rows, target_cols, p1.level, p1.is_ntt)
-        if p1.col_size() == target_cols and tp2 is not None:
-            z = perturbed.gauss_samp_gq_arb_base(self.c, self.sigma, seed_z if seed_z is not None else random_gpu_rng_seed(), coeff_out=True)
-            out.ntt_add_rows_from(p1_rows, z, p2, consume=True)
-            re_x = td.re * out.row_view(p1_rows, p1_rows + p2_rows)
-            out.add_rows_from(0, p1 - tp2, re_x)
-            return out
         z_hat = perturbed.gauss_samp_gq_arb_base(self.c, self.sigma, seed_z if seed_z is not None else random_gpu_rng_seed())
         re_z = td.re * z_hat
         if p1.col_size() == target_cols:
@@ -274,6 +275,29 @@
         out.copy_block_from(p2, p1_rows, 0, 0, 0, p2_rows, target_cols)
         out.add_block_from(re_z, 0, 0, 0, 0, re_z.row_size(), target_cols)
         out.add_block_from(z_hat, 2 * d, 0, 0, 0, z_hat.row_size(), target_cols)
+        return out
+
+    def _preimage_traffic_bound(self, params, td, s, dgg_large_std, left, right, stacked, target, seeds) -> GpuDCRTPolyMatrix:
+        target_cols = target.col_size()
+        p1_rows, p2_rows = td.re.row_size(), td.re.col_size()
+        prep = []
+        try:
+            p1, p2, tp2, rp2 = self._sample_pert_parts(
+                params, td, s, self.c, self.sigma, dgg_large_std, target_cols, stacked, seeds,
+                before_p1=lambda: prep.append(GpuGaussSampPrepared.prepare(target, self.c, seeds[2])))
+            assert (p1.row_size(), p2.row_size()) == (p1_rows, p2_rows) and p1.col_size() == target_cols and tp2 is not None
+            perturbed = target - ((left * p1) + (rp2 if rp2 is not None else right * p2))
+            out = GpuDCRTPolyMatrix(params, p1_rows + p2_rows, target_cols, p1.level, p1.is_ntt)
+            if prep and prep[0] is not None:
+                z = perturbed.gauss_samp_gq_arb_base_prepared(prep[0], coeff_out=True)
+            else:
+                z = perturbed.gauss_samp_gq_arb_base(self.c, self.sigma, seeds[2], coeff_out=True)
+        finally:
+            if prep and prep[0] is not None:
+                prep[0].destroy()
+        out.ntt_add_rows_from(p1_rows, z, p2, consume=True)
+        re_x = td.re * out.row_view(p1_rows, p1_rows + p2_rows)
+        out.add_rows_from(0, p1 - tp2, re_x)
         return out
 
     def preimage_reference_sequence(self, params, td: GpuDCRTTrapdoor, public_matrix, target) -> GpuDCRTPolyMatrix:
```

After: 8.257 million. Within noise of the previous version (-0.1%).
